# WISDEM/RAFT

Measured on AMD Instinct MI355X. Metric: design-case-frequency solves/sec (whole node), higher is better.
Workload: dtype f64

## Files before the change

raft_amd/csrc/raftx_geom.h:

```cpp
#pragma once

#define MP_N 24
#define MH_N 48
#define MI_N 48

__host__ __device__ inline void derive_design_tables(const double *strips, int64_t i0, int64_t i1, double *dsv,
                                                     int *dsf) {
    int64_t s = i0;
    while (s < i1) {
        int64_t e = s + 1;
        double proj[64];
        int np = 0;
        while (e < i1 && (e - s) < 64) {
            const double *pr = strips + (size_t)(e - 1) * NF, *cr = strips + (size_t)e * NF;
            bool same = true;
            double dv[3], pj = 0.0;
            for (int j = 0; j < 3; j++) {
                same = same && (pr[RAFTX_F_Q + j] == cr[RAFTX_F_Q + j]);
                dv[j] = cr[RAFTX_F_X + j] - pr[RAFTX_F_X + j];
                pj += dv[j] * cr[RAFTX_F_Q + j];
            }
            if (!same || !(pj > 0.0) || !(fabs(pj) <= 1.797e308)) break;
            double perp2 = 0.0, scale = 1.0;
            for (int j = 0; j < 3; j++) {
                double t = dv[j] - pj * cr[RAFTX_F_Q + j];
                perp2 += t * t;
                scale += fabs(cr[RAFTX_F_X + j]);
            }
            if (sqrt(perp2) > 1e-10 * scale) break;
            proj[np++] = pj;
            e++;
        }
        double unit = 0.0;
        for (int i = 0; i < np; i++) unit = (unit == 0.0 || proj[i] < unit) ? proj[i] : unit;
        for (int64_t i = s; i < e; i++) {
            const double *rec = strips + (size_t)i * NF;
            double *o = dsv + (size_t)i * DS_N;
            int m = 0;
            if (i > s && unit > 0.0) {
                double ratio = proj[i - s - 1] / unit;
                int mi = (int)floor(ratio + 0.5);
                if (mi >= 1 && mi <= 2 && fabs(ratio - mi) < 1e-9) {
                    const double *pr = strips + (size_t)(i - 1) * NF;
                    bool ok = true;
                    for (int j = 0; j < 3; j++) {
                        double pred = pr[RAFTX_F_X + j] + (double)mi * unit * rec[RAFTX_F_Q + j];
                        if (fabs(pred - rec[RAFTX_F_X + j]) > 1e-10 * (1.0 + fabs(rec[RAFTX_F_X + j]))) ok = false;
                    }
                    if (ok) m = mi;
                }
            }
            if (m != 0) {
                const double *pr = strips + (size_t)(i - 1) * NF;
                for (int j = 0; j < 3; j++)
                    if (pr[RAFTX_F_P1 + j] != rec[RAFTX_F_P1 + j] || pr[RAFTX_F_P2 + j] != rec[RAFTX_F_P2 + j]) m = 0;
                if ((pr[RAFTX_F_CIRC] != 0.0) != (rec[RAFTX_F_CIRC] != 0.0)) m = 0;
                if ((pr[RAFTX_F_MCF] >= 0.0) != (rec[RAFTX_F_MCF] >= 0.0)) m = 0;
                for (int j = 0; j < 3; j++) {
                    const double da = rec[RAFTX_F_AX + j] - pr[RAFTX_F_AX + j], dx = rec[RAFTX_F_X + j] - pr[RAFTX_F_X + j];
                    if (!(fabs(da - dx) <= 1e-9 * (1.0 + fabs(rec[RAFTX_F_X + j]) + fabs(rec[RAFTX_F_AX + j])))) m = 0;
                }
            }
            dsf[(size_t)i] = m | (rec[RAFTX_F_CIRC] != 0.0 ? DSI_CIRC : 0);
            for (int j = 0; j < DS_N; j++) o[j] = 0.0;
            o[DS_MCF] = rec[RAFTX_F_MCF];
            for (int j = 0; j < 3; j++) {
                o[DS_X + j] = rec[RAFTX_F_X + j];
                o[DS_U + j] = unit * rec[RAFTX_F_Q + j];
                o[DS_A + j] = rec[RAFTX_F_AX + j];
                o[DS_Q + j] = rec[RAFTX_F_Q + j];
                o[DS_P1 + j] = rec[RAFTX_F_P1 + j];
                o[DS_P2 + j] = rec[RAFTX_F_P2 + j];
            }
            if (fabs(o[DS_P1]) < 1e-15 && fabs(o[DS_P1 + 1]) < 1e-15 && fabs(o[DS_P2 + 2]) < 1e-15) dsf[(size_t)i] |= DSI_AXAL;
            if (fabs(o[DS_Q]) < 1e-15 && fabs(o[DS_Q + 1]) < 1e-15 && fabs(o[DS_P1 + 2]) < 1e-15 && fabs(o[DS_P2 + 2]) < 1e-15)
                dsf[(size_t)i] |= DSI_VAX;
            o[DS_IQ] = rec[RAFTX_F_IQ];
            o[DS_IQ + 1] = rec[RAFTX_F_IP1];
            o[DS_IQ + 2] = rec[RAFTX_F_IP2];
            o[DS_IQ + 3] = rec[RAFTX_F_AI];
            o[DS_IQ + 4] = rec[RAFTX_F_RHOV];
            o[DS_DQ] = rec[RAFTX_F_DQ];
            o[DS_DQ + 1] = rec[RAFTX_F_DP1];
            o[DS_DQ + 2] = rec[RAFTX_F_DP2];
            o[DS_DQ + 3] = rec[RAFTX_F_DEND];
        }
        s = e;
    }
}

struct GeomArgs {
    int nDesign;
    int64_t nMember;
    const int64_t *memberOff;
    const double *gm;
    const int64_t *stationOff;
    const double *gs;
    const double *pose;
    const int *mdesign;
    const int64_t *capOff;
    const double *caps;
    double *minert;
    int *err;
    double *Ms, *Cs, *Ws;
    const double *Fz;
    double *drho;
    double rho, g;
    int nw;
    const double *k;
    int *cnt, *cntm;
    double *mpose, *mhyd;
    double *abi;
    double *mcfaux;
    cplx *cm;
    int64_t *off, *cmoff;
    double *ds;
    int *dsi;
    double *A, *Ch, *Wh, *props;
    double *M0, *C0;
    int add_mask;
    int addup_in_design;
    long long *tot;
    long long *hostOut;
    int64_t mbase, sbase, cbase;
    int *mdesign_w;
    int mgrid;
    const double *fixRec;
    const int *fixInt, *fixIdx;
    int fixNM;
    __device__ int64_t mo(int d) const { return memberOff[d] - mbase; }
    __device__ int64_t so(int64_t m) const { return stationOff[m] - sbase; }
    __device__ int64_t co(int64_t m) const { return capOff[m] - cbase; }
};

#define GEOM_NOFMA _Pragma("clang fp contract(off)")

__device__ inline double geom_interp(double x, const double *gs, int n, int f) {
    GEOM_NOFMA
    if (x < gs[RAFTX_GS_S]) return gs[f];
    if (x > gs[(size_t)(n - 1) * RAFTX_GS_N + RAFTX_GS_S]) return gs[(size_t)(n - 1) * RAFTX_GS_N + f];
    int j = 0;
    for (int i = 0; i < n; i++)
        if (gs[(size_t)i * RAFTX_GS_N + RAFTX_GS_S] <= x) j = i;
    const double fj = gs[(size_t)j * RAFTX_GS_N + f];
    if (j == n - 1) return fj;
    const double xj = gs[(size_t)j * RAFTX_GS_N + RAFTX_GS_S];
    if (xj == x) return fj;
    const double slope = (gs[(size_t)(j + 1) * RAFTX_GS_N + f] - fj) / (gs[(size_t)(j + 1) * RAFTX_GS_N + RAFTX_GS_S] - xj);
    return slope * (x - xj) + fj;
}

struct GLocate {
    int idx;
    int j;
    double xj, dx;
};
__device__ inline GLocate geom_locate(double x, const double *gs, int n) {
    GEOM_NOFMA
    GLocate L{0, 0, 0.0, 0.0};
    if (x < gs[RAFTX_GS_S]) return L;
    if (x > gs[(size_t)(n - 1) * RAFTX_GS_N + RAFTX_GS_S]) { L.idx = n - 1; return L; }
    int j = 0;
    for (int i0 = 0; i0 < n; i0 += 8) {
        double sv[8];
#pragma unroll
        for (int u = 0; u < 8; u++) sv[u] = gs[(size_t)min(i0 + u, n - 1) * RAFTX_GS_N + RAFTX_GS_S];
#pragma unroll
        for (int u = 0; u < 8; u++)
            if (i0 + u < n && sv[u] <= x) j = i0 + u;
    }
    L.j = j;
    L.idx = j;
    if (j == n - 1) return L;
    L.xj = gs[(size_t)j * RAFTX_GS_N + RAFTX_GS_S];
    if (L.xj == x) return L;
    L.dx = gs[(size_t)(j + 1) * RAFTX_GS_N + RAFTX_GS_S] - L.xj;
    L.idx = -1;
    return L;
}
__device__ inline double geom_interp_at(const GLocate &L, double x, const double *gs, int f) {
    GEOM_NOFMA
    if (L.idx >= 0) return gs[(size_t)L.idx * RAFTX_GS_N + f];
    const double fj = gs[(size_t)L.j * RAFTX_GS_N + f];
    const double slope = (gs[(size_t)(L.j + 1) * RAFTX_GS_N + f] - fj) / L.dx;
    return slope * (x - L.xj) + fj;
}

__device__ inline int geom_interval_strips(double lstrip, double dlsMax) {
    GEOM_NOFMA
    if (lstrip > 0.0) return (int)ceil(lstrip / dlsMax);
    return lstrip == 0.0 ? 1 : 0;
}

struct GStrip {
    double ls, dls, ds0, ds1, drs0, drs1;
};
__device__ inline GStrip geom_strip(const double *gs, int n, int g, int j, int nsub, bool circ) {
    GEOM_NOFMA
    GStrip s;
    const int c1 = circ ? 0 : 1;
    if (g == 0) {
        s.ls = 0.0; s.dls = 0.0;
        s.ds0 = 0.5 * gs[RAFTX_GS_D]; s.ds1 = 0.5 * gs[RAFTX_GS_D + c1];
        s.drs0 = s.ds0; s.drs1 = s.ds1;
    } else if (g == n) {
        const double *b = gs + (size_t)(n - 1) * RAFTX_GS_N;
        s.ls = b[RAFTX_GS_S]; s.dls = 0.0;
        s.ds0 = 0.5 * b[RAFTX_GS_D]; s.ds1 = 0.5 * b[RAFTX_GS_D + c1];
        s.drs0 = -0.5 * b[RAFTX_GS_D]; s.drs1 = -0.5 * b[RAFTX_GS_D + c1];
    } else {
        const double *a = gs + (size_t)(g - 1) * RAFTX_GS_N, *b = gs + (size_t)g * RAFTX_GS_N;
        const double lstrip = b[RAFTX_GS_S] - a[RAFTX_GS_S];
        if (lstrip > 0.0) {
            const double dl = lstrip / nsub;
            const double m0 = 0.5 * (b[RAFTX_GS_D] - a[RAFTX_GS_D]) / lstrip;
            const double m1 = 0.5 * (b[RAFTX_GS_D + c1] - a[RAFTX_GS_D + c1]) / lstrip;
            s.ls = a[RAFTX_GS_S] + dl * (0.5 + j);
            s.dls = dl;
            s.ds0 = a[RAFTX_GS_D] + dl * 2 * m0 * (0.5 + j);
            s.ds1 = a[RAFTX_GS_D + c1] + dl * 2 * m1 * (0.5 + j);
            s.drs0 = dl * m0;
            s.drs1 = dl * m1;
        } else {
            s.ls = a[RAFTX_GS_S]; s.dls = 0.0;
            s.ds0 = 0.5 * (a[RAFTX_GS_D] + b[RAFTX_GS_D]); s.ds1 = 0.5 * (a[RAFTX_GS_D + c1] + b[RAFTX_GS_D + c1]);
            s.drs0 = 0.5 * (b[RAFTX_GS_D] - a[RAFTX_GS_D]); s.drs1 = 0.5 * (b[RAFTX_GS_D + c1] - a[RAFTX_GS_D + c1]);
        }
    }
    return s;
}
__device__ __forceinline__ void geom_strip_volumes(const GStrip &st, bool circ, double z, double &v_i, double &v_end, double &a_i) {
    GEOM_NOFMA
    const double ds0 = st.ds0, ds1 = st.ds1, dr0 = st.drs0, dr1 = st.drs1, dls = st.dls;
    if (circ) {
        v_i = 0.25 * M_PI * ds0 * ds0 * dls;
        const double a3 = ds0 + dr0, b3 = ds0 - dr0;
        v_end = M_PI / 12.0 * fabs(a3 * a3 * a3 - b3 * b3 * b3);
        a_i = M_PI * ds0 * dr0;
    } else {
        v_i = ds0 * ds1 * dls;
        const double ma = 0.5 * ((ds0 + dr0) + (ds1 + dr1)), mb = 0.5 * ((ds0 - dr0) + (ds1 - dr1));
        v_end = M_PI / 12.0 * (ma * ma * ma - mb * mb * mb);
        a_i = (ds0 + dr0) * (ds1 + dr1) - (ds0 - dr0) * (ds1 - dr1);
    }
    if (z + 0.5 * dls > 0) v_i = v_i * (0.5 * dls - z) / dls;
}
__device__ inline double geom_along(double rA, double rB, double ls, double L) {
    GEOM_NOFMA
    return rA + (ls / L) * (rB - rA);
}

__device__ inline void geom_frustum(double a0, double a1, double b0, double b1, bool circ, double H, double &V, double &hc) {
    GEOM_NOFMA
    const double sA = circ ? a0 : a0 + a1, sB = circ ? b0 : b0 + b1;
    if (sA == 0.0 && sB == 0.0) { V = 0.0; hc = 0.0; return; }
    double A1, A2, Am;
    if (circ) {
        A1 = (M_PI / 4) * a0 * a0; A2 = (M_PI / 4) * b0 * b0; Am = (M_PI / 4) * a0 * b0;
    } else {
        A1 = a0 * a1; A2 = b0 * b1; Am = sqrt(A1 * A2);
    }
    V = (A1 + A2 + Am) * H / 3;
    hc = ((A1 + 2 * Am + 3 * A2) / (A1 + Am + A2)) * H / 4;
}


__device__ inline double geom_pow5(double r) {
    GEOM_NOFMA
    const double h2 = r * r, l2 = fma(r, r, -h2);
    double h4 = h2 * h2, l4 = fma(h2, h2, -h4) + 2.0 * h2 * l2;
    const double s = h4 + l4;
    l4 = l4 - (s - h4);
    h4 = s;
    const double h5 = h4 * r, l5 = fma(h4, r, -h5) + l4 * r;
    return h5 + l5;
}
__device__ inline void geom_frustum_moi(double dA, double dB, double H, double p, double &Irad, double &Iax) {
    GEOM_NOFMA
    if (H == 0) { Irad = 0; Iax = 0; return; }
    const double r1 = dA / 2, r2 = dB / 2;
    if (dA == dB) {
        Irad = (1.0 / 12) * (p * H * M_PI * r1 * r1) * (3 * r1 * r1 + 4 * H * H);
        Iax = (1.0 / 2) * p * M_PI * H * r1 * r1 * r1 * r1;
    } else {
        const double q5 = (geom_pow5(r2) - geom_pow5(r1)) / (r2 - r1);
        Irad = (1.0 / 20) * p * M_PI * H * q5 + (1.0 / 30) * p * M_PI * H * H * H * (r1 * r1 + 3 * r1 * r2 + 6 * r2 * r2);
        Iax = (1.0 / 10) * p * M_PI * H * q5;
    }
}
__device__ inline void geom_rect_moi(double La, double Wa, double Lb, double Wb, double H, double p, double (&Iv)[3]) {
    GEOM_NOFMA
    if (H == 0) { Iv[0] = Iv[1] = Iv[2] = 0; return; }
    double x2, y2, z2;
    if (La == Lb && Wa == Wb) {
        const double M = p * La * Wa * H;
        Iv[0] = (1.0 / 12) * M * (Wa * Wa + 4 * H * H);
        Iv[1] = (1.0 / 12) * M * (La * La + 4 * H * H);
        Iv[2] = (1.0 / 12) * M * (La * La + Wa * Wa);
        return;
    } else if (La != Lb && Wa != Wb) {
        const double dL = Lb - La, dW = Wb - Wa;
        x2 = (1.0 / 12) * p * (dL * dL * dL * H * (Wb / 5 + Wa / 20) + dL * dL * La * H * (3 * Wb / 4 + Wa / 4) +
                               dL * La * La * H * (Wb + Wa / 2) + La * La * La * H * (Wb / 2 + Wa / 2));
        y2 = (1.0 / 12) * p * (dW * dW * dW * H * (Lb / 5 + La / 20) + dW * dW * Wa * H * (3 * Lb / 4 + La / 4) +
                               dW * Wa * Wa * H * (Lb + La / 2) + Wa * Wa * Wa * H * (Lb / 2 + La / 2));
        z2 = p * (Wb * Lb / 5 + Wa * Lb / 20 + La * Wb / 20 + Wa * La * (1.0 / 30)) * H * H * H;
    } else if (La == Lb) {
        x2 = (1.0 / 24) * p * (La * La * La) * H * (Wb + Wa);
        y2 = (1.0 / 48) * p * La * H * (Wb * Wb * Wb + Wa * Wb * Wb + Wa * Wa * Wb + Wa * Wa * Wa);
        z2 = (1.0 / 12) * p * La * (H * H * H) * (3 * Wb + Wa);
    } else {
        x2 = (1.0 / 48) * p * Wa * H * (Lb * Lb * Lb + La * Lb * Lb + La * La * Lb + La * La * La);
        y2 = (1.0 / 24) * p * (Wa * Wa * Wa) * H * (Lb + La);
        z2 = (1.0 / 12) * p * Wa * (H * H * H) * (3 * Lb + La);
    }
    Iv[0] = y2 + z2; Iv[1] = x2 + z2; Iv[2] = x2 + y2;
}
__device__ inline double geom_interp_inner(double x, const double *gs, int n, int c) {
    GEOM_NOFMA
#define DIN_(j) (gs[(size_t)(j) * RAFTX_GS_N + RAFTX_GS_D + c] - 2 * gs[(size_t)(j) * RAFTX_GS_N + RAFTX_GS_T])
    if (x < gs[RAFTX_GS_S]) return DIN_(0);
    if (x > gs[(size_t)(n - 1) * RAFTX_GS_N + RAFTX_GS_S]) return DIN_(n - 1);
    int j = 0;
    for (int i = 0; i < n; i++)
        if (gs[(size_t)i * RAFTX_GS_N + RAFTX_GS_S] <= x) j = i;
    const double fj = DIN_(j);
    if (j == n - 1) return fj;
    const double xj = gs[(size_t)j * RAFTX_GS_N + RAFTX_GS_S];
    if (xj == x) return fj;
    const double slope = (DIN_(j + 1) - fj) / (gs[(size_t)(j + 1) * RAFTX_GS_N + RAFTX_GS_S] - xj);
    return slope * (x - xj) + fj;
#undef DIN_
}
__device__ inline void geom_add_submember(double *M, double mass, const double (&Iv)[3], const double *p1, const double *p2,
                                          const double *q, const double (&r)[3], bool whole = false) {
    GEOM_NOFMA
    const double H[3][3] = {{0, r[2], -r[1]}, {-r[2], 0, r[0]}, {r[1], -r[0], 0}};
    for (int i = 0; i < 3; i++)
        for (int j = 0; j < 3; j++) {
            double hh = 0.0;
            for (int l = 0; l < 3; l++) hh += H[i][l] * mass * H[j][l];
            M[i * 6 + j] += (i == j) ? mass : 0.0;
            M[i * 6 + 3 + j] += mass * H[i][j];
            M[(3 + i) * 6 + j] += mass * H[j][i];
            const double ir = p1[i] * Iv[0] * p1[j] + p2[i] * Iv[1] * p2[j] + q[i] * Iv[2] * q[j];
            M[(3 + i) * 6 + 3 + j] += hh + (whole ? trunc(ir) : ir);
        }
}

struct GInertia {
    double M[36], mc[3], I3[3], vfill;
};
__device__ inline void geom_inertia_init(GInertia &J) {
    for (int i = 0; i < 36; i++) J.M[i] = 0.0;
    for (int c = 0; c < 3; c++) { J.mc[c] = 0.0; J.I3[c] = 0.0; }
    J.vfill = 0.0;
}
__device__ inline void geom_inertia_section(GInertia &J, const double *a, const double *b, bool circ, double rho_shell, bool trim,
                                            double drho, const double *rA, const double *q, const double *p1, const double *p2) {
    GEOM_NOFMA
    double (&M)[36] = J.M;
    double (&mc)[3] = J.mc;
    double (&I3)[3] = J.I3;
    double &vfill = J.vfill;
    {
        const double l = b[RAFTX_GS_S] - a[RAFTX_GS_S];
        double mass = 0.0, center[3] = {0, 0, 0};
        if (l > 0) {
            const double l_fill = (trim && a[RAFTX_GS_RHOFILL] == 0.0) ? 0.0 : a[RAFTX_GS_LFILL];
            const double rho_fill = a[RAFTX_GS_RHOFILL] + (l_fill > 0.0 ? drho : 0.0);
            const double dA0 = a[RAFTX_GS_D], dA1 = (circ ? a[RAFTX_GS_D] : a[RAFTX_GS_D + 1]), dB0 = b[RAFTX_GS_D], dB1 = (circ ? b[RAFTX_GS_D] : b[RAFTX_GS_D + 1]);
            const double iA0 = dA0 - 2 * a[RAFTX_GS_T], iA1 = dA1 - 2 * a[RAFTX_GS_T];
            const double iB0 = dB0 - 2 * b[RAFTX_GS_T], iB1 = dB1 - 2 * b[RAFTX_GS_T];
            const double f0 = (iB0 - iA0) * (l_fill / l) + iA0, f1 = (iB1 - iA1) * (l_fill / l) + iA1;
            double Vo, hco, Vi, hci, vf, hcf;
            geom_frustum(dA0, dA1, dB0, dB1, circ, l, Vo, hco);
            geom_frustum(iA0, iA1, iB0, iB1, circ, l, Vi, hci);
            const double m_shell = (Vo - Vi) * rho_shell;
            const double hc_shell = (Vo - Vi != 0) ? ((hco * Vo) - (hci * Vi)) / (Vo - Vi) : 0.0;
            geom_frustum(iA0, iA1, f0, f1, circ, l_fill, vf, hcf);
            vfill += vf;
            const double m_fill = vf * rho_fill;
            mass = m_shell + m_fill;
            const double hc = (mass != 0) ? ((hcf * m_fill) + (hc_shell * m_shell)) / mass : 0.0;
            if (circ) {
                double Iro, Iao, Iri, Iai, Irf, Iaf;
                geom_frustum_moi(dA0, dB0, l, rho_shell, Iro, Iao);
                geom_frustum_moi(iA0, iB0, l, rho_shell, Iri, Iai);
                geom_frustum_moi(iA0, f0, l_fill, rho_fill, Irf, Iaf);
                I3[0] = I3[1] = ((Iro - Iri) + Irf) - mass * hc * hc;
                I3[2] = (Iao - Iai) + Iaf;
            } else {
                double Io[3], Ii[3], If[3];
                geom_rect_moi(dA0, dA1, dB0, dB1, l, rho_shell, Io);
                geom_rect_moi(iA0, iA1, iB0, iB1, l, rho_shell, Ii);
                geom_rect_moi(iA0, iA1, f0, f1, l_fill, rho_fill, If);
                I3[0] = ((Io[0] - Ii[0]) + If[0]) - mass * hc * hc;
                I3[1] = ((Io[1] - Ii[1]) + If[1]) - mass * hc * hc;
                I3[2] = (Io[2] - Ii[2]) + If[2];
            }
            for (int c = 0; c < 3; c++) center[c] = rA[c] + q[c] * (a[RAFTX_GS_S] + hc);
        }
        double rel[3];
        for (int c = 0; c < 3; c++) { mc[c] += mass * center[c]; rel[c] = center[c] - rA[c]; }
        geom_add_submember(M, mass, I3, p1, p2, q, rel, !(l > 0));
    }
}
__device__ inline int geom_inertia_caps_finish(GInertia &J, const double *gs, int n, const double *gc, int ncap, bool circ,
                                               double rho_shell, const double *rA, const double *q, const double *p1,
                                               const double *p2, double g, double *out) {
    GEOM_NOFMA
    const int c1 = circ ? 0 : 1;
    double (&M)[36] = J.M;
    double (&mc)[3] = J.mc;
    const double vfill = J.vfill;
    const double s0 = gs[RAFTX_GS_S], s1 = gs[(size_t)(n - 1) * RAFTX_GS_N + RAFTX_GS_S];
    for (int i = 0; i < ncap; i++) {
        const double *cp = gc + (size_t)i * RAFTX_GC_N;
        const double Lc = cp[RAFTX_GC_S], h = cp[RAFTX_GC_T];
        double dA[2] = {0, 0}, dB[2] = {0, 0}, dAi[2] = {0, 0}, dBi[2] = {0, 0};
        int where;
        if (Lc == s0) {
            where = 0;
            for (int c = 0; c <= c1; c++) {
                dA[c] = gs[RAFTX_GS_D + c] - 2 * gs[RAFTX_GS_T];
                dB[c] = geom_interp_inner(Lc + h, gs, n, c);
                dAi[c] = cp[RAFTX_GC_DIN + c];
                dBi[c] = dB[c] * (dAi[c] / dA[c]);
            }
        } else if (Lc == s1) {
            where = 1;
            if (!circ) return 2;
            dA[0] = geom_interp_inner(Lc - h, gs, n, 0);
            dB[0] = gs[(size_t)(n - 1) * RAFTX_GS_N + RAFTX_GS_D] - 2 * gs[(size_t)(n - 1) * RAFTX_GS_N + RAFTX_GS_T];
            dBi[0] = cp[RAFTX_GC_DIN];
            dAi[0] = dA[0] * (dBi[0] / dB[0]);
        } else if ((Lc > s0 && Lc < s0 + h) || (Lc < s1 && Lc > s1 - h)) {
            return 3;
        } else {
            where = 2;
            if (!circ) return 2;
            if (i < ncap - 1 && Lc == gc[(size_t)(i + 1) * RAFTX_GC_N + RAFTX_GC_S]) {
                if (i >= n) return 4;
                dA[0] = geom_interp_inner(Lc - h, gs, n, 0);
                dB[0] = gs[(size_t)i * RAFTX_GS_N + RAFTX_GS_D] - 2 * gs[(size_t)i * RAFTX_GS_N + RAFTX_GS_T];
                dBi[0] = cp[RAFTX_GC_DIN];
                dAi[0] = dA[0] * (dBi[0] / dB[0]);
            } else if (i > 0 && Lc == gc[(size_t)(i - 1) * RAFTX_GC_N + RAFTX_GC_S]) {
                if (i >= n) return 4;
                dA[0] = gs[(size_t)i * RAFTX_GS_N + RAFTX_GS_D] - 2 * gs[(size_t)i * RAFTX_GS_N + RAFTX_GS_T];
                dB[0] = geom_interp_inner(Lc + h, gs, n, 0);
                dAi[0] = cp[RAFTX_GC_DIN];
                dBi[0] = dB[0] * (dAi[0] / dA[0]);
            } else {
                dA[0] = geom_interp_inner(Lc - h / 2, gs, n, 0);
                dB[0] = geom_interp_inner(Lc + h / 2, gs, n, 0);
                const double dM = geom_interp_inner(Lc, gs, n, 0);
                dAi[0] = dA[0] * (cp[RAFTX_GC_DIN] / dM);
                dBi[0] = dB[0] * (cp[RAFTX_GC_DIN] / dM);
            }
        }
        double Vo, hco, Vi, hci;
        geom_frustum(dA[0], dA[1], dB[0], dB[1], circ, h, Vo, hco);
        geom_frustum(dAi[0], dAi[1], dBi[0], dBi[1], circ, h, Vi, hci);
        const double m_cap = (Vo - Vi) * rho_shell;
        const double hc_cap = (Vo - Vi != 0) ? ((hco * Vo) - (hci * Vi)) / (Vo - Vi) : 0.0;
        double Ic[3];
        if (circ) {
            double Iro, Iao, Iri, Iai;
            geom_frustum_moi(dA[0], dB[0], h, rho_shell, Iro, Iao);
            geom_frustum_moi(dAi[0], dBi[0], h, rho_shell, Iri, Iai);
            Ic[0] = Ic[1] = (Iro - Iri) - m_cap * hc_cap * hc_cap;
            Ic[2] = Iao - Iai;
        } else {
            double Io[3], Ii[3];
            geom_rect_moi(dA[0], dA[1], dB[0], dB[1], h, rho_shell, Io);
            geom_rect_moi(dAi[0], dAi[1], dBi[0], dBi[1], h, rho_shell, Ii);
            Ic[0] = (Io[0] - Ii[0]) - m_cap * hc_cap * hc_cap;
            Ic[1] = (Io[1] - Ii[1]) - m_cap * hc_cap * hc_cap;
            Ic[2] = Io[2] - Ii[2];
        }
        double rel[3];
        for (int c = 0; c < 3; c++) {
            const double pos = rA[c] + q[c] * Lc;
            const double cc = (where == 0) ? pos + q[c] * hc_cap : (where == 1 ? pos - q[c] * (h - hc_cap) : pos - q[c] * ((h / 2) - hc_cap));
            rel[c] = cc - rA[c];
            mc[c] += m_cap * cc;
        }
        geom_add_submember(M, m_cap, Ic, p1, p2, q, rel);
    }
    const double mass = M[0];
    for (int i = 0; i < 36; i++) out[i] = M[i];
    out[36] = mass;
    double dR[3];
    for (int c = 0; c < 3; c++) {
        const double cen = (mass != 0) ? mc[c] / mass : 0.0;
        out[37 + c] = cen;
        dR[c] = cen - rA[c];
    }
    const double Fz = -g * mass;
    out[40] = 0.0; out[41] = 0.0; out[42] = Fz;
    out[43] = dR[1] * Fz; out[44] = -dR[0] * Fz; out[45] = 0.0;
    out[46] = -mass * g * dR[2];
    out[47] = vfill;
    return 0;
}
__device__ inline int geom_member_inertia(const double *gm, const double *gs, int n, const double *gc, int ncap,
                                          const double *rA, const double *q, const double *p1, const double *p2, double g,
                                          bool trim, double drho, double *out) {
    const bool circ = gm[RAFTX_GM_SHAPE] != 0.0;
    const double rho_shell = gm[RAFTX_GM_RHOSHELL];
    GInertia J;
    geom_inertia_init(J);
    for (int i = 1; i < n; i++)
        geom_inertia_section(J, gs + (size_t)(i - 1) * RAFTX_GS_N, gs + (size_t)i * RAFTX_GS_N, circ, rho_shell, trim, drho, rA, q, p1, p2);
    return geom_inertia_caps_finish(J, gs, n, gc, ncap, circ, rho_shell, rA, q, p1, p2, g, out);
}

__global__ void k_geom_zero(GeomArgs A) {
    const int d = blockIdx.x * blockDim.x + threadIdx.x;
    if (d < A.nDesign) {
        A.drho[d] = 0.0;
        A.off[d + 1] = 0;
        A.cmoff[d + 1] = 0;
    }
    if (d < 4) A.err[d] = 0;
    if (d < 5) A.tot[d] = 0;
    if (d == 0) { A.off[0] = 0; A.cmoff[0] = 0; }
    if (d < A.nDesign)
        for (int64_t m = A.mo(d); m < A.mo(d + 1); m++) A.mdesign_w[m] = d;
}
#define GEOM_MAX_STATIONS 1024
__device__ inline int64_t geom_member_of_thread(const GeomArgs &A) {
    const int64_t t = (int64_t)blockIdx.x * blockDim.x + threadIdx.x;
    if (A.mgrid <= 0) return t < A.nMember ? t : -1;
    const int64_t k = t / A.nDesign;
    if (k >= A.mgrid) return -1;
    const int d = (int)(t % A.nDesign);
    const int64_t m = A.mo(d) + k;
    return m < A.mo(d + 1) ? m : -1;
}
__device__ __forceinline__ void geom_load_row(const double *gs, int i, double (&r)[RAFTX_GS_N]) {
    const double2 *p = reinterpret_cast<const double2 *>(gs + (size_t)i * RAFTX_GS_N);
#pragma unroll
    for (int k = 0; k < RAFTX_GS_N / 2; k++) {
        const double2 v = p[k];
        r[2 * k] = v.x;
        r[2 * k + 1] = v.y;
    }
}
struct GMember {
    int wet, wetm;
    int code;
    int rej;
};
__device__ __forceinline__ void geom_pose(const double *gm, const double (&ps)[6], double (&rA0)[3], double (&q)[3], double (&p1)[3],
                                          double (&p2)[3], double (&rA)[3], double (&rB)[3], double (&R)[2][2]) {
    GEOM_NOFMA
    double q0[3], nrm = 0.0;
    for (int i = 0; i < 3; i++) {
        rA0[i] = gm[RAFTX_GM_RA + i];
        q0[i] = gm[RAFTX_GM_RB + i] - gm[RAFTX_GM_RA + i];
        nrm += q0[i] * q0[i];
    }
    nrm = sqrt(nrm);
    for (int i = 0; i < 3; i++) q0[i] /= nrm;
    const double beta = atan2(q0[1], q0[0]);
    const double phi = atan2(sqrt(q0[0] * q0[0] + q0[1] * q0[1]), q0[2]);
    const double gam = gm[RAFTX_GM_GAMMA] * (M_PI / 180.0);
    const double s1 = sin(beta), c1 = cos(beta), s2 = sin(phi), c2 = cos(phi), s3 = sin(gam), c3 = cos(gam);
    const double R0[3][3] = {{c1 * c2 * c3 - s1 * s3, -c3 * s1 - c1 * c2 * s3, c1 * s2},
                             {c1 * s3 + c2 * c3 * s1, c1 * c3 - c2 * s1 * s3, s1 * s2},
                             {-c3 * s2, s2 * s3, c2}};
    const double p10[3] = {R0[0][0], R0[1][0], R0[2][0]};
    const double p20[3] = {q0[1] * p10[2] - q0[2] * p10[1], q0[2] * p10[0] - q0[0] * p10[2], q0[0] * p10[1] - q0[1] * p10[0]};
    const double sy = sin(ps[5]), cy = cos(ps[5]), sp = sin(ps[4]), cp = cos(ps[4]), sr = sin(ps[3]), cr = cos(ps[3]);
    const double Rp[3][3] = {{cy * cp, cy * sp * sr - cr * sy, sy * sr + cy * cr * sp},
                             {cp * sy, cy * cr + sy * sp * sr, cr * sy * sp - cy * sr},
                             {-sp, cp * sr, cp * cr}};
    const double L = gm[RAFTX_GM_L];
    for (int i = 0; i < 3; i++) {
        q[i] = Rp[i][0] * q0[0] + Rp[i][1] * q0[1] + Rp[i][2] * q0[2];
        p1[i] = Rp[i][0] * p10[0] + Rp[i][1] * p10[1] + Rp[i][2] * p10[2];
        p2[i] = Rp[i][0] * p20[0] + Rp[i][1] * p20[1] + Rp[i][2] * p20[2];
        const double dsp = (Rp[i][0] - (i == 0 ? 1.0 : 0.0)) * rA0[0] + (Rp[i][1] - (i == 1 ? 1.0 : 0.0)) * rA0[1] +
                           (Rp[i][2] - (i == 2 ? 1.0 : 0.0)) * rA0[2];
        rA[i] = rA0[i] + (ps[i] + dsp);
    }
    for (int i = 0; i < 3; i++) rB[i] = rA[i] + L * q[i];
    for (int i = 0; i < 2; i++)
        for (int j = 0; j < 2; j++) R[i][j] = Rp[i][0] * R0[0][j] + Rp[i][1] * R0[1][j] + Rp[i][2] * R0[2][j];
}
#define FR_N (MP_N + MH_N + MI_N)
#define FR_I 4
__device__ __forceinline__ GMember geom_member_body(const double *gmrow, const double *gs, const int n, const double *gc, const int ncap,
                                                    const double *pose, const double rho, const double g, const bool trim,
                                                    const bool haveK, double *mp, double *mh, double *mi) {
    GEOM_NOFMA
    GMember res = {0, 0, 0, 0};
    double gm[RAFTX_GM_N];
    {
        const double2 *p = reinterpret_cast<const double2 *>(gmrow);
#pragma unroll
        for (int k = 0; k < RAFTX_GM_N / 2; k++) {
            const double2 v = p[k];
            gm[2 * k] = v.x;
            gm[2 * k + 1] = v.y;
        }
    }
    if (n < 2 || n > GEOM_MAX_STATIONS || !(gm[RAFTX_GM_DLSMAX] > 0.0) || !(gm[RAFTX_GM_L] > 0.0)) {
        res.rej = 1;
        return res;
    }
    if (((int)gm[RAFTX_GM_FLAGS] & RAFTX_GM_FLAG_MCF) && gm[RAFTX_GM_SHAPE] != 0.0 && !haveK) {
        res.rej = 2;
        return res;
    }
    double ps[6] = {0, 0, 0, 0, 0, 0};
    if (pose)
        for (int i = 0; i < 6; i++) ps[i] = pose[i];
    double a[RAFTX_GS_N], b[RAFTX_GS_N];
    geom_load_row(gs, 0, b);
    const bool circ = gm[RAFTX_GM_SHAPE] != 0.0;
    const int flags = (int)gm[RAFTX_GM_FLAGS];
    double rA0[3], q[3], p1[3], p2[3], rA[3], rB[3], R[2][2];
    const double L = gm[RAFTX_GM_L];
    geom_pose(gm, ps, rA0, q, p1, p2, rA, rB, R);
    int wet = 0;
    if (geom_along(rA[2], rB[2], 0.0, L) < 0) wet++;
    double C[36], F[6], Vt = 0.0, rcV[3] = {0, 0, 0}, AWPm = 0.0;
    for (int i = 0; i < 36; i++) C[i] = 0.0;
    for (int i = 0; i < 6; i++) F[i] = 0.0;
    const double beta2 = atan2(q[1], q[0]), phi2 = atan2(sqrt(q[0] * q[0] + q[1] * q[1]), q[2]);
    const double cosPhi = cos(phi2), sinPhi = sin(phi2), tanPhi = tan(phi2), cosBeta = cos(beta2), sinBeta = sin(beta2);
    const double rg = rho * g;
    const bool nostatic = (flags & RAFTX_GM_FLAG_NOSTATIC) != 0;
    const double rho_shell = gm[RAFTX_GM_RHOSHELL];
    for (int i = 1; i < n; i++) {
#pragma unroll
        for (int f = 0; f < RAFTX_GS_N; f++) a[f] = b[f];
        geom_load_row(gs, i, b);
        {
            const double lstrip = b[RAFTX_GS_S] - a[RAFTX_GS_S];
            const int cntg = geom_interval_strips(lstrip, gm[RAFTX_GM_DLSMAX]);
            for (int j = 0; j < cntg; j++) {
                double ls;
                if (lstrip > 0.0) {
                    const double dl = lstrip / cntg;
                    ls = a[RAFTX_GS_S] + dl * (0.5 + j);
                } else {
                    ls = a[RAFTX_GS_S];
                }
                if (geom_along(rA[2], rB[2], ls, L) < 0) wet++;
            }
        }
        if (nostatic) continue;
        {
            double ra[3], rb[3];
            for (int c = 0; c < 3; c++) {
                ra[c] = rA[c] + q[c] * a[RAFTX_GS_S];
                rb[c] = rA[c] + q[c] * b[RAFTX_GS_S];
            }
            const double aD1 = circ ? a[RAFTX_GS_D] : a[RAFTX_GS_D + 1], bD1 = circ ? b[RAFTX_GS_D] : b[RAFTX_GS_D + 1];
            if (ra[2] * rb[2] <= 0) {
                const double t = (0 - ra[2]);
                double xWP = ra[0] + t * (rb[0] - ra[0]) / (rb[2] - ra[2]);
                double yWP = ra[1] + t * (rb[1] - ra[1]) / (rb[2] - ra[2]);
                const double w0 = b[RAFTX_GS_D] + t * (a[RAFTX_GS_D] - b[RAFTX_GS_D]) / (rb[2] - ra[2]);
                const double w1 = bD1 + t * (aD1 - bD1) / (rb[2] - ra[2]);
                double AWP, IxWP, IyWP;
                if (circ) {
                    AWP = (M_PI / 4) * w0 * w0;
                    IxWP = IyWP = (M_PI / 64) * w0 * w0 * w0 * w0;
                } else {
                    AWP = w0 * w1;
                    const double Ix = (1.0 / 12) * w0 * w1 * w1 * w1, Iy = (1.0 / 12) * w0 * w0 * w0 * w1;
                    IxWP = R[0][0] * Ix * R[0][0] + R[0][1] * Iy * R[0][1];
                    IyWP = R[1][0] * Ix * R[1][0] + R[1][1] * Iy * R[1][1];
                }
                const double LWP = fabs(ra[2] / cosPhi);
                double V, hc;
                geom_frustum(a[RAFTX_GS_D], aD1, w0, w1, circ, LWP, V, hc);
                double M = 0.0;
                if (circ) M = -rg * M_PI * (w0 * w0 / 32 * (2.0 + tanPhi * tanPhi) + 0.5 * (ra[2] / cosPhi) * (ra[2] / cosPhi)) * sinPhi;
                const double Fz = rg * V;
                const double ex = ra[0] - rA[0], ey = ra[1] - rA[1];
                F[2] += Fz;
                F[3] += ey * Fz;
                F[4] += -ex * Fz;
                F[3] += M * (-sinBeta);
                F[4] += M * cosBeta;
                xWP -= rA[0];
                yWP -= rA[1];
                C[2 * 6 + 2] += rg * AWP / cosPhi;
                C[2 * 6 + 3] += rg * (-AWP * yWP);
                C[2 * 6 + 4] += rg * (AWP * xWP);
                C[3 * 6 + 2] += rg * (-AWP * yWP);
                C[3 * 6 + 3] += rg * (IxWP + AWP * yWP * yWP);
                C[3 * 6 + 4] += rg * (AWP * xWP * yWP);
                C[4 * 6 + 2] += rg * (AWP * xWP);
                C[4 * 6 + 3] += rg * (AWP * xWP * yWP);
                C[4 * 6 + 4] += rg * (IyWP + AWP * xWP * xWP);
                double rc[3];
                for (int c = 0; c < 3; c++) rc[c] = ra[c] + q[c] * hc;
                C[3 * 6 + 3] += rg * V * (rc[2] - rA[2]);
                C[4 * 6 + 4] += rg * V * (rc[2] - rA[2]);
                C[3 * 6 + 5] += -rg * V * (rc[0] - rA[0]);
                C[4 * 6 + 5] += -rg * V * (rc[1] - rA[1]);
                Vt += V;
                for (int c = 0; c < 3; c++) rcV[c] += rc[c] * V;
                AWPm = AWP;
            } else if (ra[2] <= 0 && rb[2] <= 0) {
                double V, hc;
                geom_frustum(a[RAFTX_GS_D], aD1, b[RAFTX_GS_D], bD1, circ, b[RAFTX_GS_S] - a[RAFTX_GS_S], V, hc);
                double rc[3], rr[3];
                for (int c = 0; c < 3; c++) { rc[c] = ra[c] + q[c] * hc; rr[c] = rc[c] - rA[c]; }
                const double Fz = rg * V;
                F[2] += Fz;
                F[3] += rr[1] * Fz;
                F[4] += -rr[0] * Fz;
                C[3 * 6 + 3] += rg * V * rr[2];
                C[4 * 6 + 4] += rg * V * rr[2];
                C[3 * 6 + 5] += -rg * V * rr[0];
                C[4 * 6 + 5] += -rg * V * rr[1];
                Vt += V;
                for (int c = 0; c < 3; c++) rcV[c] += rc[c] * V;
            }
        }
    }
    if (geom_along(rA[2], rB[2], b[RAFTX_GS_S], L) < 0) wet++;
    if (!nostatic) {
        for (int i = 0; i < 36; i++) mh[i] = C[i];
        for (int i = 0; i < 6; i++) mh[36 + i] = F[i];
        mh[42] = Vt; mh[43] = rcV[0]; mh[44] = rcV[1]; mh[45] = rcV[2]; mh[46] = AWPm; mh[47] = 0.0;
    }
    int code = 0;
    if (!nostatic) {
        GInertia J;
        geom_inertia_init(J);
        geom_load_row(gs, 0, b);
        for (int i = 1; i < n; i++) {
#pragma unroll
            for (int f = 0; f < RAFTX_GS_N; f++) a[f] = b[f];
            geom_load_row(gs, i, b);
            geom_inertia_section(J, a, b, circ, rho_shell, trim, 0.0, rA, q, p1, p2);
        }
        code = geom_inertia_caps_finish(J, gs, n, gc, ncap, circ, rho_shell, rA, q, p1, p2, g, mi);
    }
    for (int i = 0; i < 3; i++) {
        mp[i] = rA0[i]; mp[3 + i] = rA[i]; mp[6 + i] = q[i]; mp[9 + i] = p1[i]; mp[12 + i] = p2[i];
    }
    mp[15] = R[0][0]; mp[16] = R[0][1]; mp[17] = R[1][0]; mp[18] = R[1][1]; mp[19] = L;
    const int wetm = ((flags & RAFTX_GM_FLAG_MCF) && circ && !(flags & RAFTX_GM_FLAG_POTMOD)) ? wet : 0;
    res.wet = wet;
    res.wetm = wetm;
    if (nostatic) {
        for (int i = 0; i < MH_N; i++) mh[i] = 0.0;
        for (int i = 0; i < MI_N; i++) mi[i] = 0.0;
        return res;
    }
    if (code) {
        for (int i = 0; i < MI_N; i++) mi[i] = 0.0;
        res.code = code;
    }
    return res;
}

struct FixedArgs {
    int nFix;
    const double *gm, *gs, *gc;
    const int *desc;
    double rho, g;
    int trim, haveK;
    double *rec;
    int *irec;
};
__global__ __launch_bounds__(64) void k_geom_member_fixed(FixedArgs F) {
    const int f = blockIdx.x * blockDim.x + threadIdx.x;
    if (f >= F.nFix) return;
    const int *ds = F.desc + (size_t)f * 5;
    double *r = F.rec + (size_t)f * FR_N;
    const GMember R = geom_member_body(F.gm + (size_t)ds[0] * RAFTX_GM_N, F.gs + (size_t)ds[1] * RAFTX_GS_N, ds[2],
                                       ds[4] >= 0 ? F.gc + (size_t)ds[3] * RAFTX_GC_N : nullptr, ds[4] >= 0 ? ds[4] : 0, nullptr, F.rho,
                                       F.g, F.trim != 0, F.haveK != 0, r, r + MP_N, r + MP_N + MH_N);
    int *ir = F.irec + (size_t)f * FR_I;
    ir[0] = R.wet; ir[1] = R.wetm; ir[2] = R.code; ir[3] = R.rej;
}
__global__ __launch_bounds__(128) void k_geom_member(GeomArgs A) {
    GEOM_NOFMA
    if (A.mgrid > 0 && A.err[2]) return;
    const int64_t m = geom_member_of_thread(A);
    if (m < 0) return;
    if (A.err[2]) {
        A.cnt[m] = 0;
        A.cntm[m] = 0;
        return;
    }
    GMember R;
    int d;
    const int fix = A.fixRec ? A.fixIdx[m % A.fixNM] : -1;
    if (fix >= 0) {
        d = (int)(m / A.fixNM);
        const int4 ir = *reinterpret_cast<const int4 *>(A.fixInt + (size_t)fix * FR_I);
        R.wet = ir.x; R.wetm = ir.y; R.code = ir.z; R.rej = ir.w;
        if (!R.rej) {
            const double2 *src = reinterpret_cast<const double2 *>(A.fixRec + (size_t)fix * FR_N);
            double2 *mp = reinterpret_cast<double2 *>(A.mpose + (size_t)m * MP_N), *mh = reinterpret_cast<double2 *>(A.mhyd + (size_t)m * MH_N),
                    *mi = reinterpret_cast<double2 *>(A.minert + (size_t)m * MI_N);
#pragma unroll
            for (int i = 0; i < MP_N / 2; i++) mp[i] = src[i];
#pragma unroll 8
            for (int i = 0; i < MH_N / 2; i++) mh[i] = src[MP_N / 2 + i];
#pragma unroll 8
            for (int i = 0; i < MI_N / 2; i++) mi[i] = src[(MP_N + MH_N) / 2 + i];
        }
    } else {
        const int64_t so0 = A.so(m), so1 = A.so(m + 1);
        const int64_t co0 = A.capOff ? A.co(m) : 0, co1 = A.capOff ? A.co(m + 1) : 0;
        d = A.mdesign[m];
        R = geom_member_body(A.gm + (size_t)m * RAFTX_GM_N, A.gs + (size_t)so0 * RAFTX_GS_N, (int)(so1 - so0),
                             A.capOff ? A.caps + (size_t)co0 * RAFTX_GC_N : nullptr, A.capOff ? (int)(co1 - co0) : 0,
                             A.pose ? A.pose + (size_t)d * 6 : nullptr, A.rho, A.g, (A.add_mask & RAFTX_TRIM_BALLAST) != 0, A.k != nullptr,
                             A.mpose + (size_t)m * MP_N, A.mhyd + (size_t)m * MH_N, A.minert + (size_t)m * MI_N);
    }
    if (R.rej) {
        A.cnt[m] = 0;
        A.cntm[m] = 0;
        atomicCAS(A.err + 3, 0, R.rej == 1 ? (int)(m + 1) : -(int)(m + 1));
        return;
    }
    A.cnt[m] = R.wet;
    A.cntm[m] = R.wetm;
    if (R.wet) atomicAdd(reinterpret_cast<unsigned long long *>(A.off + d + 1), (unsigned long long)R.wet);
    if (R.wetm) atomicAdd(reinterpret_cast<unsigned long long *>(A.cmoff + d + 1), (unsigned long long)R.wetm);
    if (R.code) atomicCAS(A.err, 0, (int)(m + 1));
}

__global__ void k_geom_trim(GeomArgs A) {
    GEOM_NOFMA
    if (A.err[2] | A.err[3]) return;
    const int d = blockIdx.x * blockDim.x + threadIdx.x;
    if (d >= A.nDesign) return;
    double mass = A.M0[(size_t)d * 36], V = 0.0, vol = 0.0;
    for (int64_t m = A.mo(d); m < A.mo(d + 1); m++) {
        mass += A.minert[(size_t)m * MI_N + 36];
        vol += A.minert[(size_t)m * MI_N + 47];
        V += A.mhyd[(size_t)m * MH_N + 42];
    }
    if (!(vol > 0.0)) {
        A.drho[d] = 0.0;
        atomicCAS(A.err + 1, 0, d + 1);
        return;
    }
    const double sumFz = -mass * A.g + V * A.rho * A.g + (A.Fz ? A.Fz[d] : 0.0);
    A.drho[d] = sumFz / A.g / vol;
}
__global__ __launch_bounds__(128) void k_geom_reinertia(GeomArgs A) {
    GEOM_NOFMA
    if (A.err[2] | A.err[3]) return;
    const int64_t m = geom_member_of_thread(A);
    if (m < 0) return;
    const double *gm = A.gm + (size_t)m * RAFTX_GM_N;
    if ((int)gm[RAFTX_GM_FLAGS] & RAFTX_GM_FLAG_NOSTATIC) return;
    const double *gs = A.gs + (size_t)A.so(m) * RAFTX_GS_N;
    const int n = (int)(A.so(m + 1) - A.so(m));
    const double *mp = A.mpose + (size_t)m * MP_N;
    const int ncap = A.capOff ? (int)(A.co(m + 1) - A.co(m)) : 0;
    const double *gc = A.capOff ? A.caps + (size_t)A.co(m) * RAFTX_GC_N : nullptr;
    double *mi = A.minert + (size_t)m * MI_N;
    if (geom_member_inertia(gm, gs, n, gc, ncap, mp + 3, mp + 6, mp + 9, mp + 12, A.g, true, A.drho[A.mdesign[m]], mi))
        for (int i = 0; i < MI_N; i++) mi[i] = 0.0;
}

#define GSCAN_CH 4096
template <int T>
__global__ __launch_bounds__(T) void k_geom_scan_t(GeomArgs A) {
    __shared__ long long part[2][17];
    __shared__ unsigned buf[2][GSCAN_CH];
    const int t = threadIdx.x;
    const int n = A.nDesign;
    constexpr int PER = GSCAN_CH / T;
    long long carrya = 0, carryb = 0, mx = 0;
    for (int c0 = 0; c0 < n; c0 += GSCAN_CH) {
        const int cn = (n - c0 < GSCAN_CH) ? n - c0 : GSCAN_CH;
        for (int i = t; i < GSCAN_CH; i += T) {
            long long va = 0, vb = 0;
            if (i < cn) { va = A.off[c0 + i + 1]; vb = A.cmoff[c0 + i + 1]; }
            buf[0][i] = (unsigned)va;
            buf[1][i] = (unsigned)vb;
            mx = va > mx ? va : mx;
        }
        __syncthreads();
        long long a = 0, b = 0;
        for (int i = 0; i < PER; i++) { a += buf[0][t * PER + i]; b += buf[1][t * PER + i]; }
        const int lane = t & 63, wv = t >> 6;
        long long ia = a, ib = b;
        for (int o = 1; o < 64; o <<= 1) {
            const long long ua = __shfl_up(ia, o, 64), ub = __shfl_up(ib, o, 64);
            if (lane >= o) { ia += ua; ib += ub; }
        }
        if (lane == 63) { part[0][wv] = ia; part[1][wv] = ib; }
        __syncthreads();
        long long ra = carrya, rb = carryb, sa = 0, sb = 0;
        for (int i = 0; i < T / 64; i++) {
            if (i < wv) { ra += part[0][i]; rb += part[1][i]; }
            sa += part[0][i]; sb += part[1][i];
        }
        ra += ia - a;
        rb += ib - b;
        for (int i = 0; i < PER; i++) {
            ra += buf[0][t * PER + i];
            rb += buf[1][t * PER + i];
            buf[0][t * PER + i] = (unsigned)ra;
            buf[1][t * PER + i] = (unsigned)rb;
        }
        __syncthreads();
        for (int i = t; i < cn; i += T) {
            const long long va = buf[0][i], vb = buf[1][i];
            A.off[c0 + i + 1] = va;
            A.cmoff[c0 + i + 1] = vb;
            if (A.hostOut) A.hostOut[8 + c0 + i + 1] = va;
        }
        carrya += sa;
        carryb += sb;
        __syncthreads();
    }
    if (mx) atomicMax(reinterpret_cast<unsigned long long *>(A.tot + 2), (unsigned long long)mx);
    __syncthreads();
    if (t == 0) {
        A.off[0] = 0;
        A.cmoff[0] = 0;
        A.tot[0] = carrya;
        A.tot[1] = carryb;
        if (A.hostOut) {
            A.hostOut[0] = carrya;
            A.hostOut[1] = carryb;
            A.hostOut[2] = A.tot[2];
            int *e = reinterpret_cast<int *>(A.hostOut + 3);
            e[0] = A.err[0]; e[1] = A.err[1]; e[2] = A.err[2]; e[3] = A.err[3];
            A.hostOut[8] = 0;
        }
    }
}
__global__ __launch_bounds__(64) void k_geom_mcf(GeomArgs A, int64_t nRows) {
    GEOM_NOFMA
    const int64_t row = blockIdx.x;
    const int iw = blockIdx.y * blockDim.x + threadIdx.x;
    if (row >= nRows || iw >= A.nw) return;
    const double R = A.mcfaux[row * 3], Ca1 = A.mcfaux[row * 3 + 1], Ca2 = A.mcfaux[row * 3 + 2];
    const double k = A.k[iw];
    const double Tr = M_PI / 5 / R;
    double ramp;
    if (k <= 0.0) ramp = 0.0;
    else if (k < Tr) ramp = 0.5 * (1 - cos(M_PI * k / Tr));
    else ramp = 1.0;
    double cr = 0.0, ci = 0.0;
    if (ramp != 0.0) {
        const double x = k * R;
        const double hr = 0.5 * (j0(x) - jn(2, x)), hi = 0.5 * (y0(x) - yn(2, x));
        const double den = M_PI * (x * x);
        const double mag = den * (hr * hr + hi * hi);
        cr = 4.0 * hi / mag;
        ci = 4.0 * hr / mag;
    }
    A.cm[((size_t)row * 2 + 0) * A.nw + iw] = cplx{cr * ramp + (1.0 + Ca1) * (1 - ramp), ci * ramp};
    A.cm[((size_t)row * 2 + 1) * A.nw + iw] = cplx{cr * ramp + (1.0 + Ca2) * (1 - ramp), ci * ramp};
}


__device__ inline void geom_reduce_matrix(const double *C, const double (&a)[3], double *out) {
    GEOM_NOFMA
    const double H[3][3] = {{0, a[2], -a[1]}, {-a[2], 0, a[0]}, {a[1], -a[0], 0}};
    double t12[3][3], t21[3][3];
    for (int i = 0; i < 3; i++)
        for (int j = 0; j < 3; j++) {
            double s12 = C[i * 6 + 3 + j], s21 = C[(3 + i) * 6 + j];
            for (int l = 0; l < 3; l++) {
                s12 += C[i * 6 + l] * H[l][j];
                s21 += H[l][i] * C[l * 6 + j];
            }
            t12[i][j] = s12;
            t21[i][j] = s21;
        }
    for (int i = 0; i < 3; i++)
        for (int j = 0; j < 3; j++) {
            out[i * 6 + j] += C[i * 6 + j];
            out[i * 6 + 3 + j] += t12[i][j];
            out[(3 + i) * 6 + j] += t21[i][j];
            double s = C[(3 + i) * 6 + 3 + j];
            for (int l = 0; l < 3; l++) s += H[l][i] * t12[l][j] + C[(3 + i) * 6 + l] * H[l][j];
            out[(3 + i) * 6 + 3 + j] += s;
        }
}
__device__ inline void geom_reduce_vector(const double *W, const double (&a)[3], const double *arm0, const double (&th)[3],
                                          double *Wout, double *Cout) {
    GEOM_NOFMA
    Wout[0] += W[0]; Wout[1] += W[1]; Wout[2] += W[2];
    Wout[3] += W[3] + (a[1] * W[2] - a[2] * W[1]);
    Wout[4] += W[4] + (a[2] * W[0] - a[0] * W[2]);
    Wout[5] += W[5] + (a[0] * W[1] - a[1] * W[0]);
    for (int j = 0; j < 3; j++) {
        double tj[3] = {th[0], th[1], th[2]};
        tj[j] += 1.0;
        const double dA[3] = {arm0[0] + (tj[1] * a[2] - tj[2] * a[1]) - a[0], arm0[1] + (tj[2] * a[0] - tj[0] * a[2]) - a[1],
                              arm0[2] + (tj[0] * a[1] - tj[1] * a[0]) - a[2]};
        Cout[3 * 6 + 3 + j] -= dA[1] * W[2] - dA[2] * W[1];
        Cout[4 * 6 + 3 + j] -= dA[2] * W[0] - dA[0] * W[2];
        Cout[5 * 6 + 3 + j] -= dA[0] * W[1] - dA[1] * W[0];
    }
}

__device__ constexpr int DS_SRC[DS_N] = {
    -1, -1, RAFTX_F_MCF, -1,
    RAFTX_F_X, RAFTX_F_X + 1, RAFTX_F_X + 2,
    -2, -3, -4,
    RAFTX_F_AX, RAFTX_F_AX + 1, RAFTX_F_AX + 2,
    RAFTX_F_Q, RAFTX_F_Q + 1, RAFTX_F_Q + 2,
    RAFTX_F_P1, RAFTX_F_P1 + 1, RAFTX_F_P1 + 2,
    RAFTX_F_P2, RAFTX_F_P2 + 1, RAFTX_F_P2 + 2,
    RAFTX_F_IQ, RAFTX_F_IP1, RAFTX_F_IP2, RAFTX_F_AI, RAFTX_F_RHOV,
    RAFTX_F_DQ, RAFTX_F_DP1, RAFTX_F_DP2, RAFTX_F_DEND, -1};
static_assert(DS_MCF == 2 && DS_X == 4 && DS_U == 7 && DS_A == 10 && DS_Q == 13 && DS_P1 == 16 && DS_P2 == 19 &&
              DS_IQ == 22 && DS_DQ == 27 && DS_N == 32, "DS_SRC follows the device record layout");
#define GD_ROW (NF + 1)
#define GD_GM_N 3
#define GD_MP_N 13
#ifdef GEOM_PHASE_TIMING
__device__ unsigned long long geom_phase_cycles[10];
#define GEOM_PHASE(i)                                                                                   \
    do {                                                                                                \
        __syncthreads();                                                                                \
        const unsigned long long now_ = wall_clock64();                                                 \
        if (threadIdx.x == 0) atomicAdd(&geom_phase_cycles[i], now_ - tphase_);                         \
        tphase_ = now_;                                                                                 \
    } while (0)
#define GEOM_PHASE_BEGIN unsigned long long tphase_ = wall_clock64();
#else
#define GEOM_PHASE(i)
#define GEOM_PHASE_BEGIN
#endif
#ifndef GD_T
#define GD_T 128
#endif
static_assert(GD_T % 64 == 0 && GD_T % DS_N == 0 && GD_T <= 256, "k_geom_design: whole wavefronts, a lane keeps its record field");
template <bool ABI, bool ADDUP>
__device__ __forceinline__ void geom_design_block(const GeomArgs &A, const int d, double *gd_lds, int *wcnt) {
    GEOM_NOFMA
    const int lane = threadIdx.x;
    const int64_t i0 = A.off[d], i1 = A.off[d + 1];
    const int S = (int)(i1 - i0);
    double *rec = gd_lds;
    double *pjv = rec + (size_t)S * GD_ROW, *unv = pjv + S;
    int *okv = reinterpret_cast<int *>(unv + S), *rsv = okv + S, *mfl = rsv + S;
    GEOM_PHASE_BEGIN
    {
        const int64_t m0 = A.mo(d), m1 = A.mo(d + 1);
        const int nMem = (int)(m1 - m0);
        const int64_t s0 = A.so(m0);
        const int nSta = (int)(A.so(m1) - s0);
        int *mcum = mfl + S;
        int *mbase = mcum + nSta + 2 * nMem;
        int *ssta = mbase + nMem + 1;
        double *sgm = reinterpret_cast<double *>(okv + (((int)(ssta - okv) + nMem + 2) & ~1));
        double *sgs = sgm + (size_t)nMem * GD_GM_N;
        double *smp = sgs + (size_t)nSta * RAFTX_GS_N;
        int cnt_lane = 0;
        {
            const double *g0 = A.gm + (size_t)m0 * RAFTX_GM_N, *g1 = A.gs + (size_t)s0 * RAFTX_GS_N, *g2 = A.mpose + (size_t)m0 * MP_N;
            const int n0 = nMem * GD_GM_N, n01 = n0 + nSta * RAFTX_GS_N, total = n01 + nMem * GD_MP_N;
            constexpr int SU = 10;
            const int64_t so_lane = lane <= nMem ? A.so(m0 + lane) : s0;
            cnt_lane = lane < nMem ? A.cnt[m0 + lane] : 0;
            for (int base = 0; base < total; base += SU * GD_T) {
                double v[SU];
#pragma unroll
                for (int u = 0; u < SU; u++) {
                    const int idx = base + u * GD_T + lane;
                    const double *src;
                    if (idx < n0) {
                        const int row = idx / GD_GM_N, col = idx % GD_GM_N;
                        src = g0 + (size_t)row * RAFTX_GM_N + (col == 0 ? RAFTX_GM_DLSMAX : (col == 1 ? RAFTX_GM_SHAPE : RAFTX_GM_FLAGS));
                    } else if (idx < n01) {
                        src = g1 + (idx - n0);
                    } else {
                        const int k = idx - n01, row = k / GD_MP_N, col = k % GD_MP_N;
                        src = g2 + (size_t)row * MP_N + (col < 12 ? 3 + col : 19);
                    }
                    v[u] = idx < total ? *src : 0.0;
                }
#pragma unroll
                for (int u = 0; u < SU; u++) {
                    const int idx = base + u * GD_T + lane;
                    if (idx < total) sgm[idx] = v[u];
                }
            }
            if (lane <= nMem) mbase[lane] = ssta[lane] = (int)(so_lane - s0);
            for (int mi = lane + GD_T; mi <= nMem; mi += GD_T) mbase[mi] = ssta[mi] = (int)(A.so(m0 + mi) - s0);
        }
        __syncthreads();
        for (int u = lane; u < nSta + nMem; u += GD_T) {
            int mi = 0;
            while (mi + 1 < nMem && mbase[mi + 1] + mi + 1 <= u) mi++;
            const int sta0 = mbase[mi], n = mbase[mi + 1] - sta0, g = u - (sta0 + mi);
            int cntg = 1;
            if (g > 0 && g < n) {
                const double *gs = sgs + (size_t)sta0 * RAFTX_GS_N;
                cntg = geom_interval_strips(gs[(size_t)g * RAFTX_GS_N + RAFTX_GS_S] - gs[(size_t)(g - 1) * RAFTX_GS_N + RAFTX_GS_S],
                                            sgm[(size_t)mi * GD_GM_N]);
            }
            mcum[sta0 + 2 * mi + g + 1] = cntg;
        }
        __syncthreads();
        for (int mi = lane; mi < nMem; mi += GD_T) {
            const int n = ssta[mi + 1] - ssta[mi];
            int *cum = mcum + ssta[mi] + 2 * mi;
            const bool dry = (mi == lane ? cnt_lane : A.cnt[m0 + mi]) == 0;
            int a = 0;
            cum[0] = 0;
            for (int g = 0; g <= n; g++) { a += dry ? 0 : cum[g + 1]; cum[g + 1] = a; }
            mbase[mi + 1] = a;
        }
        __syncthreads();
        if (lane == 0) {
            int a = 0;
            mbase[0] = 0;
            for (int mi = 0; mi < nMem; mi++) { a += mbase[mi + 1]; mbase[mi + 1] = a; }
        }
        __syncthreads();
        const int total = mbase[nMem];
        GEOM_PHASE(0);
        const double rho = A.rho, cdrag = sqrt(8 / M_PI);
        double rP[3] = {0, 0, 0};
        if (A.pose)
            for (int i = 0; i < 3; i++) rP[i] = A.pose[(size_t)d * 6 + i];
        int nwet = 0;
        for (int t0 = 0; t0 < total; t0 += GD_T) {
            const int t = t0 + lane;
            const bool act = t < total;
            const int tq = act ? t : 0;
            int mi = 0;
            while (mi + 1 < nMem && mbase[mi + 1] <= tq) mi++;
            const int64_t m = m0 + mi;
            const int tt = tq - mbase[mi];
            const int n = ssta[mi + 1] - ssta[mi];
            const int *cum = mcum + ssta[mi] + 2 * mi;
            const double *gm = sgm + (size_t)mi * GD_GM_N;
            const double *gs = sgs + (size_t)ssta[mi] * RAFTX_GS_N;
            const double *mp = smp + (size_t)mi * GD_MP_N;
            const bool circ = gm[1] != 0.0;
            const int flags = (int)gm[2];
            const bool potMod = flags & RAFTX_GM_FLAG_POTMOD;
            const bool mcf = (flags & RAFTX_GM_FLAG_MCF) && circ && !potMod;
            const double L = mp[12];
            double rA[3], rB[3], q[3], p1[3], p2[3], armN[3];
            for (int i = 0; i < 3; i++) {
                rA[i] = mp[i]; q[i] = mp[3 + i]; p1[i] = mp[6 + i]; p2[i] = mp[9 + i];
                rB[i] = rA[i] + L * q[i];
                armN[i] = rA[i] - rP[i];
            }
            int g = 0;
            while (g < n && cum[g + 1] <= tt) g++;
            const int j = tt - cum[g];
            const int nsub = (g > 0 && g < n) ? cum[g + 1] - cum[g] : 1;
            GStrip st = geom_strip(gs, n, g, j, nsub, circ);
            double r[3];
            for (int c = 0; c < 3; c++) r[c] = geom_along(rA[c], rB[c], st.ls, L);
            const bool wet = act && (r[2] < 0);
            const GLocate at = geom_locate(st.ls, gs, n);
            const unsigned long long mask = __ballot(wet);
            const int wv = lane >> 6, ln = lane & 63;
            if (ln == 0) wcnt[wv] = __popcll(mask);
            __syncthreads();
            int before = 0, all = 0;
            for (int w = 0; w < GD_T / 64; w++) {
                before += w < wv ? wcnt[w] : 0;
                all += wcnt[w];
            }
            const int pos = nwet + before + __popcll(mask & ((1ull << ln) - 1ull));
            nwet += all;
            __syncthreads();
            if (!wet || pos >= S) continue;
            double *row = rec + (size_t)pos * GD_ROW;
            for (int c = 0; c < NF; c++) row[c] = 0.0;
            for (int c = 0; c < 3; c++) {
                row[RAFTX_F_X + c] = r[c];
                row[RAFTX_F_AX + c] = (r[c] - rA[c]) + armN[c];
                row[RAFTX_F_Q + c] = q[c];
                row[RAFTX_F_P1 + c] = p1[c];
                row[RAFTX_F_P2 + c] = p2[c];
            }
            row[RAFTX_F_CIRC] = circ ? 1.0 : 0.0;
            row[RAFTX_F_MCF] = -1.0;
            row[26] = (double)mi;
            row[27] = (double)tt;
            const double ds0 = st.ds0, ds1 = st.ds1, dr0 = st.drs0, dr1 = st.drs1, dls = st.dls;
            if (!potMod) {
                double v_i, v_end, a_i;
                geom_strip_volumes(st, circ, r[2], v_i, v_end, a_i);
                const double Ca1 = geom_interp_at(at, st.ls, gs, RAFTX_GS_CA + 1), Ca2 = geom_interp_at(at, st.ls, gs, RAFTX_GS_CA + 2);
                const double CaE = geom_interp_at(at, st.ls, gs, RAFTX_GS_CA + 3);
                row[RAFTX_F_IQ] = rho * v_end * CaE;
                row[RAFTX_F_AI] = a_i;
                row[RAFTX_F_RHOV] = rho * v_i;
                row[RAFTX_F_AP1] = rho * v_i * Ca1;
                row[RAFTX_F_AP2] = rho * v_i * Ca2;
                if (mcf) {
                    int64_t cmbase = A.cmoff[d], cmrow0 = cmbase;
                    int wet0 = 0;
                    for (int64_t mm = m0; mm < m; mm++) { cmrow0 += A.cntm[mm]; wet0 += A.cnt[mm]; }
                    const int posm = pos - wet0;
                    row[RAFTX_F_MCF] = (double)((cmrow0 - cmbase) + posm);
                    double *ax = A.mcfaux + (size_t)(cmrow0 + posm) * 3;
                    ax[0] = ds0 / 2; ax[1] = Ca1; ax[2] = Ca2;
                } else {
                    row[RAFTX_F_IP1] = rho * v_i * (1.0 + Ca1);
                    row[RAFTX_F_IP2] = rho * v_i * (1.0 + Ca2);
                }
            }
            double a_q, a_p1, a_p2, a_end;
            if (circ) {
                a_q = M_PI * ds0 * dls; a_p1 = ds0 * dls; a_p2 = ds0 * dls; a_end = fabs(M_PI * ds0 * dr0);
            } else {
                a_q = 2 * (ds0 + ds0) * dls; a_p1 = ds0 * dls; a_p2 = ds1 * dls;
                a_end = fabs((ds0 + dr0) * (ds1 + dr1) - (ds0 - dr0) * (ds1 - dr1));
            }
            row[RAFTX_F_DQ] = cdrag * 0.5 * rho * a_q * geom_interp_at(at, st.ls, gs, RAFTX_GS_CD + 0);
            row[RAFTX_F_DP1] = cdrag * 0.5 * rho * a_p1 * geom_interp_at(at, st.ls, gs, RAFTX_GS_CD + 1);
            row[RAFTX_F_DP2] = cdrag * 0.5 * rho * a_p2 * geom_interp_at(at, st.ls, gs, RAFTX_GS_CD + 2);
            row[RAFTX_F_DEND] = cdrag * 0.5 * rho * a_end * geom_interp_at(at, st.ls, gs, RAFTX_GS_CD + 3);
        }
        __syncthreads();
        GEOM_PHASE(1);
        if constexpr (ABI) {
            double *abi = A.abi + (size_t)i0 * NF;
            for (int t = lane; t < S * NF; t += GD_T) abi[t] = rec[(t / NF) * GD_ROW + (t % NF)];
        }
    }
    __syncthreads();
    GEOM_PHASE(2);
    for (int t = lane; t < S; t += GD_T) {
        bool pass = false;
        double pj = 0.0;
        const double *pr = rec + (size_t)(t > 0 ? t - 1 : 0) * GD_ROW, *cr = rec + (size_t)t * GD_ROW;
        double pq[3], cq[3], px[3], cx[3];
        for (int j = 0; j < 3; j++) {
            pq[j] = pr[RAFTX_F_Q + j]; cq[j] = cr[RAFTX_F_Q + j]; px[j] = pr[RAFTX_F_X + j]; cx[j] = cr[RAFTX_F_X + j];
        }
        if (t > 0) {
            bool same = true;
            double dv[3];
            for (int j = 0; j < 3; j++) {
                same = same && (pq[j] == cq[j]);
                dv[j] = cx[j] - px[j];
                pj += dv[j] * cq[j];
            }
            if (same && (pj > 0.0) && (fabs(pj) <= 1.797e308)) {
                double perp2 = 0.0, scale = 1.0;
                for (int j = 0; j < 3; j++) {
                    double tt = dv[j] - pj * cq[j];
                    perp2 += tt * tt;
                    scale += fabs(cx[j]);
                }
                pass = !(sqrt(perp2) > 1e-10 * scale);
            }
        }
        okv[t] = pass ? 1 : 0;
        pjv[t] = pj;
    }
    __syncthreads();
    bool serial = S > GD_T;
    if (!serial) {
        const int wv = lane >> 6, ln = lane & 63;
        const bool st = lane < S && (lane == 0 || !okv[lane]);
        const unsigned long long mask = __ballot(st);
        if (ln == 0) wcnt[wv] = mask ? wv * 64 + 63 - __builtin_clzll(mask) : -1;
        if (st) reinterpret_cast<unsigned long long *>(unv)[lane] = 0x7ff0000000000000ull;
        __syncthreads();
        const unsigned long long below = mask & (ln == 63 ? ~0ull : ((2ull << ln) - 1ull));
        int s = below ? wv * 64 + 63 - __builtin_clzll(below) : -1;
        for (int w = wv - 1; w >= 0 && s < 0; w--) s = wcnt[w];
        if (lane < S) {
            rsv[lane] = s;
            if (!st) atomicMin(reinterpret_cast<unsigned long long *>(unv) + s, (unsigned long long)__double_as_longlong(pjv[lane]));
        }
        serial = __syncthreads_or(lane < S && lane - s >= 64) != 0;
        if (!serial && st && reinterpret_cast<unsigned long long *>(unv)[lane] == 0x7ff0000000000000ull) unv[lane] = 0.0;
    }
    if (serial && lane == 0) {
        int s = 0;
        double unit = 0.0;
        for (int t = 0; t < S; t++) {
            if (t == 0 || !okv[t] || (t - s) >= 64) {
                if (t > 0) unv[s] = unit;
                s = t;
                unit = 0.0;
            } else {
                const double pj = pjv[t];
                unit = (unit == 0.0 || pj < unit) ? pj : unit;
            }
            rsv[t] = s;
        }
        if (S > 0) unv[s] = unit;
    }
    __syncthreads();
    for (int t = lane; t < S; t += GD_T) {
        const int s = rsv[t];
        const double unit = unv[s];
        const double *cr = rec + (size_t)t * GD_ROW, *pr = rec + (size_t)(t > 0 ? t - 1 : 0) * GD_ROW;
        double cX[3], cQ[3], cP1[3], cP2[3], cA[3], pX[3], pP1[3], pP2[3], pA[3];
        for (int j = 0; j < 3; j++) {
            cX[j] = cr[RAFTX_F_X + j]; cQ[j] = cr[RAFTX_F_Q + j]; cP1[j] = cr[RAFTX_F_P1 + j]; cP2[j] = cr[RAFTX_F_P2 + j];
            cA[j] = cr[RAFTX_F_AX + j];
            pX[j] = pr[RAFTX_F_X + j]; pP1[j] = pr[RAFTX_F_P1 + j]; pP2[j] = pr[RAFTX_F_P2 + j]; pA[j] = pr[RAFTX_F_AX + j];
        }
        const double cCirc = cr[RAFTX_F_CIRC], cMcf = cr[RAFTX_F_MCF], pCirc = pr[RAFTX_F_CIRC], pMcf = pr[RAFTX_F_MCF];
        const double pjt = pjv[t];
        int m = 0;
        if (t > s && unit > 0.0) {
            double ratio = pjt / unit;
            int mi = (int)floor(ratio + 0.5);
            if (mi >= 1 && mi <= 2 && fabs(ratio - mi) < 1e-9) {
                bool ok = true;
                for (int j = 0; j < 3; j++) {
                    double pred = pX[j] + (double)mi * unit * cQ[j];
                    if (fabs(pred - cX[j]) > 1e-10 * (1.0 + fabs(cX[j]))) ok = false;
                }
                if (ok) m = mi;
            }
        }
        if (m != 0) {
            for (int j = 0; j < 3; j++)
                if (pP1[j] != cP1[j] || pP2[j] != cP2[j]) m = 0;
            if ((pCirc != 0.0) != (cCirc != 0.0)) m = 0;
            if ((pMcf >= 0.0) != (cMcf >= 0.0)) m = 0;
            for (int j = 0; j < 3; j++) {
                const double da = cA[j] - pA[j], dx = cX[j] - pX[j];
                if (!(fabs(da - dx) <= 1e-9 * (1.0 + fabs(cX[j]) + fabs(cA[j])))) m = 0;
            }
        }
        int fl = m | (cCirc != 0.0 ? DSI_CIRC : 0);
        if (fabs(cP1[0]) < 1e-15 && fabs(cP1[1]) < 1e-15 && fabs(cP2[2]) < 1e-15) fl |= DSI_AXAL;
        if (fabs(cQ[0]) < 1e-15 && fabs(cQ[1]) < 1e-15 && fabs(cP1[2]) < 1e-15 && fabs(cP2[2]) < 1e-15)
            fl |= DSI_VAX;
        A.dsi[(size_t)i0 + t] = fl;
    }
    GEOM_PHASE(3);
    {
        double *dso = A.ds + (size_t)i0 * DS_N;
        const int j = lane % DS_N, f = DS_SRC[j], nT = S * DS_N;
        constexpr int DU = 4;
        for (int t0 = lane; t0 < nT; t0 += DU * GD_T) {
          double vv[DU];
#pragma unroll
          for (int u = 0; u < DU; u++) {
            const int t = t0 + u * GD_T;
            const int i = t < nT ? t / DS_N : 0;
            const double *cr = rec + (size_t)i * GD_ROW;
            double v = 0.0;
            if (f >= 0) v = cr[f];
            else if (f <= -2) v = unv[rsv[i]] * cr[RAFTX_F_Q + (-2 - f)];
            if (t < nT && j == DS_MCF && v >= 0.0) {
                const double *ax0 = A.mcfaux + (size_t)A.cmoff[d] * 3, *axm = ax0 + (size_t)v * 3;
                const int mrow = (int)v;
                for (int r = 0; r < mrow; r++)
                    if (ax0[r * 3] == axm[0] && ax0[r * 3 + 1] == axm[1] && ax0[r * 3 + 2] == axm[2]) {
                        v = (double)r;
                        break;
                    }
            }
            vv[u] = v;
          }
#pragma unroll
          for (int u = 0; u < DU; u++) {
            const int t = t0 + u * GD_T;
            if (t < nT) dso[t] = vv[u];
          }
        }
    }
    GEOM_PHASE(4);
    constexpr int GV = 21;
    for (int t0 = 0; t0 < S; t0 += GD_T) {
        const int t = t0 + lane;
        double gv[GV];
        if (t < S) {
            const double *cr = rec + (size_t)t * GD_ROW;
            const double ax = cr[RAFTX_F_AX], ay = cr[RAFTX_F_AX + 1], az = cr[RAFTX_F_AX + 2];
            const double cs[3] = {cr[RAFTX_F_AP1], cr[RAFTX_F_AP2], cr[RAFTX_F_IQ]};
            const int fs[3] = {RAFTX_F_P1, RAFTX_F_P2, RAFTX_F_Q};
            for (int tt = 0; tt < 3; tt++) {
                const double nx = cr[fs[tt]], ny = cr[fs[tt] + 1], nz = cr[fs[tt] + 2];
                gv[tt * 7] = cs[tt];
                gv[tt * 7 + 1] = nx; gv[tt * 7 + 2] = ny; gv[tt * 7 + 3] = nz;
                gv[tt * 7 + 4] = ay * nz - az * ny;
                gv[tt * 7 + 5] = az * nx - ax * nz;
                gv[tt * 7 + 6] = ax * ny - ay * nx;
            }
        }
        __syncthreads();
        if (t < S)
            for (int e = 0; e < GV; e++) rec[(size_t)t * GV + e] = gv[e];
    }
    __syncthreads();
    GEOM_PHASE(5);
    {
        const int k3 = lane / 36, e = lane % 36, i = e / 6, j = e % 6;
        double am = 0.0;
        if (k3 < 3) {
            const int lo = (int)(((long long)S * k3) / 3), hi = (int)(((long long)S * (k3 + 1)) / 3);
            for (int s = lo; s < hi; s++) {
                const double *g = rec + (size_t)s * GV;
                for (int tt = 0; tt < 3; tt++) am += g[tt * 7] * g[tt * 7 + 1 + i] * g[tt * 7 + 1 + j];
            }
        }
        __syncthreads();
        if (k3 < 3) rec[lane] = am;
        __syncthreads();
        if (lane < 36) {
            am = (rec[lane] + rec[36 + lane]) + rec[72 + lane];
            const size_t o = (size_t)d * 36 + lane;
            A.A[o] = am;
            if constexpr (ADDUP) {
                double m0 = A.M0[o], c0 = A.C0[o];
                if (A.add_mask & RAFTX_ADD_MORISON) m0 += am;
                if (A.add_mask & RAFTX_ADD_HYDROSTATIC) c0 += A.Ch[o];
                if (A.add_mask & RAFTX_ADD_INERTIA) { m0 += A.Ms[o]; c0 += A.Cs[o]; }
                A.M0[o] = m0;
                A.C0[o] = c0;
            }
        }
    }
    GEOM_PHASE(6);
    (void)mfl;
}
__global__ __launch_bounds__(GD_T) void k_geom_design(GeomArgs A) {
    extern __shared__ double gd_lds[];
    __shared__ int wcnt[GD_T / 64];
    if ((int)blockIdx.x >= A.nDesign) return;
    if (A.abi) geom_design_block<true, false>(A, (int)blockIdx.x, gd_lds, wcnt);
    else if (A.addup_in_design) geom_design_block<false, true>(A, (int)blockIdx.x, gd_lds, wcnt);
    else geom_design_block<false, false>(A, (int)blockIdx.x, gd_lds, wcnt);
}
__global__ void k_geom_addup(GeomArgs A) {
    const size_t o = (size_t)blockIdx.x * blockDim.x + threadIdx.x;
    if (o >= (size_t)A.nDesign * 36) return;
    if (A.add_mask & RAFTX_ADD_MORISON) A.M0[o] += A.A[o];
    if (A.add_mask & RAFTX_ADD_HYDROSTATIC) A.C0[o] += A.Ch[o];
    if (A.add_mask & RAFTX_ADD_INERTIA) { A.M0[o] += A.Ms[o]; A.C0[o] += A.Cs[o]; }
}
static size_t geom_design_lds(int maxS, int maxSta, int maxMem) {
    const size_t S = (size_t)(maxS > 0 ? maxS : 1);
    return sizeof(double) * (S * GD_ROW + 2 * S) + sizeof(int) * (3 * S + (size_t)maxSta + 3 * (size_t)maxMem + 1) + 16 +
           sizeof(int) * ((size_t)maxMem + 4) +
           sizeof(double) * ((size_t)maxMem * (GD_GM_N + GD_MP_N) + (size_t)maxSta * RAFTX_GS_N);
}

__global__ __launch_bounds__(64) void k_geom_reduce(GeomArgs A) {
    GEOM_NOFMA
    const int t = blockIdx.x * blockDim.x + threadIdx.x;
    const int d = t / 3, role = t % 3;
    if (d >= A.nDesign) return;
    double th[3] = {0, 0, 0}, rP[3] = {0, 0, 0};
    if (A.pose)
        for (int i = 0; i < 3; i++) { rP[i] = A.pose[(size_t)d * 6 + i]; th[i] = A.pose[(size_t)d * 6 + 3 + i]; }
    double out[36], Wv[6] = {0, 0, 0, 0, 0, 0}, sc0 = 0.0, sc1 = 0.0, sr[3] = {0, 0, 0};
    for (int i = 0; i < 36; i++) out[i] = 0.0;
    for (int64_t m = A.mo(d); m < A.mo(d + 1); m++) {
        const double *mp = A.mpose + (size_t)m * MP_N, *mh = A.mhyd + (size_t)m * MH_N, *mi = A.minert + (size_t)m * MI_N;
        const double a[3] = {mp[3] - rP[0], mp[4] - rP[1], mp[5] - rP[2]};
        double C[36];
        if (role == 1) {
            for (int i = 0; i < 36; i++) C[i] = 0.0;
            C[3 * 6 + 3] = C[4 * 6 + 4] = mi[46];
        } else {
            const double *src = role == 0 ? mh : mi;
            for (int i = 0; i < 36; i++) C[i] = src[i];
        }
        geom_reduce_matrix(C, a, out);
        if (role < 2) {
            const double *W = role == 0 ? mh + 36 : mi + 40;
            geom_reduce_vector(W, a, mp, th, Wv, out);
        }
        if (role == 2) {
            for (int c = 0; c < 3; c++) sr[c] += ((mi[37 + c] - mp[3 + c]) + mp[c]) * mi[36];
            sc0 += mi[47];
        } else if (role == 0) {
            const double V = mh[42];
            sc0 += V;
            sc1 += mh[46];
            if (V > 0)
                for (int c = 0; c < 3; c++) sr[c] += ((mh[43 + c] / V - mp[3 + c]) + mp[c]) * V;
        }
    }
    for (int i = 0; i < 6; i++)
        for (int j = i + 1; j < 6; j++) {
            const double s = (out[i * 6 + j] + out[j * 6 + i]) / 2;
            out[i * 6 + j] = out[j * 6 + i] = s;
        }
    double *dst = (role == 0 ? A.Ch : role == 1 ? A.Cs : A.Ms) + (size_t)d * 36;
    for (int i = 0; i < 36; i++) dst[i] = out[i];
    double *pr = A.props + (size_t)d * RAFTX_SP_N;
    if (role == 0) {
        for (int i = 0; i < 6; i++) A.Wh[(size_t)d * 6 + i] = Wv[i];
        pr[RAFTX_SP_V] = sc0;
        pr[RAFTX_SP_AWP] = sc1;
        for (int c = 0; c < 3; c++) pr[RAFTX_SP_RCB + c] = sc0 != 0.0 ? sr[c] / sc0 : 0.0;
    } else if (role == 1) {
        for (int i = 0; i < 6; i++) A.Ws[(size_t)d * 6 + i] = Wv[i];
    } else {
        pr[RAFTX_SP_VFILL] = sc0;
        pr[RAFTX_SP_DRHO] = (A.add_mask & RAFTX_TRIM_BALLAST) ? A.drho[d] : 0.0;
        pr[RAFTX_SP_MASS] = out[0];
        for (int c = 0; c < 3; c++) pr[RAFTX_SP_RCG + c] = out[0] != 0.0 ? sr[c] / out[0] : 0.0;
        pr[11] = 0.0;
    }
}

struct ExpandArgs {
    int n, nM, nSt, nCap, nP;
    const double *params;
    const double *gm, *gs, *gc;
    const int *stMember, *capMember;
    const double *stFrac, *fillFrac, *capFrac;
    const double *endCoef, *headCS, *diaCoef;
    const int *endEdit, *diaEdit;
    double *gm_out, *gs_out, *gc_out;
};
__device__ inline double affine_eval(const double *coef, const double *p, int nP) {
    GEOM_NOFMA
    double v = coef[0];
    for (int q = 0; q < nP; q++) v = v + coef[1 + q] * p[q];
    return v;
}
#define GE_T 256
__global__ void __launch_bounds__(GE_T) k_geom_expand(ExpandArgs E, unsigned nbM, unsigned nbS) {
    GEOM_NOFMA
    __shared__ double tile[GE_T * 17];
    const int kind = blockIdx.x < nbM ? 0 : (blockIdx.x < nbM + nbS ? 1 : 2);
    const int nX = kind == 0 ? E.nM : (kind == 1 ? E.nSt : E.nCap);
    const int W = kind == 2 ? RAFTX_GC_N : RAFTX_GM_N;
    const size_t total = (size_t)E.n * nX;
    const size_t row0 = (size_t)(blockIdx.x - (kind == 0 ? 0u : (kind == 1 ? nbM : nbM + nbS))) * GE_T;
    const int nrows = (int)(total - row0 < (size_t)GE_T ? total - row0 : (size_t)GE_T);
    const int t = threadIdx.x;
    if (t < nrows) {
        const size_t R = row0 + t;
        const int d = (int)(R / nX), idx = (int)(R % nX);
        const double *p = E.params + (size_t)d * E.nP;
        const int m = kind == 0 ? idx : (kind == 1 ? E.stMember[idx] : E.capMember[idx]);
        const double *bm = E.gm + (size_t)m * RAFTX_GM_N;
        const bool ed = E.endEdit[m] != 0;
        double e[6] = {0, 0, 0, 0, 0, 0}, L = bm[RAFTX_GM_L];
        if (ed) {
            for (int i = 0; i < 6; i++) e[i] = affine_eval(E.endCoef + ((size_t)m * 6 + i) * (E.nP + 1), p, E.nP);
            const double dx = e[3] - e[0], dy = e[4] - e[1], dz = e[5] - e[2];
            L = sqrt((dx * dx + dy * dy) + dz * dz);
        }
        double *o = tile + t * 17;
        if (kind == 0) {
            for (int i = 0; i < RAFTX_GM_N; i++) o[i] = bm[i];
            if (ed) {
                const double c = E.headCS[2 * m], s = E.headCS[2 * m + 1];
                o[RAFTX_GM_RA + 0] = c * e[0] + (-s) * e[1];
                o[RAFTX_GM_RA + 1] = s * e[0] + c * e[1];
                o[RAFTX_GM_RA + 2] = e[2];
                o[RAFTX_GM_RB + 0] = c * e[3] + (-s) * e[4];
                o[RAFTX_GM_RB + 1] = s * e[3] + c * e[4];
                o[RAFTX_GM_RB + 2] = e[5];
                o[RAFTX_GM_L] = L;
            }
        } else if (kind == 1) {
            const double *b = E.gs + (size_t)idx * RAFTX_GS_N;
            for (int i = 0; i < RAFTX_GS_N; i++) o[i] = b[i];
            if (ed) {
                o[RAFTX_GS_S] = E.stFrac[idx] * L;
                o[RAFTX_GS_LFILL] = E.fillFrac[idx] * L;
            }
            if (E.diaEdit[idx]) {
                o[RAFTX_GS_D] = affine_eval(E.diaCoef + ((size_t)idx * 2 + 0) * (E.nP + 1), p, E.nP);
                o[RAFTX_GS_D + 1] = affine_eval(E.diaCoef + ((size_t)idx * 2 + 1) * (E.nP + 1), p, E.nP);
            }
        } else {
            const double *b = E.gc + (size_t)idx * RAFTX_GC_N;
            for (int i = 0; i < RAFTX_GC_N; i++) o[i] = b[i];
            if (ed) o[RAFTX_GC_S] = E.capFrac[idx] * L;
        }
    }
    __syncthreads();
    double *out = (kind == 0 ? E.gm_out : (kind == 1 ? E.gs_out : E.gc_out)) + row0 * W;
    const int npiece = nrows * W / 2;
    for (int i = t; i < npiece; i += GE_T) {
        const int r = (2 * i) / W, f = (2 * i) % W;
        *reinterpret_cast<double2 *>(out + 2 * (size_t)i) = make_double2(tile[r * 17 + f], tile[r * 17 + f + 1]);
    }
}
static inline void launch_expand(const ExpandArgs &E, hipStream_t st) {
    const unsigned nbM = (unsigned)(((size_t)E.n * E.nM + GE_T - 1) / GE_T), nbS = (unsigned)(((size_t)E.n * E.nSt + GE_T - 1) / GE_T),
                   nbC = (unsigned)(((size_t)E.n * E.nCap + GE_T - 1) / GE_T);
    if (nbM + nbS + nbC) hipLaunchKernelGGL(k_geom_expand, dim3(nbM + nbS + nbC), dim3(GE_T), 0, st, E, nbM, nbS);
}
```

raft_amd/csrc/raftx_hip.hip:

```cpp

#include <hip/hip_runtime.h>
#include <rccl/rccl.h>
#include <dlfcn.h>

#include <algorithm>
#include <cmath>
#include <cstdint>
#include <cstdio>
#include <cstdlib>
#include <cstring>
#include <chrono>
#include <map>
#include <functional>
#include <mutex>
#include <type_traits>
#include <thread>
#include <unordered_map>
#include <vector>

#include "../../include/raftx.h"
#include "../../include/raftx_modal.h"
#include "../../include/raftx_current.h"
#include "../../include/raftx_channels.h"
#include "../../include/raftx_qtfgen.h"
// ... 395 lines not shown
            for (int ih = 0; ih < nHead; ih++) {
                const cplx *x = Xi + (((size_t)p * nHead + ih) * 6) * nw + i;
                const cplx x0 = x[0], x1 = x[(size_t)nw], x2 = x[(size_t)2 * nw], x3 = x[(size_t)3 * nw], x4 = x[(size_t)4 * nw],
                           x5 = x[(size_t)5 * nw];
                const double yr = ws * (l0 * x0.re + l1 * x1.re + l2 * x2.re + l3 * x3.re + l4 * x4.re + l5 * x5.re);
                const double yi = ws * (l0 * x0.im + l1 * x1.im + l2 * x2.im + l3 * x3.im + l4 * x4.im + l5 * x5.im);
                a2 += yr * yr + yi * yi;
            }
            acc += a2;
            if (psd) psd[((size_t)p * nChan + ch) * nw + i] = 0.5 * a2 * inv_dw;
        }
        for (int o = 32; o > 0; o >>= 1) acc += __shfl_xor(acc, o, 64);
        __syncthreads();
        if (lane == 0) part[wv] = acc;
        __syncthreads();
        if (threadIdx.x == 0) {
            double a = 0.0;
            for (int q = 0; q < (int)(blockDim.x >> 6); q++) a += part[q];
            sd[(size_t)p * nChan + ch] = sqrt(0.5 * a);
        }
    }
}

__global__ void __launch_bounds__(256) k_bem_excitation(DevTables T, int nHB, const double *__restrict__ heads,
                                                        const cplx *__restrict__ X, const double *__restrict__ hadj,
                                                        const double *__restrict__ xy, const cplx *__restrict__ Fadd,
                                                        cplx *__restrict__ F) {
    const int ih = blockIdx.x % T.nHead, p = blockIdx.x / T.nHead;
    const int d = p / T.nCase, ic = p % T.nCase;
    const double beta = T.beta[(size_t)ic * T.nHead + ih];
    double bdeg = fmod(beta * (180.0 / M_PI) - (hadj ? hadj[d] : 0.0), 360.0);
    if (bdeg < 0.0) bdeg += 360.0;
    int i1 = nHB - 1, i2 = 0;
    double f2;
    if (bdeg <= heads[0]) {
        const double hlast = heads[nHB - 1] - 360.0;
        f2 = (bdeg - hlast) / (heads[0] - hlast);
    } else if (bdeg >= heads[nHB - 1]) {
        const double hfirst = heads[0] + 360.0;
        f2 = (bdeg - heads[nHB - 1]) / (hfirst - heads[nHB - 1]);
    } else {
        f2 = 0.0;
        for (int i = 0; i < nHB - 1; i++)
            if (heads[i + 1] > bdeg) {
                i1 = i;
                i2 = i + 1;
                f2 = (bdeg - heads[i]) / (heads[i + 1] - heads[i]);
                break;
            }
    }
    const double f1 = 1.0 - f2, sb = sin(beta), cb = cos(beta);
    const double xr = xy ? xy[2 * d] : 0.0, yr = xy ? xy[2 * d + 1] : 0.0;
    const cplx *X1 = X + ((size_t)d * nHB + i1) * 6 * T.nw, *X2 = X + ((size_t)d * nHB + i2) * 6 * T.nw;
    const size_t base = ((size_t)p * T.nHead + ih) * 6 * T.nw;
    for (int i = threadIdx.x; i < T.nw; i += blockDim.x) {
        cplx xp[6];
#pragma unroll
        for (int j = 0; j < 6; j++) {
            const cplx a = X1[(size_t)j * T.nw + i], b = X2[(size_t)j * T.nw + i];
            xp[j] = {a.re * f1 + b.re * f2, a.im * f1 + b.im * f2};
        }
        cplx g[6];
        g[0] = {xp[0].re * cb - xp[1].re * sb, xp[0].im * cb - xp[1].im * sb};
        g[1] = {xp[0].re * sb + xp[1].re * cb, xp[0].im * sb + xp[1].im * cb};
        g[2] = xp[2];
        g[3] = {xp[3].re * cb - xp[4].re * sb, xp[3].im * cb - xp[4].im * sb};
        g[4] = {xp[3].re * sb + xp[4].re * cb, xp[3].im * sb + xp[4].im * cb};
        g[5] = xp[5];
        double ps, pc;
        sincos(-(T.k[i] * (xr * cos(beta) + yr * sin(beta))), &ps, &pc);
        const double z = T.zeta[((size_t)ic * T.nHead + ih) * T.nw + i];
#pragma unroll
        for (int j = 0; j < 6; j++) {
            const double gr = g[j].re * z, gi = g[j].im * z;
            cplx o = {gr * pc - gi * ps, gr * ps + gi * pc};
            if (Fadd) {
                const cplx a = Fadd[base + (size_t)j * T.nw + i];
                o.re += a.re;
                o.im += a.im;
            }
            F[base + (size_t)j * T.nw + i] = o;
        }
    }
}

__global__ void __launch_bounds__(256) k_channel_stats_poly(int nCase, int nHead, int nw, int nChan, double inv_dw,
                                                            const double *__restrict__ w, const cplx *__restrict__ Xi,
                                                            const double *__restrict__ L, const cplx *__restrict__ Gw,
                                                            double *__restrict__ sd, double *__restrict__ psd) {
    __shared__ double part[4];
    const int p = blockIdx.x, d = p / nCase;
    const int lane = threadIdx.x & 63, wv = threadIdx.x >> 6;
    for (int ch = 0; ch < nChan; ch++) {
        const double *row = L + ((size_t)d * nChan + ch) * 18;
        const cplx *g = Gw ? Gw + ((size_t)d * nChan + ch) * 6 * nw : nullptr;
        double acc = 0.0;
        for (int i = threadIdx.x; i < nw; i += blockDim.x) {
            const double wi = w[i], w2 = wi * wi;
            double a2 = 0.0;
            for (int ih = 0; ih < nHead; ih++) {
                const cplx *x = Xi + (((size_t)p * nHead + ih) * 6) * nw + i;
                double yr = 0.0, yi = 0.0;
#pragma unroll
                for (int j = 0; j < 6; j++) {
                    const cplx xj = x[(size_t)j * nw];
                    double cr = row[j] - w2 * row[12 + j], ci = wi * row[6 + j];
                    if (g) {
                        const cplx gj = g[(size_t)j * nw + i];
                        cr += gj.re;
                        ci += gj.im;
                    }
                    yr += cr * xj.re - ci * xj.im;
                    yi += cr * xj.im + ci * xj.re;
                }
                a2 += yr * yr + yi * yi;
            }
            acc += a2;
            if (psd) psd[((size_t)p * nChan + ch) * nw + i] = 0.5 * a2 * inv_dw;
        }
        for (int o = 32; o > 0; o >>= 1) acc += __shfl_xor(acc, o, 64);
        __syncthreads();
        if (lane == 0) part[wv] = acc;
        __syncthreads();
        if (threadIdx.x == 0) {
            double a = 0.0;
            for (int q = 0; q < (int)(blockDim.x >> 6); q++) a += part[q];
            sd[(size_t)p * nChan + ch] = sqrt(0.5 * a);
        }
    }
}

__global__ void __launch_bounds__(256) k_response_stats(int nDof, int nResp, int nw, double inv_dw, const double *__restrict__ w,
                                                        const cplx *__restrict__ Xi, const double *__restrict__ L,
                                                        const cplx *__restrict__ Gw, double *__restrict__ sd, double *__restrict__ psd) {
    __shared__ double part[4];
    const int ch = blockIdx.x;
    const int lane = threadIdx.x & 63, wv = threadIdx.x >> 6;
    const double *row = L + (size_t)ch * 3 * nDof;
    const cplx *g = Gw ? Gw + (size_t)ch * nDof * nw : nullptr;
    double acc = 0.0;
    for (int i = threadIdx.x; i < nw; i += blockDim.x) {
        const double wi = w[i], w2 = wi * wi;
        double a2 = 0.0;
        for (int ih = 0; ih < nResp; ih++) {
            const cplx *x = Xi + ((size_t)ih * nDof) * nw + i;
            double yr = 0.0, yi = 0.0;
            for (int j = 0; j < nDof; j++) {
                const cplx xj = x[(size_t)j * nw];
                double cr = row[j] - w2 * row[2 * nDof + j], ci = wi * row[nDof + j];
                if (g) {
                    const cplx gj = g[(size_t)j * nw + i];
                    cr += gj.re;
                    ci += gj.im;
                }
                yr += cr * xj.re - ci * xj.im;
                yi += cr * xj.im + ci * xj.re;
            }
            a2 += yr * yr + yi * yi;
        }
        acc += a2;
        if (psd) psd[(size_t)ch * nw + i] = 0.5 * a2 * inv_dw;
    }
    for (int o = 32; o > 0; o >>= 1) acc += __shfl_xor(acc, o, 64);
    if (lane == 0) part[wv] = acc;
    __syncthreads();
    if (threadIdx.x == 0) {
        double a = 0.0;
        for (int q = 0; q < (int)(blockDim.x >> 6); q++) a += part[q];
        sd[ch] = sqrt(0.5 * a);
    }
}

#define RAFTX_NSLOT RAFTX_SWEEP_SLOTS
struct DevPool {
    std::multimap<size_t, void *> free_;
    std::unordered_map<void *, size_t> size_;
    static size_t round_up(size_t b) {
        if (b < 256) b = 256;
        if (b <= ((size_t)1 << 20)) {
            size_t p = 256;
            while (p < b) p <<= 1;
            return p;
        }
        return (b + ((size_t)1 << 20) - 1) & ~(((size_t)1 << 20) - 1);
    }
    hipError_t get(size_t bytes, void **out) {
        const size_t cap = round_up(bytes);
        auto it = free_.lower_bound(cap);
        if (it != free_.end() && it->first <= cap + cap / 2 + ((size_t)1 << 20)) {
            *out = it->second;
            free_.erase(it);
            return hipSuccess;
        }
        static const bool dbg = getenv("RAFTX_POOL_DEBUG") != nullptr;
        const auto t0 = std::chrono::steady_clock::now();
        hipError_t e = hipMalloc(out, cap);
        if (dbg)
            fprintf(stderr, "[raftx pool] miss: hipMalloc(%zu) %.3f ms (%zu blocks free)\n", cap,
                    std::chrono::duration<double, std::milli>(std::chrono::steady_clock::now() - t0).count(), free_.size());
        if (e != hipSuccess) {
            (void)hipGetLastError();
            trim();
            e = hipMalloc(out, cap);
        }
        if (e == hipSuccess) size_[*out] = cap;
        return e;
    }
    void put(void *p) {
        if (!p) return;
        auto it = size_.find(p);
        if (it == size_.end()) {
            (void)hipFree(p);
            return;
        }
        free_.emplace(it->second, p);
    }
    void trim() {
        for (auto &kv : free_) {
            size_.erase(kv.second);
            (void)hipFree(kv.second);
        }
        free_.clear();
    }
};

template <typename Tp>
struct Pinned {
    Tp *p = nullptr;
    size_t cap = 0;
    hipError_t reserve(size_t n) {
        if (p && cap >= n) return hipSuccess;
        release();
        void *q = nullptr;
        const hipError_t e = hipHostMalloc(&q, (n ? n : 1) * sizeof(Tp), hipHostMallocDefault);
        if (e != hipSuccess) return e;
        p = reinterpret_cast<Tp *>(q);
        cap = n;
        return hipSuccess;
    }
    void release() {
        if (p) (void)hipHostFree(p);
        p = nullptr;
        cap = 0;
    }
};

struct BuildJob {
    GeomArgs A;
    std::vector<void *> tmp;
    int nDesign = 0, nw = 0;
    int64_t maxMem = 0, maxSta = 0;
    size_t nStrips = 0, nRows = 0;
    int maxS = 0;
    double *M0d = nullptr, *C0d = nullptr;
    const double *B0d = nullptr, *MBwd = nullptr;
    bool active = false;
    hipStream_t reduce_stream = nullptr;
    bool gen_deferred = false;
    size_t gen_lds = 0;
};

struct CaseSet {
    std::vector<double> key;
    DevTables T;
    std::vector<void *> allocs;
    int users = 0;
    unsigned long long stamp = 0;
};

struct FixedRecord {
    bool valid = false;
    double rho = 0, g = 0;
    int trim = 0, haveK = 0;
    double *rec = nullptr;
    int *irec = nullptr;
    int users = 0;
    unsigned long long stamp = 0;
    hipEvent_t ev = nullptr;
    hipStream_t stream = nullptr;
};
struct VariantProg {
    int nM = 0, nSt = 0, nCap = 0, nP = 0;
    int nFix = 0;
    int *fixDesc = nullptr, *fixIdx = nullptr;
    FixedRecord recs[RAFTX_NSLOT + 1];
    unsigned long long rec_clock = 0;
    bool has_caps = false;
    double *gm = nullptr, *gs = nullptr, *gc = nullptr;
    int *stMember = nullptr, *capMember = nullptr;
    double *stFrac = nullptr, *fillFrac = nullptr, *capFrac = nullptr;
    double *endCoef = nullptr, *headCS = nullptr, *diaCoef = nullptr;
    int *endEdit = nullptr, *diaEdit = nullptr;
    std::vector<int64_t> hS, hC;
    std::vector<void *> allocs;
    int cachedN = -1;
    std::vector<int64_t> memberOff, stationOff, capOff;
};
struct VariantSrc {
    const VariantProg *prog;
    const double *params;
    const FixedRecord *rec = nullptr;
};

static void expand_args(const VariantProg &P, int n, double *gm_out, double *gs_out, double *gc_out, ExpandArgs &E) {
    E.n = n; E.nM = P.nM; E.nSt = P.nSt; E.nCap = P.nCap; E.nP = P.nP;
    E.gm = P.gm; E.gs = P.gs; E.gc = P.gc;
    E.stMember = P.stMember; E.capMember = P.capMember;
    E.stFrac = P.stFrac; E.fillFrac = P.fillFrac; E.capFrac = P.capFrac;
    E.endCoef = P.endCoef; E.headCS = P.headCS; E.diaCoef = P.diaCoef;
    E.endEdit = P.endEdit; E.diaEdit = P.diaEdit;
    E.gm_out = gm_out; E.gs_out = gs_out; E.gc_out = gc_out;
}

struct DenseResident {
    int nSet = 0, n = 0, nw = 0, freq_mask = 0;
    double *w = nullptr, *M = nullptr, *B = nullptr, *C = nullptr;
    std::vector<void *> allocs;
};
struct QtfResident {
    bool valid = false;
    int nDesign = 0;
    std::vector<int64_t> off;
    int64_t *dOff = nullptr;
    double *strips = nullptr, *members = nullptr, *kay = nullptr;
    std::vector<void *> allocs;
    int64_t total(int j) const { return off[(size_t)j * (nDesign + 1) + nDesign]; }
};
struct raftx_ctx {
    int device;
    hipStream_t stream;
    bool owns_stream;
    hipEvent_t ev0, ev1;
    hipEvent_t evUp, evTot, evG0, evG1, evG2, evG3, evS0, evS1, evDone;
    hipEvent_t evZ;
    hipEvent_t evMem, evRed;
    hipStream_t sAux;
    BuildJob job;
    Pinned<long long> pin;
    Pinned<double> pinRes;
    Pinned<double> pinModal;
    Pinned<double> pinCur;
    Pinned<double> pinChan;
    Pinned<double> pinMoorT;
    hipEvent_t evMoor = nullptr;
    hipStream_t sCopy, sPrep, sD2H, sGen;
    hipStream_t sSlab[2] = {nullptr, nullptr};
    hipStream_t sD2Hhigh = nullptr;
    hipEvent_t evEpoch = nullptr;
    CaseSet csets[RAFTX_NSLOT + 1];
    unsigned long long cset_clock = 0;
    char err[512];
    DevTables T;
    DevPool pool;
    std::vector<void *> design_allocs, case_allocs, result_allocs;
    cplx *rXi, *rFw, *rZ, *rFe;
    double *rB, *rXl;
    cplx *flexXl0;
    size_t flexXl0_n, flexXl0_cap;
    unsigned long long *rXlSlots;
    size_t rXl_n;
    unsigned *kpCtr = nullptr;
    unsigned kpNext = 0;
    int nCU = 0;
    int last_flags = -1, last_minb = 0, last_rc = 0;
    cplx *rQtf;
    size_t rQtf_n;
    int rQtf_sets, rQtf_nw2;
    cplx *rXl0, *rXlOut;
    size_t rXlio_n;
    bool have_xl0, want_xlout;
    int *rNi, *rFl;
    size_t r_npair, r_nx, r_nz;
    int r_mask;
    int r_last_mask = 0;
    bool r_fe;
    int maxS;
    std::vector<int> hS;
    int *pairList;
    size_t pairList_n;
    DenseResident dense;
    int *identList = nullptr;
    size_t identList_n = 0;
    std::vector<hipEvent_t> evSlab;
    hipEvent_t evFork = nullptr, evJoin = nullptr;
    unsigned long long *dbg;
    double last_ms;
    bool have_designs, have_cases;
    int nw_designs;
    cplx *rKay;
    size_t rKay_n;
    int rKay_sets, rKay_nw2;
    bool kay_ready;
    cplx *bemF;
    size_t bemF_n;
    bool bem_ready;
    int g_n;
    size_t g_nStrips, g_nRows;
    double *g_abi, *g_A, *g_Ch, *g_Wh, *g_props, *g_Ms, *g_Cs, *g_Ws;
    bool last_gen_fused = false;
    cplx *g_cm;
    void *comm;
    int comm_rank, comm_world;
    int *commFlag = nullptr;
    std::vector<raftx_ctx *> workers[RAFTX_NSLOT];
    struct SweepSlot *slots;
    VariantProg vprog;
    struct {
        int nLine = 0, nP = 0;
        double *base = nullptr, *coef = nullptr;
        int *edit = nullptr;
    } mprog;
    QtfResident qt;
};
struct DevOffsets {
    const int64_t *memberOff, *stationOff, *capOff;
};
struct SeaStates { int nCase, nHead, nw; const double *w, *k; double depth, rho, g; const double *zeta, *beta; };
struct BuildSource {
    const int64_t *memberOff, *stationOff, *capOff;
    const double *members, *stations, *caps;
    const double *pose, *M0, *B0, *C0, *MBw, *Fz_moor, *k;
    double rho, g;
    int nw, add_mask;
    DevOffsets dOff{nullptr, nullptr, nullptr};
    const double *k_dev = nullptr;
    VariantSrc var{nullptr, nullptr};
};
struct SweepSlot {
    bool busy = false;
    int cset = -1;
    int frec = -1;
    bool prepared = false;
    int nIter = 0;
    double tol = 0, XiStart = 0, dw = 0;
    std::vector<raftx_ctx *> blk;
    std::vector<int> bnd;
    int nCase = 0, nHead = 0, nw = 0;
    double *sd = nullptr;
    int32_t *niter = nullptr, *flags = nullptr;
    raftx_c128 *Xi = nullptr;
    int64_t *stripOffsets = nullptr;
    std::vector<void *> allocs;
    hipEvent_t evXi = nullptr;
    BuildSource p1;
    size_t next_p1 = 0;
    std::chrono::steady_clock::time_point t0;
    double since() const { return std::chrono::duration<double, std::milli>(std::chrono::steady_clock::now() - t0).count(); }
    double tl[4] = {0, 0, 0, 0};
    double span[2] = {0, 0};
    size_t nSlabEv = 0;
    bool slab = false;
    std::vector<double> tlb;
    struct {
        bool on = false;
        const double *dM = nullptr, *dC = nullptr;
        double *fn = nullptr, *modes = nullptr, *props = nullptr;
        int32_t *flags = nullptr;
        hipEvent_t evUp = nullptr;
    } modal;
    struct {
        bool on = false;
        int nCur = 0;
        double shearExp = 0;
        std::vector<double> host;
        const double *par = nullptr, *Zref = nullptr;
        double *D = nullptr;
        hipEvent_t evUp = nullptr;
    } current;
    struct {
        bool on = false;
        int nChan = 0, nL = 0, nG = 0;
        const double *L = nullptr;
        const cplx *Gw = nullptr;
        double *out = nullptr;
        hipEvent_t evUp = nullptr;
    } channels;
    struct {
        bool on = false, add = false;
        int nLine = 0;
        const double *C = nullptr, *Lr = nullptr;
        Pinned<double> pin;
        double *C_out = nullptr, *F_out = nullptr, *T_out = nullptr, *Tstd_out = nullptr;
        int32_t *flags_out = nullptr;
        hipEvent_t evUp = nullptr;
    } mooring;
};

#define MAX_NW 2048
#define HIPCHK(ctx, call)                                                                              \
    do {                                                                                               \
        hipError_t e_ = (call);                                                                        \
        if (e_ != hipSuccess) {                                                                        \
            snprintf((ctx)->err, sizeof((ctx)->err), "%s failed: %s (%s:%d)", #call, hipGetErrorString(e_), \
                     __FILE__, __LINE__);                                                              \
            return -2;                                                                                 \
        }                                                                                              \
    } while (0)
#define FAIL(ctx, ...)                                        \
    do {                                                      \
        snprintf((ctx)->err, sizeof((ctx)->err), __VA_ARGS__); \
        return -1;                                            \
    } while (0)

extern "C" int raftx_version(void) { return RAFTX_VERSION; }
extern "C" int raftx_is_device(void) { return 1; }
extern "C" int raftx_device_count(void) {
    int n = 0;
    if (hipGetDeviceCount(&n) != hipSuccess) {
        (void)hipGetLastError();
        return 0;
    }
    return n;
}

extern "C" int raftx_ctx_create(int device_id, raftx_ctx **out) {
    if (!out) return -1;
    *out = nullptr;
    int ndev = 0;
    if (hipGetDeviceCount(&ndev) != hipSuccess || ndev <= 0) return -3;
    if (device_id < 0 || device_id >= ndev) return -4;
    if (hipSetDevice(device_id) != hipSuccess) return -5;
    raftx_ctx *c = new raftx_ctx();
    memset(&c->T, 0, sizeof(c->T));
    c->device = device_id;
    c->err[0] = 0;
    c->maxS = 0;
    c->pairList = nullptr;
    c->pairList_n = 0;
    c->dbg = nullptr;
    c->last_ms = 0.0;
    c->have_designs = c->have_cases = false;
    c->nw_designs = 0;
    c->g_n = 0;
    c->bemF = nullptr;
    c->bemF_n = 0;
    c->bem_ready = false;
    c->rKay = nullptr;
    c->rKay_n = 0;
    c->rKay_sets = c->rKay_nw2 = 0;
    c->kay_ready = false;
    c->rXi = c->rFw = c->rZ = c->rFe = nullptr;
    c->rB = c->rXl = nullptr;
    c->rXlSlots = nullptr;
    c->flexXl0 = nullptr;
    c->flexXl0_n = c->flexXl0_cap = 0;
    c->rXl_n = 0;
    c->rQtf = nullptr;
    c->rQtf_n = 0;
    c->rQtf_sets = c->rQtf_nw2 = 0;
    c->rXl0 = c->rXlOut = nullptr;
    c->rXlio_n = 0;
    c->have_xl0 = c->want_xlout = false;
    c->rNi = c->rFl = nullptr;
    c->r_npair = c->r_nx = c->r_nz = 0;
    c->r_mask = 0;
    c->r_fe = false;
    c->comm = nullptr;
    c->comm_rank = 0;
    c->comm_world = 1;
    c->owns_stream = true;
    c->slots = new SweepSlot[RAFTX_NSLOT];
    c->sCopy = c->sPrep = c->sD2H = c->sGen = nullptr;
    bool ok = hipStreamCreateWithFlags(&c->stream, hipStreamNonBlocking) == hipSuccess;
    c->sAux = nullptr;
    for (hipEvent_t *e : {&c->evZ, &c->ev0, &c->ev1, &c->evUp, &c->evTot, &c->evG0, &c->evG1, &c->evG2, &c->evG3, &c->evS0,
                          &c->evS1, &c->evDone, &c->evMem, &c->evRed})
        ok = ok && hipEventCreate(e) == hipSuccess;
    if (!ok) {
        delete[] c->slots;
        delete c;
        return -6;
    }
    *out = c;
    return 0;
}

static void free_list(raftx_ctx *c, std::vector<void *> &v) {
    for (void *p : v) c->pool.put(p);
    v.clear();
}

static void variant_release(raftx_ctx *c) {
    for (FixedRecord &R : c->vprog.recs)
        if (R.ev) (void)hipEventDestroy(R.ev);
    free_list(c, c->vprog.allocs);
    c->vprog = VariantProg();
}
static void mooring_program_release(raftx_ctx *c) {
    if (c->mprog.base) (void)hipFree(c->mprog.base);
    if (c->mprog.coef) (void)hipFree(c->mprog.coef);
    if (c->mprog.edit) (void)hipFree(c->mprog.edit);
    c->mprog.base = c->mprog.coef = nullptr;
    c->mprog.edit = nullptr;
    c->mprog.nLine = c->mprog.nP = 0;
}
extern "C" void raftx_ctx_destroy(raftx_ctx *c) {
    if (!c) return;
#ifdef GEOM_PHASE_TIMING
    if (c->owns_stream && c->slots) {
        unsigned long long ph[10] = {0};
        (void)hipDeviceSynchronize();
        if (hipMemcpyFromSymbol(ph, HIP_SYMBOL(geom_phase_cycles), sizeof(ph)) == hipSuccess && ph[0]) {
            unsigned long long tot = 0;
            for (int i = 0; i < 7; i++) tot += ph[i];
            fprintf(stderr, "[k_geom_design phases, %% of wave time] counts %.1f | generate %.1f | abi out %.1f | runs %.1f | ds out %.1f | g-vectors %.1f | morison+matrices %.1f\n",
                    100.0 * ph[0] / tot, 100.0 * ph[1] / tot, 100.0 * ph[2] / tot, 100.0 * ph[3] / tot, 100.0 * ph[4] / tot,
                    100.0 * ph[5] / tot, 100.0 * ph[6] / tot);
        }
    }
#endif
    (void)raftx_comm_destroy(c);
    if (c->owns_stream) {
        (void)hipSetDevice(c->device);
        (void)hipDeviceSynchronize();
    }
    for (int sl = 0; sl < RAFTX_NSLOT; sl++) {
        for (raftx_ctx *w : c->workers[sl]) raftx_ctx_destroy(w);
        c->workers[sl].clear();
    }
    (void)hipSetDevice(c->device);
    (void)hipStreamSynchronize(c->stream);
    free_list(c, c->design_allocs);
    free_list(c, c->case_allocs);
    free_list(c, c->result_allocs);
    free_list(c, c->qt.allocs);
    for (CaseSet &cs : c->csets) free_list(c, cs.allocs);
    c->pool.trim();
    if (c->rXl) (void)hipFree(c->rXl);
    if (c->rXlSlots) (void)hipFree(c->rXlSlots);
    if (c->kpCtr) (void)hipFree(c->kpCtr);
    if (c->flexXl0) (void)hipFree(c->flexXl0);
    if (c->rXl0) (void)hipFree(c->rXl0);
    if (c->rXlOut) (void)hipFree(c->rXlOut);
    if (c->rQtf) (void)hipFree(c->rQtf);
    if (c->bemF) (void)hipFree(c->bemF);
    if (c->rKay) (void)hipFree(c->rKay);
    if (c->pairList) (void)hipFree(c->pairList);
    free_list(c, c->dense.allocs);
    variant_release(c);
    mooring_program_release(c);
    if (c->identList) (void)hipFree(c->identList);
    for (hipEvent_t e : c->evSlab) (void)hipEventDestroy(e);
    if (c->evFork) (void)hipEventDestroy(c->evFork);
    if (c->evJoin) (void)hipEventDestroy(c->evJoin);
    free_list(c, c->job.tmp);
    for (int sl = 0; sl < RAFTX_NSLOT; sl++) {
        free_list(c, c->slots[sl].allocs);
        if (c->slots[sl].evXi) (void)hipEventDestroy(c->slots[sl].evXi);
        if (c->slots[sl].modal.evUp) (void)hipEventDestroy(c->slots[sl].modal.evUp);
        if (c->slots[sl].current.evUp) (void)hipEventDestroy(c->slots[sl].current.evUp);
        if (c->slots[sl].channels.evUp) (void)hipEventDestroy(c->slots[sl].channels.evUp);
        if (c->slots[sl].mooring.evUp) (void)hipEventDestroy(c->slots[sl].mooring.evUp);
        c->slots[sl].mooring.pin.release();
    }
    delete[] c->slots;
    c->pool.trim();
    c->pin.release();
    c->pinRes.release();
    c->pinModal.release();
    c->pinCur.release();
    c->pinChan.release();
    c->pinMoorT.release();
    if (c->evMoor) (void)hipEventDestroy(c->evMoor);
    for (hipEvent_t e : {c->evZ, c->ev0, c->ev1, c->evUp, c->evTot, c->evG0, c->evG1, c->evG2, c->evG3, c->evS0, c->evS1, c->evDone,
                         c->evMem, c->evRed})
        (void)hipEventDestroy(e);
    if (c->sAux) (void)hipStreamDestroy(c->sAux);
    if (c->evEpoch) (void)hipEventDestroy(c->evEpoch);
    for (hipStream_t st : {c->sCopy, c->sPrep, c->sD2H, c->sGen, c->sD2Hhigh, c->sSlab[0], c->sSlab[1]})
        if (st) (void)hipStreamDestroy(st);
    if (c->owns_stream) (void)hipStreamDestroy(c->stream);
    delete c;
}

extern "C" int raftx_host_alloc(raftx_ctx *c, size_t bytes, void **out) {
    if (!c || !out) return -1;
    *out = nullptr;
    HIPCHK(c, hipSetDevice(c->device));
    HIPCHK(c, hipHostMalloc(out, bytes ? bytes : 1, hipHostMallocDefault));
    return 0;
}
extern "C" int raftx_host_free(raftx_ctx *c, void *ptr) {
    if (!c) return -1;
    if (ptr) HIPCHK(c, hipHostFree(ptr));
    return 0;
}

extern "C" int raftx_device_locality(int device, char *pci_bus_id, int len, int *numa_node) {
    if (numa_node) *numa_node = -1;
    char id[64] = {0};
    if (hipDeviceGetPCIBusId(id, (int)sizeof(id), device) != hipSuccess) return -2;
    if (pci_bus_id && len > 0) snprintf(pci_bus_id, (size_t)len, "%s", id);
    for (char *p = id; *p; p++) *p = (char)tolower(*p);
    char path[160];
    snprintf(path, sizeof(path), "/sys/bus/pci/devices/%s/numa_node", id);
    if (FILE *f = fopen(path, "r")) {
        int node = -1;
        if (fscanf(f, "%d", &node) == 1 && numa_node) *numa_node = node;
        fclose(f);
    }
    return 0;
}

extern "C" const char *raftx_last_error(raftx_ctx *c) { return c ? c->err : "null ctx"; }
extern "C" double raftx_last_kernel_ms(raftx_ctx *c) { return c ? c->last_ms : 0.0; }

template <typename Tp>
static int pool_alloc(raftx_ctx *c, std::vector<void *> &bag, size_t n, Tp **out) {
    *out = nullptr;
    void *p = nullptr;
    HIPCHK(c, c->pool.get((n ? n : 1) * sizeof(Tp), &p));
    bag.push_back(p);
    *out = reinterpret_cast<Tp *>(p);
    return 0;
}
template <typename Tp, typename Dp>
static int upload_on(raftx_ctx *c, hipStream_t st, std::vector<void *> &bag, const Tp *host, size_t n, Dp *dev) {
    *dev = nullptr;
    if (!host || n == 0) return 0;
    Tp *p = nullptr;
    if (pool_alloc(c, bag, n, &p)) return -2;
    HIPCHK(c, hipMemcpyAsync(p, host, n * sizeof(Tp), hipMemcpyHostToDevice, st));
    *dev = p;
    return 0;
}
template <typename Tp, typename Dp>
static int upload(raftx_ctx *c, std::vector<void *> &bag, const Tp *host, size_t n, Dp *dev) { return upload_on(c, c->stream, bag, host, n, dev); }

extern "C" int raftx_upload_designs(raftx_ctx *c, int nDesign, const int64_t *stripOffsets, const double *strips,
                                    int nStripFields, const double *M0, const double *B0, const double *C0, int nw,
                                    const double *MBw, const int64_t *cmOffsets, const raftx_c128 *CmMCF) {
    RangeScope range_("raftx_upload_designs: run detection + H2D");
    if (!c) return -1;
    if (nStripFields != NF) FAIL(c, "nStripFields=%d, expected %d", nStripFields, NF);
    if (nDesign < 0 || !stripOffsets || !M0 || !B0 || !C0) FAIL(c, "upload_designs: bad arguments");
    HIPCHK(c, hipSetDevice(c->device));
    HIPCHK(c, hipStreamSynchronize(c->stream));
    free_list(c, c->design_allocs);
    c->have_designs = false;
    c->bem_ready = false;
    int maxS = 0;
    c->hS.assign((size_t)nDesign, 0);
    for (int d = 0; d < nDesign; d++) {
        int64_t S = stripOffsets[d + 1] - stripOffsets[d];
        if (S < 0) FAIL(c, "strip offsets not monotone at design %d", d);
        if (S > maxS) maxS = (int)S;
        c->hS[(size_t)d] = (int)S;
    }
    std::vector<double> dsv((size_t)stripOffsets[nDesign] * DS_N, 0.0);
    std::vector<int> dsf((size_t)stripOffsets[nDesign], 0);
    for (int d = 0; d < nDesign; d++)
        derive_design_tables(strips, stripOffsets[d], stripOffsets[d + 1], dsv.data(), dsf.data());
    DevTables &T = c->T;
    T.nDesign = nDesign;
    int rc = 0;
    rc |= upload(c, c->design_allocs, stripOffsets, (size_t)nDesign + 1, &T.off);
    rc |= upload(c, c->design_allocs, dsv.data(), dsv.size(), &T.ds);
    rc |= upload(c, c->design_allocs, dsf.data(), dsf.size(), &T.dsi);
    rc |= upload(c, c->design_allocs, M0, (size_t)nDesign * 36, &T.M0);
    rc |= upload(c, c->design_allocs, B0, (size_t)nDesign * 36, &T.B0);
    rc |= upload(c, c->design_allocs, C0, (size_t)nDesign * 36, &T.C0);
    rc |= upload(c, c->design_allocs, MBw, MBw ? (size_t)nDesign * 72 * nw : 0, &T.MBw);
    T.cmoff = nullptr;
    T.cm = nullptr;
    if (cmOffsets && CmMCF) {
        rc |= upload(c, c->design_allocs, cmOffsets, (size_t)nDesign + 1, &T.cmoff);
        rc |= upload(c, c->design_allocs, reinterpret_cast<const cplx *>(CmMCF), (size_t)cmOffsets[nDesign] * 2 * nw,
                     &T.cm);
    }
    if (rc) return -2;
    HIPCHK(c, hipStreamSynchronize(c->stream));
    c->maxS = maxS;
    c->nw_designs = nw;
    c->have_designs = true;
    c->g_n = 0;
    return 0;
}

constexpr size_t PIN_TOT = 0;
constexpr size_t PIN_ERR = 3;
constexpr size_t PIN_OFF = 8;
static int check_source(raftx_ctx *c, const BuildSource &B, int nDesign, const char *who, const char *bad) {
    const bool var = B.var.prog != nullptr;
    if (nDesign < 0 || !B.memberOff || (!B.members && !var) || !B.stationOff || (!B.stations && !var) || !B.M0 || !B.B0 || !B.C0)
        FAIL(c, "%s: %s", who, bad);
    if (!var && (B.capOff == nullptr) != (B.caps == nullptr)) FAIL(c, "%s: capOff and caps must be given together", who);
    return 0;
}
static void launch_scan(hipStream_t st, const GeomArgs &A) {
    static const int scan_t = getenv("RAFTX_SCAN_T") ? atoi(getenv("RAFTX_SCAN_T")) : 1024;
    if (scan_t == 256) hipLaunchKernelGGL(k_geom_scan_t<256>, dim3(1), dim3(256), 0, st, A);
    else hipLaunchKernelGGL(k_geom_scan_t<1024>, dim3(1), dim3(1024), 0, st, A);
}
struct Slice { int lo; int64_t m0, m1, s0, s1, c0, c1; };
static int slice_of(raftx_ctx *c, const BuildSource &B, int lo, int nDesign, Slice &L) {
    if (lo < 0 || nDesign < 0) FAIL(c, "build_designs: bad arguments");
    const int64_t m0 = B.memberOff[lo], m1 = B.memberOff[lo + nDesign];
    if (m1 < m0 || m0 < 0) FAIL(c, "build_designs: member offsets not monotone");
    const int64_t s0 = B.stationOff[m0], s1 = B.stationOff[m1];
    if (s1 < s0 || s0 < 0) FAIL(c, "build_designs: station offsets not monotone");
    const int64_t c0 = B.capOff ? B.capOff[m0] : 0, c1 = B.capOff ? B.capOff[m1] : 0;
    if (c1 < c0 || c0 < 0) FAIL(c, "build_designs: cap offsets not monotone");
    L = {lo, m0, m1, s0, s1, c0, c1};
    return 0;
}
static int upload_descriptors(raftx_ctx *c, hipStream_t sCopy, const BuildSource &B, const Slice &L, ExpandArgs &E) {
    BuildJob &J = c->job;
    GeomArgs &A = J.A;
    std::vector<void *> &tmp = J.tmp, &keep = c->design_allocs;
    const size_t lo = (size_t)L.lo, nDesign = (size_t)A.nDesign, nMember = (size_t)A.nMember, nw = (size_t)B.nw;
    const size_t nSta = (size_t)(L.s1 - L.s0), nCap = (size_t)(L.c1 - L.c0);
    int rc = 0;
    if (B.dOff.memberOff) {
        A.memberOff = B.dOff.memberOff + lo;
        A.stationOff = B.dOff.stationOff + L.m0;
        A.capOff = B.capOff ? B.dOff.capOff + L.m0 : nullptr;
    } else {
        rc |= upload_on(c, sCopy, tmp, B.memberOff + lo, nDesign + 1, &A.memberOff);
        rc |= upload_on(c, sCopy, tmp, B.stationOff + L.m0, nMember + 1, &A.stationOff);
        if (B.capOff) rc |= upload_on(c, sCopy, tmp, B.capOff + L.m0, nMember + 1, &A.capOff);
    }
    memset(&E, 0, sizeof(E));
    if (const VariantProg *P = B.var.prog) {
        if (nMember != nDesign * P->nM || nSta != nDesign * P->nSt || nCap != nDesign * P->nCap)
            FAIL(c, "build_designs: offsets do not describe %d variants of the program's base unit", A.nDesign);
        double *gm = nullptr, *gs = nullptr, *gc = nullptr;
        if (pool_alloc(c, tmp, nMember * RAFTX_GM_N, &gm) || pool_alloc(c, tmp, nSta * RAFTX_GS_N, &gs) ||
            pool_alloc(c, tmp, nCap * RAFTX_GC_N, &gc))
            return -2;
        rc |= upload_on(c, sCopy, tmp, B.var.params + lo * P->nP, nDesign * P->nP, &E.params);
        expand_args(*P, A.nDesign, gm, gs, gc, E);
        A.gm = gm; A.gs = gs; A.caps = B.capOff ? gc : nullptr;
    } else {
        rc |= upload_on(c, sCopy, tmp, B.members + (size_t)L.m0 * RAFTX_GM_N, nMember * RAFTX_GM_N, &A.gm);
        rc |= upload_on(c, sCopy, tmp, B.stations + (size_t)L.s0 * RAFTX_GS_N, nSta * RAFTX_GS_N, &A.gs);
    }
    rc |= upload_on(c, sCopy, tmp, B.pose ? B.pose + lo * 6 : nullptr, nDesign * 6, &A.pose);
    if (B.capOff && !B.var.prog) {
        if (nCap) rc |= upload_on(c, sCopy, tmp, B.caps + (size_t)L.c0 * RAFTX_GC_N, nCap * RAFTX_GC_N, &A.caps);
        else rc |= pool_alloc(c, tmp, RAFTX_GC_N, &A.caps);
    }
    if (B.k_dev) A.k = B.k_dev;
    else rc |= upload_on(c, sCopy, keep, B.k, nw, &A.k);
    rc |= upload_on(c, sCopy, keep, B.M0 + lo * 36, nDesign * 36, &J.M0d);
    rc |= upload_on(c, sCopy, keep, B.C0 + lo * 36, nDesign * 36, &J.C0d);
    rc |= upload_on(c, sCopy, keep, B.B0 + lo * 36, nDesign * 36, &J.B0d);
    rc |= upload_on(c, sCopy, keep, B.MBw ? B.MBw + lo * 72 * nw : nullptr, nDesign * 72 * nw, &J.MBwd);
    if (B.Fz_moor) rc |= upload_on(c, sCopy, tmp, B.Fz_moor + lo, nDesign, &A.Fz);
    if (rc) return -2;
    A.M0 = J.M0d; A.C0 = J.C0d;
    return 0;
}
static int alloc_member_scratch(raftx_ctx *c) {
    GeomArgs &A = c->job.A;
    std::vector<void *> &tmp = c->job.tmp, &keep = c->design_allocs;
    const size_t nDesign = (size_t)A.nDesign, nMember = (size_t)A.nMember;
    if (pool_alloc(c, tmp, nMember, &A.cnt) || pool_alloc(c, tmp, nMember, &A.cntm) || pool_alloc(c, tmp, nMember * MP_N, &A.mpose) ||
        pool_alloc(c, tmp, nMember * MH_N, &A.mhyd) || pool_alloc(c, tmp, nMember * MI_N, &A.minert) || pool_alloc(c, tmp, 4, &A.err) ||
        pool_alloc(c, tmp, nMember, &A.mdesign_w) || pool_alloc(c, tmp, nDesign, &A.drho) || pool_alloc(c, tmp, 5, &A.tot) ||
        pool_alloc(c, keep, nDesign + 1, &A.off) || pool_alloc(c, keep, nDesign + 1, &A.cmoff) || pool_alloc(c, keep, nDesign * 36, &A.Ch) ||
        pool_alloc(c, keep, nDesign * 6, &A.Wh) || pool_alloc(c, keep, nDesign * 36, &A.Ms) || pool_alloc(c, keep, nDesign * 36, &A.Cs) ||
        pool_alloc(c, keep, nDesign * 6, &A.Ws) || pool_alloc(c, keep, nDesign * RAFTX_SP_N, &A.props))
        return -2;
    A.mdesign = A.mdesign_w;
    return 0;
}
static int design_bounds(raftx_ctx *c, const BuildSource &B, const Slice &L) {
    BuildJob &J = c->job;
    J.maxMem = J.maxSta = 0;
    for (int d = 0; d < J.nDesign; d++) {
        const int64_t a = B.memberOff[L.lo + d], b = B.memberOff[L.lo + d + 1];
        if (b < a || a < L.m0 || b > L.m1) FAIL(c, "member offsets not monotone at design %d", L.lo + d);
        if (B.stationOff[b] < B.stationOff[a]) FAIL(c, "build_designs: station offsets not monotone");
        J.maxMem = std::max(J.maxMem, b - a);
        J.maxSta = std::max(J.maxSta, B.stationOff[b] - B.stationOff[a]);
    }
    return 0;
}
static int enqueue_member_pass(raftx_ctx *c, hipStream_t sPrep) {
    BuildJob &J = c->job;
    GeomArgs &A = J.A;
    const int64_t nDesign = J.nDesign, nMember = A.nMember;
    hipLaunchKernelGGL(k_geom_zero, dim3((unsigned)(nDesign / 256 + 1)), dim3(256), 0, sPrep, A);
    HIPCHK(c, hipEventRecord(c->evZ, sPrep));
    HIPCHK(c, hipEventRecord(c->evG2, sPrep));
    A.mgrid = 0;
    if (nMember > 0) {
        A.mgrid = (nDesign >= 64 && J.maxMem * nDesign <= nMember + nMember / 4) ? (int)J.maxMem : 0;
        const int64_t nThread = A.mgrid > 0 ? (int64_t)A.mgrid * nDesign : nMember;
        hipLaunchKernelGGL(k_geom_member, dim3((unsigned)((nThread + 127) / 128)), dim3(128), 0, sPrep, A);
        if (A.add_mask & RAFTX_TRIM_BALLAST) {
            hipLaunchKernelGGL(k_geom_trim, dim3((unsigned)(nDesign / 128 + 1)), dim3(128), 0, sPrep, A);
            hipLaunchKernelGGL(k_geom_reinertia, dim3((unsigned)((nThread + 127) / 128)), dim3(128), 0, sPrep, A);
        }
    }
    return 0;
}
static int enqueue_scan_reduce(raftx_ctx *c, hipStream_t sPrep) {
    BuildJob &J = c->job;
    const bool side = J.nDesign > 0 && sPrep != c->stream;
    auto scan = [&]() -> int {
        if (J.nDesign > 0) launch_scan(sPrep, J.A);
        HIPCHK(c, hipEventRecord(c->evG3, sPrep));
        HIPCHK(c, hipEventRecord(c->evTot, sPrep));
        return 0;
    };
    J.reduce_stream = nullptr;
    hipStream_t sRed = sPrep;
    if (side) {
        HIPCHK(c, hipEventRecord(c->evMem, sPrep));
        if (scan()) return -2;
        if (!c->sAux) HIPCHK(c, hipStreamCreateWithFlags(&c->sAux, hipStreamNonBlocking));
        sRed = c->sAux;
        HIPCHK(c, hipStreamWaitEvent(sRed, c->evMem, 0));
    }
    if (J.nDesign > 0) hipLaunchKernelGGL(k_geom_reduce, dim3((unsigned)(((size_t)J.nDesign * 3 + 63) / 64)), dim3(64), 0, sRed, J.A);
    if (!side) return scan();
    HIPCHK(c, hipEventRecord(c->evRed, sRed));
    J.reduce_stream = sRed;
    return 0;
}
static int build_phase1(raftx_ctx *c, hipStream_t sCopy, hipStream_t sPrep, const BuildSource &B, int lo, int nDesign) {
    RangeScope range_("build phase 1: descriptor H2D, member pass, scans (enqueue)");
    BuildJob &J = c->job;
    Slice L;
    if (int rc = slice_of(c, B, lo, nDesign, L)) return rc;
    HIPCHK(c, hipSetDevice(c->device));
    free_list(c, c->design_allocs);
    free_list(c, J.tmp);
    c->have_designs = false; c->bem_ready = false; c->g_n = 0;
    HIPCHK(c, c->pin.reserve(PIN_OFF + (size_t)nDesign + 1));
    GeomArgs &A = J.A;
    memset(&A, 0, sizeof(A));
    A.nDesign = nDesign; A.nMember = L.m1 - L.m0;
    A.rho = B.rho; A.g = B.g; A.nw = B.nw; A.add_mask = B.add_mask;
    A.mbase = L.m0; A.sbase = L.s0; A.cbase = L.c0;
    A.hostOut = c->pin.p;
    memset(c->pin.p, 0, (PIN_OFF + 1) * sizeof(long long));
    J.nDesign = nDesign; J.nw = B.nw;
    ExpandArgs E;
    if (int rc = upload_descriptors(c, sCopy, B, L, E)) return rc;
    HIPCHK(c, hipEventRecord(c->evUp, sCopy));
    HIPCHK(c, hipStreamWaitEvent(sPrep, c->evUp, 0));
    if (B.var.prog && nDesign > 0) {
        launch_expand(E, sPrep);
        if (const FixedRecord *R = B.var.rec) {
            if (R->stream != sPrep) HIPCHK(c, hipStreamWaitEvent(sPrep, R->ev, 0));
            A.fixRec = R->rec; A.fixInt = R->irec; A.fixIdx = B.var.prog->fixIdx; A.fixNM = B.var.prog->nM;
        }
    }
    if (int rc = alloc_member_scratch(c)) return rc;
    if (int rc = design_bounds(c, B, L)) return rc;
    if (int rc = enqueue_member_pass(c, sPrep)) return rc;
    if (int rc = enqueue_scan_reduce(c, sPrep)) return rc;
    J.active = true;
    return 0;
}

constexpr int GEN_CROSSING = 1;
constexpr int GEN_MAY_DEFER = 2;
constexpr int GEN_PIPELINED = 4;
static void launch_design(raftx_ctx *c, hipStream_t st) {
    hipLaunchKernelGGL(k_geom_design, dim3((unsigned)c->job.nDesign), dim3(GD_T), c->job.gen_lds, st, c->job.A);
}
static int wait_totals(raftx_ctx *c, int64_t *stripOffsets) {
    BuildJob &J = c->job;
    for (;;) {
        const hipError_t q = hipEventQuery(c->evTot);
        if (q == hipSuccess) break;
        if (q != hipErrorNotReady) HIPCHK(c, q);
    }
    HIPCHK(c, hipGetLastError());
    const int *bad = reinterpret_cast<const int *>(c->pin.p + PIN_ERR);
    if (bad[3] > 0) FAIL(c, "member %d: needs 2..%d stations, dlsMax > 0 and length > 0", bad[3] - 1, GEOM_MAX_STATIONS);
    if (bad[3] < 0) FAIL(c, "build_designs: member %d is MacCamy-Fuchs but no wave numbers were given", -bad[3] - 1);
    if (bad[0]) FAIL(c, "member %d: cap/bulkhead layout not supported (the reference raises here too)", bad[0] - 1);
    if (bad[1]) FAIL(c, "design %d: ballast trim needs some ballast volume", bad[1] - 1);
    J.nStrips = (size_t)c->pin.p[PIN_TOT]; J.nRows = (size_t)c->pin.p[PIN_TOT + 1]; J.maxS = (int)c->pin.p[PIN_TOT + 2];
    const long long *off = c->pin.p + PIN_OFF;
    if (stripOffsets) memcpy(stripOffsets, off, ((size_t)J.nDesign + 1) * sizeof(int64_t));
    c->hS.resize((size_t)J.nDesign);
    for (int d = 0; d < J.nDesign; d++) c->hS[(size_t)d] = (int)(off[d + 1] - off[d]);
    return 0;
}
static int enqueue_generation(raftx_ctx *c, hipStream_t sGen, int kind) {
    BuildJob &J = c->job;
    GeomArgs &A = J.A;
    const int nDesign = J.nDesign, nw = J.nw;
    const size_t nRows = J.nRows;
    const char *fg_ = getenv("RAFTX_FUSED_GEN");
    const bool fused_gen = fg_ && atoi(fg_);
    const bool defer = (kind & GEN_MAY_DEFER) && fused_gen && nDesign > 0 && nRows == 0;
    J.gen_deferred = false;
    const size_t gd_lds = geom_design_lds(J.maxS, (int)J.maxSta, (int)J.maxMem);
    if (gd_lds > 160 * 1024)
        FAIL(c, "build_designs: designs of up to %d submerged strips, %d stations and %d members need %zu B of LDS in k_geom_design, 160 KiB available",
             J.maxS, (int)J.maxSta, (int)J.maxMem, gd_lds);
    if (gd_lds > 64 * 1024)
        HIPCHK(c, hipFuncSetAttribute(reinterpret_cast<const void *>(k_geom_design), hipFuncAttributeMaxDynamicSharedMemorySize, (int)gd_lds));
    J.gen_lds = gd_lds;
    if (!sGen || defer) sGen = c->stream;
    HIPCHK(c, hipStreamWaitEvent(sGen, c->evTot, 0));
    HIPCHK(c, hipEventRecord(c->evG0, sGen));
    if (defer) {
        HIPCHK(c, hipStreamWaitEvent(c->stream, c->evTot, 0));
        if (J.reduce_stream) HIPCHK(c, hipStreamWaitEvent(c->stream, c->evRed, 0));
        J.gen_deferred = true;
    } else if (nDesign > 0) {
        static const bool addup_kernel = getenv("RAFTX_ADDUP_KERNEL") && atoi(getenv("RAFTX_ADDUP_KERNEL"));
        A.addup_in_design = ((kind & GEN_PIPELINED) && !addup_kernel && nRows == 0 && !A.abi) ? 1 : 0;
        if (A.addup_in_design && J.reduce_stream) HIPCHK(c, hipStreamWaitEvent(sGen, c->evRed, 0));
        launch_design(c, sGen);
        if (!A.addup_in_design) {
            if (J.reduce_stream) HIPCHK(c, hipStreamWaitEvent(sGen, c->evRed, 0));
            hipLaunchKernelGGL(k_geom_addup, dim3((unsigned)(((size_t)nDesign * 36 + 255) / 256)), dim3(256), 0, sGen, A);
        }
    }
    if (nRows > 0)
        hipLaunchKernelGGL(k_geom_mcf, dim3((unsigned)nRows, (unsigned)((nw + 63) / 64)), dim3(64), 0, sGen, A, (int64_t)nRows);
    HIPCHK(c, hipEventRecord(c->evG1, sGen));
    if (sGen != c->stream) HIPCHK(c, hipStreamWaitEvent(c->stream, c->evG1, 0));
    return 0;
}
static void publish_tables(raftx_ctx *c) {
    const BuildJob &J = c->job;
    const GeomArgs &A = J.A;
    DevTables &T = c->T;
    T.nDesign = J.nDesign; T.off = A.off; T.ds = A.ds; T.dsi = A.dsi;
    T.M0 = J.M0d; T.C0 = J.C0d; T.B0 = J.B0d; T.MBw = J.MBwd;
    T.cmoff = J.nRows ? A.cmoff : nullptr; T.cm = J.nRows ? A.cm : nullptr;
    c->maxS = J.maxS; c->nw_designs = J.nw; c->have_designs = true;
    c->g_n = J.nDesign; c->g_nStrips = J.nStrips; c->g_nRows = J.nRows;
    c->g_abi = A.abi; c->g_cm = A.cm;
    c->g_A = A.A; c->g_Ch = A.Ch; c->g_Wh = A.Wh; c->g_props = A.props;
    c->g_Ms = A.Ms; c->g_Cs = A.Cs; c->g_Ws = A.Ws;
}
static int build_phase2(raftx_ctx *c, int64_t *stripOffsets, hipStream_t sGen = nullptr, int kind = 0) {
    RangeScope range_("build phase 2: wait for totals, strip tables + statics (enqueue)");
    BuildJob &J = c->job;
    GeomArgs &A = J.A;
    if (!J.active) FAIL(c, "build_designs: phase 2 without phase 1");
    if (int rc = wait_totals(c, stripOffsets)) return rc;
    std::vector<void *> &keep = c->design_allocs;
    A.abi = nullptr;
    if ((!kind && pool_alloc(c, keep, J.nStrips * NF, &A.abi)) || pool_alloc(c, keep, J.nStrips * DS_N, &A.ds) ||
        pool_alloc(c, keep, J.nStrips, &A.dsi) || pool_alloc(c, keep, J.nRows * 3, &A.mcfaux) ||
        pool_alloc(c, keep, J.nRows * 2 * (size_t)J.nw, &A.cm) || pool_alloc(c, keep, (size_t)J.nDesign * 36, &A.A))
        return -2;
    if (int rc = enqueue_generation(c, sGen, kind)) return rc;
    publish_tables(c);
    return 0;
}
static void build_abandon(raftx_ctx *c) {
    free_list(c, c->job.tmp);
    c->job.active = false;
}
static int build_retire(raftx_ctx *c, double *ms_out) {
    float a = 0.f, b = 0.f;
    if (c->job.active) {
        HIPCHK(c, hipEventElapsedTime(&a, c->evG2, c->evG3));
        HIPCHK(c, hipEventElapsedTime(&b, c->evG0, c->evG1));
    }
    if (ms_out) *ms_out = (double)a + (double)b;
    build_abandon(c);
    return 0;
}

extern "C" int raftx_build_designs(raftx_ctx *c, int nDesign, const int64_t *memberOff, const double *members,
                                   const int64_t *stationOff, const double *stations, const int64_t *capOff,
                                   const double *caps, const double *pose, double rho, double g, int nw, const double *k,
                                   int add_mask, const double *M0, const double *B0, const double *C0, const double *MBw,
                                   const double *Fz_moor, int64_t *stripOffsets) {
    if (!c) return -1;
    if (!stripOffsets) FAIL(c, "build_designs: bad arguments");
    HIPCHK(c, hipSetDevice(c->device));
    HIPCHK(c, hipStreamSynchronize(c->stream));
    const BuildSource src{memberOff, stationOff, capOff, members, stations, caps, pose, M0, B0, C0, MBw, Fz_moor, k, rho, g, nw, add_mask};
    int rc = check_source(c, src, nDesign, "build_designs", "bad arguments");
    if (!rc && (nw < 1 || nw > MAX_NW)) {
        snprintf(c->err, sizeof(c->err), "build_designs: nw=%d outside 1..%d", nw, MAX_NW);
        rc = -1;
    }
    if (!rc) rc = build_phase1(c, c->stream, c->stream, src, 0, nDesign);
    if (!rc) rc = build_phase2(c, stripOffsets);
    const hipError_t e = hipStreamSynchronize(c->stream);
    if (rc) {
        build_abandon(c);
        c->have_designs = false;
        return rc;
    }
    HIPCHK(c, e);
    HIPCHK(c, hipGetLastError());
    double ms = 0.0;
    if (build_retire(c, &ms)) return -2;
    c->last_ms = ms;
    return 0;
}

extern "C" int raftx_fetch_strips(raftx_ctx *c, double *strips, raftx_c128 *cm) {
    if (!c) return -1;
    if (!c->g_n || !c->have_designs) FAIL(c, "fetch_strips: no raftx_build_designs call on this ctx");
    HIPCHK(c, hipSetDevice(c->device));
    if (strips && c->g_nStrips && !c->g_abi)
        FAIL(c, "fetch_strips: the tables of this batch were generated by a sweep crossing, which keeps no ABI copy of the strip records");
    if (strips && c->g_nStrips)
        HIPCHK(c, hipMemcpyAsync(strips, c->g_abi, c->g_nStrips * NF * sizeof(double), hipMemcpyDeviceToHost, c->stream));
    if (cm && c->g_nRows)
        HIPCHK(c, hipMemcpyAsync(cm, c->g_cm, c->g_nRows * 2 * (size_t)c->nw_designs * sizeof(cplx), hipMemcpyDeviceToHost, c->stream));
    HIPCHK(c, hipStreamSynchronize(c->stream));
    return 0;
}

extern "C" int raftx_fetch_statics(raftx_ctx *c, double *A_morison, double *C_hydro, double *W_hydro, double *M_struc,
                                   double *C_struc, double *W_struc, double *props) {
    if (!c) return -1;
    if (!c->g_n || !c->have_designs) FAIL(c, "fetch_statics: no raftx_build_designs call on this ctx");
    HIPCHK(c, hipSetDevice(c->device));
    const size_t n = (size_t)c->g_n;
    if (A_morison) HIPCHK(c, hipMemcpyAsync(A_morison, c->g_A, n * 36 * sizeof(double), hipMemcpyDeviceToHost, c->stream));
    if (C_hydro) HIPCHK(c, hipMemcpyAsync(C_hydro, c->g_Ch, n * 36 * sizeof(double), hipMemcpyDeviceToHost, c->stream));
    if (W_hydro) HIPCHK(c, hipMemcpyAsync(W_hydro, c->g_Wh, n * 6 * sizeof(double), hipMemcpyDeviceToHost, c->stream));
    if (props) HIPCHK(c, hipMemcpyAsync(props, c->g_props, n * RAFTX_SP_N * sizeof(double), hipMemcpyDeviceToHost, c->stream));
    if (M_struc) HIPCHK(c, hipMemcpyAsync(M_struc, c->g_Ms, n * 36 * sizeof(double), hipMemcpyDeviceToHost, c->stream));
    if (C_struc) HIPCHK(c, hipMemcpyAsync(C_struc, c->g_Cs, n * 36 * sizeof(double), hipMemcpyDeviceToHost, c->stream));
    if (W_struc) HIPCHK(c, hipMemcpyAsync(W_struc, c->g_Ws, n * 6 * sizeof(double), hipMemcpyDeviceToHost, c->stream));
    HIPCHK(c, hipStreamSynchronize(c->stream));
    return 0;
}

static int upload_case_tables(raftx_ctx *c, hipStream_t st, std::vector<void *> &bag, DevTables &T, const SeaStates &sea) {
    const int nCase = sea.nCase, nHead = sea.nHead, nw = sea.nw;
    const double *k = sea.k, depth = sea.depth;
    std::vector<double> csh(nw), cch(nw);
    for (int i = 0; i < nw; i++) {
        double kh = k[i] * depth;
        if (k[i] == 0.0 || kh > 89.4) {
            csh[i] = cch[i] = 1.0;
        } else {
            double e2kh = exp(-2.0 * kh);
            csh[i] = 1.0 / (-expm1(-2.0 * kh));
            cch[i] = 1.0 / (1.0 + e2kh);
        }
    }
    T.nCase = nCase; T.nHead = nHead; T.nw = nw;
    T.depth = depth; T.rho = sea.rho; T.g = sea.g;
    int rc = 0;
    rc |= upload_on(c, st, bag, sea.w, (size_t)nw, &T.w);
    rc |= upload_on(c, st, bag, k, (size_t)nw, &T.k);
    rc |= upload_on(c, st, bag, csh.data(), (size_t)nw, &T.csh);
    rc |= upload_on(c, st, bag, cch.data(), (size_t)nw, &T.cch);
    rc |= upload_on(c, st, bag, sea.zeta, (size_t)nCase * nHead * nw, &T.zeta);
    rc |= upload_on(c, st, bag, sea.beta, (size_t)nCase * nHead, &T.beta);
    const hipError_t e = hipStreamSynchronize(st);
    if (rc) return -2;
    HIPCHK(c, e);
    return 0;
}

extern "C" int raftx_upload_cases(raftx_ctx *c, int nCase, int nHead, int nw, const double *w, const double *k,
                                  double depth, double rho, double g, const double *zeta, const double *beta) {
    RangeScope range_("raftx_upload_cases: H2D");
    if (!c) return -1;
    if (nCase < 0 || nHead < 1 || nw < 1 || !w || !k || !zeta || !beta) FAIL(c, "upload_cases: bad arguments");
    if (nw > MAX_NW) FAIL(c, "nw=%d exceeds the %d bins per workgroup supported by this build", nw, MAX_NW);
    HIPCHK(c, hipSetDevice(c->device));
    HIPCHK(c, hipStreamSynchronize(c->stream));
    free_list(c, c->case_allocs);
    c->have_cases = false;
    c->bem_ready = false;
    if (int rc = upload_case_tables(c, c->stream, c->case_allocs, c->T, SeaStates{nCase, nHead, nw, w, k, depth, rho, g, zeta, beta})) return rc;
    c->have_cases = true;
    return 0;
}

#define LDS_LIMIT (160 * 1024)

struct Shape {
    int nb, threads;
};
#ifndef RAFTX_MINB128
#define RAFTX_MINB128 2
#endif
#define SHAPES(X) X(1, 64, 1) X(2, 64, 1) X(4, 64, 1) X(2, 128, RAFTX_MINB128) X(1, 256, 2) X(2, 256, 2) X(2, 512, 1) X(3, 512, 1) X(4, 512, 1)
static bool shape_ok(Shape sh, int nw) {
#define X(NB_, MT_, MB_) if (sh.nb == NB_ && sh.threads == MT_) return (long)NB_ * MT_ >= nw;
    SHAPES(X)
#undef X
    return false;
}
static Shape pick_shape(int nw) {
    static const char *env = getenv("RAFTX_SHAPE");
    if (env) {
        Shape sh = {0, 0};
        if (sscanf(env, "%d,%d", &sh.nb, &sh.threads) == 2 && shape_ok(sh, nw)) return sh;
    }
    if (nw <= 64) return {1, 64};
    if (nw <= 128) return {2, 64};
    if (nw <= 256) return {2, 128};
    if (nw <= 512) return {2, 256};
    int nb = (nw + 511) / 512;
    return {nb < 2 ? 2 : nb, 512};
}

static int prep_lds(raftx_ctx *c, const void *kernel, size_t bytes) {
    if (bytes > LDS_LIMIT)
        FAIL(c, "a design has %d submerged strips / nw=%d: %zu B of LDS needed, 160 KiB available", c->maxS, c->T.nw, bytes);
    if (bytes > 64 * 1024)
        HIPCHK(c, hipFuncSetAttribute(kernel, hipFuncAttributeMaxDynamicSharedMemorySize, (int)bytes));
    return 0;
}
#define NO_KERNEL(c, sh) FAIL(c, "no kernel for shape %d x %d", (sh).nb, (sh).threads)

enum Drain { DRAIN_STREAM, DRAIN_DEVICE };
template <typename Tp>
static int grow_device(raftx_ctx *c, Tp **ptr, size_t *have_n, size_t want_n, Drain drain = DRAIN_STREAM) {
    HIPCHK(c, drain == DRAIN_DEVICE ? hipDeviceSynchronize() : hipStreamSynchronize(c->stream));
    if (*ptr) (void)hipFree(*ptr);
    *ptr = nullptr;
    *have_n = 0;
    void *p_ = nullptr;
    HIPCHK(c, hipMalloc(&p_, (want_n ? want_n : 1) * sizeof(Tp)));
    *ptr = reinterpret_cast<Tp *>(p_);
    *have_n = want_n;
    return 0;
}
template <typename Tp>
static int zeroed_once(raftx_ctx *c, Tp **ptr, size_t n) {
    if (*ptr) return 0;
    void *p_ = nullptr;
    HIPCHK(c, hipMalloc(&p_, n * sizeof(Tp)));
    *ptr = reinterpret_cast<Tp *>(p_);
    HIPCHK(c, hipMemsetAsync(*ptr, 0, n * sizeof(Tp), c->stream));
    return 0;
}

static int check_ready(raftx_ctx *c) {
    if (!c) return -1;
    if (!c->have_designs) FAIL(c, "no designs uploaded");
    if (!c->have_cases) FAIL(c, "no cases uploaded");
    if ((c->T.MBw || c->T.cm) && c->nw_designs != c->T.nw)
        FAIL(c, "nw mismatch between designs (%d) and cases (%d)", c->nw_designs, c->T.nw);
    return 0;
}

struct Scratch {
    raftx_ctx *c;
    std::vector<void *> bag;
    explicit Scratch(raftx_ctx *c_) : c(c_) {}
    ~Scratch() {
        (void)hipStreamSynchronize(c->stream);
        free_list(c, bag);
    }
    template <typename Tp>
    Tp *alloc(size_t n) {
        void *p = nullptr;
        if (n == 0) return nullptr;
        if (c->pool.get(n * sizeof(Tp), &p) != hipSuccess) return nullptr;
        bag.push_back(p);
        return reinterpret_cast<Tp *>(p);
    }
};

#define D2H(c, dst, src, bytes) HIPCHK(c, hipMemcpyAsync(dst, src, bytes, hipMemcpyDeviceToHost, (c)->stream))
#define H2D(c, dst, src, bytes) HIPCHK(c, hipMemcpyAsync(dst, src, bytes, hipMemcpyHostToDevice, (c)->stream))

static int finish_timed(raftx_ctx *c) {
    HIPCHK(c, hipEventRecord(c->ev1, c->stream));
    HIPCHK(c, hipGetLastError());
    HIPCHK(c, hipStreamSynchronize(c->stream));
    float ms = 0.f;
    HIPCHK(c, hipEventElapsedTime(&ms, c->ev0, c->ev1));
    c->last_ms = ms;
    return 0;
}

typedef void (*excitation_fn)(DevTables, cplx *);
static excitation_fn excitation_kernel(Shape sh) {
#define X(NB_, MT_, MB_) if (sh.nb == NB_ && sh.threads == MT_) return k_excitation<NB_, MT_, MB_>;
    SHAPES(X)
#undef X
    return nullptr;
}
extern "C" int raftx_excitation(raftx_ctx *c, raftx_c128 *F_iner) {
    if (check_ready(c)) return -1;
    if (!F_iner) FAIL(c, "excitation: F_iner is NULL");
    HIPCHK(c, hipSetDevice(c->device));
    const DevTables &T = c->T;
    size_t npair = (size_t)T.nDesign * T.nCase;
    size_t n = npair * T.nHead * 6 * T.nw;
    Scratch sc(c);
    cplx *dF = sc.alloc<cplx>(n);
    if (n && !dF) FAIL(c, "excitation: device allocation failed");
    const Shape sh = pick_shape(T.nw);
    HIPCHK(c, hipEventRecord(c->ev0, c->stream));
    if (npair) {
// ... 3107 lines not shown
```

Measured before the change: 688.0 million.

## Fuse variant expansion into geometry kernels instead of materializing expanded tables

Variant designs are no longer expanded by a separate k_geom_expand kernel into full member/station/cap tables by default. The base tables plus per-design parameters go to the geometry kernels, which rebuild the edited fields on the fly through a row-accessor template (GeomRowsProg). This removes an expand launch, the scratch allocations and the global-memory round trip of the expanded rows. In exchange, affine evaluations are repeated inside the member and design kernels and the templates add register pressure. The old path is kept when RAFTX_FUSED_GEN is set.

```diff
diff --git a/raft_amd/csrc/raftx_geom.h b/raft_amd/csrc/raftx_geom.h
--- a/raft_amd/csrc/raftx_geom.h
+++ b/raft_amd/csrc/raftx_geom.h
@@ -89,6 +89,15 @@
     }
 }
 
+struct VariantView {
+    int nM, nSt, nCap, nP;
+    const double *params;
+    const double *gm, *gs, *gc;
+    const int *stMember, *capMember;
+    const double *stFrac, *fillFrac, *capFrac;
+    const double *endCoef, *headCS, *diaCoef;
+    const int *endEdit, *diaEdit;
+};
 struct GeomArgs {
     int nDesign;
     int64_t nMember;
@@ -128,12 +137,114 @@
     const double *fixRec;
     const int *fixInt, *fixIdx;
     int fixNM;
+    VariantView prog;
     __device__ int64_t mo(int d) const { return memberOff[d] - mbase; }
     __device__ int64_t so(int64_t m) const { return stationOff[m] - sbase; }
     __device__ int64_t co(int64_t m) const { return capOff[m] - cbase; }
 };
 
 #define GEOM_NOFMA _Pragma("clang fp contract(off)")
+
+__device__ __forceinline__ double affine_eval(const double *coef, const double *p, int nP) {
+    GEOM_NOFMA
+    double v = coef[0];
+    for (int q = 0; q < nP; q++) v = v + coef[1 + q] * p[q];
+    return v;
+}
+__device__ __forceinline__ void variant_ends(const VariantView &V, int m, const double *p, double (&e)[6], double &L) {
+    GEOM_NOFMA
+    for (int i = 0; i < 6; i++) e[i] = affine_eval(V.endCoef + ((size_t)m * 6 + i) * (V.nP + 1), p, V.nP);
+    const double dx = e[3] - e[0], dy = e[4] - e[1], dz = e[5] - e[2];
+    L = sqrt((dx * dx + dy * dy) + dz * dz);
+}
+template <class Row>
+__device__ __forceinline__ void variant_member_edit(const VariantView &V, int m, const double (&e)[6], double L, Row &o) {
+    GEOM_NOFMA
+    const double c = V.headCS[2 * m], s = V.headCS[2 * m + 1];
+    o[RAFTX_GM_RA + 0] = c * e[0] + (-s) * e[1];
+    o[RAFTX_GM_RA + 1] = s * e[0] + c * e[1];
+    o[RAFTX_GM_RA + 2] = e[2];
+    o[RAFTX_GM_RB + 0] = c * e[3] + (-s) * e[4];
+    o[RAFTX_GM_RB + 1] = s * e[3] + c * e[4];
+    o[RAFTX_GM_RB + 2] = e[5];
+    o[RAFTX_GM_L] = L;
+}
+__device__ __forceinline__ double variant_station_S(const VariantView &V, int idx, double L) {
+    GEOM_NOFMA
+    return V.stFrac[idx] * L;
+}
+__device__ __forceinline__ double variant_station_LFILL(const VariantView &V, int idx, double L) {
+    GEOM_NOFMA
+    return V.fillFrac[idx] * L;
+}
+__device__ __forceinline__ double variant_station_D(const VariantView &V, int idx, int c, const double *p) {
+    return affine_eval(V.diaCoef + ((size_t)idx * 2 + c) * (V.nP + 1), p, V.nP);
+}
+template <class Row>
+__device__ __forceinline__ void variant_station_edit(const VariantView &V, int idx, bool ed, double L, const double *p, Row &o) {
+    if (ed) {
+        o[RAFTX_GS_S] = variant_station_S(V, idx, L);
+        o[RAFTX_GS_LFILL] = variant_station_LFILL(V, idx, L);
+    }
+    if (V.diaEdit[idx]) {
+        o[RAFTX_GS_D] = variant_station_D(V, idx, 0, p);
+        o[RAFTX_GS_D + 1] = variant_station_D(V, idx, 1, p);
+    }
+}
+__device__ __forceinline__ double variant_cap_S(const VariantView &V, int idx, double L) {
+    GEOM_NOFMA
+    return V.capFrac[idx] * L;
+}
+
+__device__ __forceinline__ void geom_load_row(const double *gs, int i, double (&r)[RAFTX_GS_N]) {
+    const double2 *p = reinterpret_cast<const double2 *>(gs + (size_t)i * RAFTX_GS_N);
+#pragma unroll
+    for (int k = 0; k < RAFTX_GS_N / 2; k++) {
+        const double2 v = p[k];
+        r[2 * k] = v.x;
+        r[2 * k + 1] = v.y;
+    }
+}
+static_assert(RAFTX_GM_N == RAFTX_GS_N, "member and station rows are loaded alike");
+struct GeomRowsPlain {
+    const double *gmrow, *gs, *gc;
+    __device__ __forceinline__ void member(double (&gm)[RAFTX_GM_N]) const { geom_load_row(gmrow, 0, gm); }
+    __device__ __forceinline__ double mcol(int f) const { return gmrow[f]; }
+    __device__ __forceinline__ void station(int i, double (&r)[RAFTX_GS_N]) const { geom_load_row(gs, i, r); }
+    __device__ __forceinline__ double st(int j, int f) const { return gs[(size_t)j * RAFTX_GS_N + f]; }
+    __device__ __forceinline__ double cap(int i, int f) const { return gc[(size_t)i * RAFTX_GC_N + f]; }
+};
+struct GeomRowsProg {
+    const VariantView V;
+    const double *p;
+    int bm, s0, c0;
+    bool ed;
+    double e[6], L;
+    __device__ __forceinline__ GeomRowsProg(const VariantView &V_, int bm_, int s0_, int c0_, int d)
+        : V(V_), p(V_.params + (size_t)d * V_.nP), bm(bm_), s0(s0_), c0(c0_), ed(V_.endEdit[bm_] != 0), e{0, 0, 0, 0, 0, 0}, L(0.0) {
+        if (ed) variant_ends(V, bm, p, e, L);
+    }
+    __device__ __forceinline__ void member(double (&gm)[RAFTX_GM_N]) const {
+        geom_load_row(V.gm, bm, gm);
+        if (ed) variant_member_edit(V, bm, e, L, gm);
+    }
+    __device__ __forceinline__ double mcol(int f) const { return V.gm[(size_t)bm * RAFTX_GM_N + f]; }
+    __device__ __forceinline__ void station(int i, double (&r)[RAFTX_GS_N]) const {
+        geom_load_row(V.gs, s0 + i, r);
+        variant_station_edit(V, s0 + i, ed, L, p, r);
+    }
+    __device__ __forceinline__ double st(int j, int f) const {
+        const int idx = s0 + j;
+        if (f == RAFTX_GS_S && ed) return variant_station_S(V, idx, L);
+        if (f == RAFTX_GS_LFILL && ed) return variant_station_LFILL(V, idx, L);
+        if ((f == RAFTX_GS_D || f == RAFTX_GS_D + 1) && V.diaEdit[idx]) return variant_station_D(V, idx, f - RAFTX_GS_D, p);
+        return V.gs[(size_t)idx * RAFTX_GS_N + f];
+    }
+    __device__ __forceinline__ double cap(int i, int f) const {
+        if (f == RAFTX_GC_S && ed) return variant_cap_S(V, c0 + i, L);
+        return V.gc[(size_t)(c0 + i) * RAFTX_GC_N + f];
+    }
+};
 
 __device__ inline double geom_interp(double x, const double *gs, int n, int f) {
     GEOM_NOFMA
@@ -316,22 +427,26 @@
     }
     Iv[0] = y2 + z2; Iv[1] = x2 + z2; Iv[2] = x2 + y2;
 }
-__device__ inline double geom_interp_inner(double x, const double *gs, int n, int c) {
-    GEOM_NOFMA
-#define DIN_(j) (gs[(size_t)(j) * RAFTX_GS_N + RAFTX_GS_D + c] - 2 * gs[(size_t)(j) * RAFTX_GS_N + RAFTX_GS_T])
-    if (x < gs[RAFTX_GS_S]) return DIN_(0);
-    if (x > gs[(size_t)(n - 1) * RAFTX_GS_N + RAFTX_GS_S]) return DIN_(n - 1);
+template <class Rows>
+__device__ __forceinline__ double geom_interp_inner_body(double x, const Rows &R, int n, int c) {
+    GEOM_NOFMA
+#define DIN_(j) (R.st(j, RAFTX_GS_D + c) - 2 * R.st(j, RAFTX_GS_T))
+    if (x < R.st(0, RAFTX_GS_S)) return DIN_(0);
+    if (x > R.st(n - 1, RAFTX_GS_S)) return DIN_(n - 1);
     int j = 0;
     for (int i = 0; i < n; i++)
-        if (gs[(size_t)i * RAFTX_GS_N + RAFTX_GS_S] <= x) j = i;
+        if (R.st(i, RAFTX_GS_S) <= x) j = i;
     const double fj = DIN_(j);
     if (j == n - 1) return fj;
-    const double xj = gs[(size_t)j * RAFTX_GS_N + RAFTX_GS_S];
+    const double xj = R.st(j, RAFTX_GS_S);
     if (xj == x) return fj;
-    const double slope = (DIN_(j + 1) - fj) / (gs[(size_t)(j + 1) * RAFTX_GS_N + RAFTX_GS_S] - xj);
+    const double slope = (DIN_(j + 1) - fj) / (R.st(j + 1, RAFTX_GS_S) - xj);
     return slope * (x - xj) + fj;
 #undef DIN_
 }
+template <class Rows>
+__device__ inline double geom_interp_inner(double x, const Rows &R, int n, int c) { return geom_interp_inner_body(x, R, n, c); }
+__device__ __forceinline__ double geom_interp_inner(double x, const GeomRowsProg &R, int n, int c) { return geom_interp_inner_body(x, R, n, c); }
 __device__ inline void geom_add_submember(double *M, double mass, const double (&Iv)[3], const double *p1, const double *p2,
                                           const double *q, const double (&r)[3], bool whole = false) {
     GEOM_NOFMA
@@ -406,58 +521,58 @@
         geom_add_submember(M, mass, I3, p1, p2, q, rel, !(l > 0));
     }
 }
-__device__ inline int geom_inertia_caps_finish(GInertia &J, const double *gs, int n, const double *gc, int ncap, bool circ,
-                                               double rho_shell, const double *rA, const double *q, const double *p1,
-                                               const double *p2, double g, double *out) {
+template <class Rows>
+__device__ __forceinline__ int geom_inertia_caps_body(GInertia &J, const Rows &R, int n, int ncap, bool circ,
+                                                      double rho_shell, const double *rA, const double *q, const double *p1,
+                                                      const double *p2, double g, double *out) {
     GEOM_NOFMA
     const int c1 = circ ? 0 : 1;
     double (&M)[36] = J.M;
     double (&mc)[3] = J.mc;
     const double vfill = J.vfill;
-    const double s0 = gs[RAFTX_GS_S], s1 = gs[(size_t)(n - 1) * RAFTX_GS_N + RAFTX_GS_S];
+    const double s0 = R.st(0, RAFTX_GS_S), s1 = R.st(n - 1, RAFTX_GS_S);
     for (int i = 0; i < ncap; i++) {
-        const double *cp = gc + (size_t)i * RAFTX_GC_N;
-        const double Lc = cp[RAFTX_GC_S], h = cp[RAFTX_GC_T];
+        const double Lc = R.cap(i, RAFTX_GC_S), h = R.cap(i, RAFTX_GC_T);
         double dA[2] = {0, 0}, dB[2] = {0, 0}, dAi[2] = {0, 0}, dBi[2] = {0, 0};
         int where;
         if (Lc == s0) {
             where = 0;
             for (int c = 0; c <= c1; c++) {
-                dA[c] = gs[RAFTX_GS_D + c] - 2 * gs[RAFTX_GS_T];
-                dB[c] = geom_interp_inner(Lc + h, gs, n, c);
-                dAi[c] = cp[RAFTX_GC_DIN + c];
+                dA[c] = R.st(0, RAFTX_GS_D + c) - 2 * R.st(0, RAFTX_GS_T);
+                dB[c] = geom_interp_inner(Lc + h, R, n, c);
+                dAi[c] = R.cap(i, RAFTX_GC_DIN + c);
                 dBi[c] = dB[c] * (dAi[c] / dA[c]);
             }
         } else if (Lc == s1) {
             where = 1;
             if (!circ) return 2;
-            dA[0] = geom_interp_inner(Lc - h, gs, n, 0);
-            dB[0] = gs[(size_t)(n - 1) * RAFTX_GS_N + RAFTX_GS_D] - 2 * gs[(size_t)(n - 1) * RAFTX_GS_N + RAFTX_GS_T];
-            dBi[0] = cp[RAFTX_GC_DIN];
+            dA[0] = geom_interp_inner(Lc - h, R, n, 0);
+            dB[0] = R.st(n - 1, RAFTX_GS_D) - 2 * R.st(n - 1, RAFTX_GS_T);
+            dBi[0] = R.cap(i, RAFTX_GC_DIN);
             dAi[0] = dA[0] * (dBi[0] / dB[0]);
         } else if ((Lc > s0 && Lc < s0 + h) || (Lc < s1 && Lc > s1 - h)) {
             return 3;
         } else {
             where = 2;
             if (!circ) return 2;
-            if (i < ncap - 1 && Lc == gc[(size_t)(i + 1) * RAFTX_GC_N + RAFTX_GC_S]) {
+            if (i < ncap - 1 && Lc == R.cap(i + 1, RAFTX_GC_S)) {
                 if (i >= n) return 4;
-                dA[0] = geom_interp_inner(Lc - h, gs, n, 0);
-                dB[0] = gs[(size_t)i * RAFTX_GS_N + RAFTX_GS_D] - 2 * gs[(size_t)i * RAFTX_GS_N + RAFTX_GS_T];
-                dBi[0] = cp[RAFTX_GC_DIN];
+                dA[0] = geom_interp_inner(Lc - h, R, n, 0);
+                dB[0] = R.st(i, RAFTX_GS_D) - 2 * R.st(i, RAFTX_GS_T);
+                dBi[0] = R.cap(i, RAFTX_GC_DIN);
                 dAi[0] = dA[0] * (dBi[0] / dB[0]);
-            } else if (i > 0 && Lc == gc[(size_t)(i - 1) * RAFTX_GC_N + RAFTX_GC_S]) {
+            } else if (i > 0 && Lc == R.cap(i - 1, RAFTX_GC_S)) {
                 if (i >= n) return 4;
-                dA[0] = gs[(size_t)i * RAFTX_GS_N + RAFTX_GS_D] - 2 * gs[(size_t)i * RAFTX_GS_N + RAFTX_GS_T];
-                dB[0] = geom_interp_inner(Lc + h, gs, n, 0);
-                dAi[0] = cp[RAFTX_GC_DIN];
+                dA[0] = R.st(i, RAFTX_GS_D) - 2 * R.st(i, RAFTX_GS_T);
+                dB[0] = geom_interp_inner(Lc + h, R, n, 0);
+                dAi[0] = R.cap(i, RAFTX_GC_DIN);
                 dBi[0] = dB[0] * (dAi[0] / dA[0]);
             } else {
-                dA[0] = geom_interp_inner(Lc - h / 2, gs, n, 0);
-                dB[0] = geom_interp_inner(Lc + h / 2, gs, n, 0);
-                const double dM = geom_interp_inner(Lc, gs, n, 0);
-                dAi[0] = dA[0] * (cp[RAFTX_GC_DIN] / dM);
-                dBi[0] = dB[0] * (cp[RAFTX_GC_DIN] / dM);
+                dA[0] = geom_interp_inner(Lc - h / 2, R, n, 0);
+                dB[0] = geom_interp_inner(Lc + h / 2, R, n, 0);
+                const double dM = geom_interp_inner(Lc, R, n, 0);
+                dAi[0] = dA[0] * (R.cap(i, RAFTX_GC_DIN) / dM);
+                dBi[0] = dB[0] * (R.cap(i, RAFTX_GC_DIN) / dM);
             }
         }
         double Vo, hco, Vi, hci;
@@ -505,16 +620,32 @@
     out[47] = vfill;
     return 0;
 }
-__device__ inline int geom_member_inertia(const double *gm, const double *gs, int n, const double *gc, int ncap,
-                                          const double *rA, const double *q, const double *p1, const double *p2, double g,
-                                          bool trim, double drho, double *out) {
-    const bool circ = gm[RAFTX_GM_SHAPE] != 0.0;
-    const double rho_shell = gm[RAFTX_GM_RHOSHELL];
+template <class Rows>
+__device__ inline int geom_inertia_caps_finish(GInertia &J, const Rows &R, int n, int ncap, bool circ, double rho_shell, const double *rA,
+                                               const double *q, const double *p1, const double *p2, double g, double *out) {
+    return geom_inertia_caps_body(J, R, n, ncap, circ, rho_shell, rA, q, p1, p2, g, out);
+}
+__device__ __forceinline__ int geom_inertia_caps_finish(GInertia &J, const GeomRowsProg &R, int n, int ncap, bool circ, double rho_shell,
+                                                        const double *rA, const double *q, const double *p1, const double *p2, double g,
+                                                        double *out) {
+    return geom_inertia_caps_body(J, R, n, ncap, circ, rho_shell, rA, q, p1, p2, g, out);
+}
+template <class Rows>
+__device__ __forceinline__ int geom_member_inertia(const Rows &R, int n, int ncap, const double *rA, const double *q, const double *p1,
+                                                   const double *p2, double g, bool trim, double drho, double *out) {
+    const bool circ = R.mcol(RAFTX_GM_SHAPE) != 0.0;
+    const double rho_shell = R.mcol(RAFTX_GM_RHOSHELL);
     GInertia J;
     geom_inertia_init(J);
-    for (int i = 1; i < n; i++)
-        geom_inertia_section(J, gs + (size_t)(i - 1) * RAFTX_GS_N, gs + (size_t)i * RAFTX_GS_N, circ, rho_shell, trim, drho, rA, q, p1, p2);
-    return geom_inertia_caps_finish(J, gs, n, gc, ncap, circ, rho_shell, rA, q, p1, p2, g, out);
+    double a[RAFTX_GS_N], b[RAFTX_GS_N];
+    R.station(0, b);
+    for (int i = 1; i < n; i++) {
+#pragma unroll
+        for (int f = 0; f < RAFTX_GS_N; f++) a[f] = b[f];
+        R.station(i, b);
+        geom_inertia_section(J, a, b, circ, rho_shell, trim, drho, rA, q, p1, p2);
+    }
+    return geom_inertia_caps_finish(J, R, n, ncap, circ, rho_shell, rA, q, p1, p2, g, out);
 }
 
 __global__ void k_geom_zero(GeomArgs A) {
@@ -527,7 +658,7 @@
     if (d < 4) A.err[d] = 0;
     if (d < 5) A.tot[d] = 0;
     if (d == 0) { A.off[0] = 0; A.cmoff[0] = 0; }
-    if (d < A.nDesign)
+    if (d < A.nDesign && !A.prog.params)
         for (int64_t m = A.mo(d); m < A.mo(d + 1); m++) A.mdesign_w[m] = d;
 }
 #define GEOM_MAX_STATIONS 1024
@@ -539,15 +670,6 @@
     const int d = (int)(t % A.nDesign);
     const int64_t m = A.mo(d) + k;
     return m < A.mo(d + 1) ? m : -1;
-}
-__device__ __forceinline__ void geom_load_row(const double *gs, int i, double (&r)[RAFTX_GS_N]) {
-    const double2 *p = reinterpret_cast<const double2 *>(gs + (size_t)i * RAFTX_GS_N);
-#pragma unroll
-    for (int k = 0; k < RAFTX_GS_N / 2; k++) {
-        const double2 v = p[k];
-        r[2 * k] = v.x;
-        r[2 * k + 1] = v.y;
-    }
 }
 struct GMember {
     int wet, wetm;
@@ -593,21 +715,14 @@
 }
 #define FR_N (MP_N + MH_N + MI_N)
 #define FR_I 4
-__device__ __forceinline__ GMember geom_member_body(const double *gmrow, const double *gs, const int n, const double *gc, const int ncap,
-                                                    const double *pose, const double rho, const double g, const bool trim,
-                                                    const bool haveK, double *mp, double *mh, double *mi) {
+template <class Rows>
+__device__ __forceinline__ GMember geom_member_body(const Rows &rows, const int n, const int ncap, const double *pose, const double rho,
+                                                    const double g, const bool trim, const bool haveK, double *mp, double *mh,
+                                                    double *mi) {
     GEOM_NOFMA
     GMember res = {0, 0, 0, 0};
     double gm[RAFTX_GM_N];
-    {
-        const double2 *p = reinterpret_cast<const double2 *>(gmrow);
-#pragma unroll
-        for (int k = 0; k < RAFTX_GM_N / 2; k++) {
-            const double2 v = p[k];
-            gm[2 * k] = v.x;
-            gm[2 * k + 1] = v.y;
-        }
-    }
+    rows.member(gm);
     if (n < 2 || n > GEOM_MAX_STATIONS || !(gm[RAFTX_GM_DLSMAX] > 0.0) || !(gm[RAFTX_GM_L] > 0.0)) {
         res.rej = 1;
         return res;
@@ -620,7 +735,7 @@
     if (pose)
         for (int i = 0; i < 6; i++) ps[i] = pose[i];
     double a[RAFTX_GS_N], b[RAFTX_GS_N];
-    geom_load_row(gs, 0, b);
+    rows.station(0, b);
     const bool circ = gm[RAFTX_GM_SHAPE] != 0.0;
     const int flags = (int)gm[RAFTX_GM_FLAGS];
     double rA0[3], q[3], p1[3], p2[3], rA[3], rB[3], R[2][2];
@@ -639,7 +754,7 @@
     for (int i = 1; i < n; i++) {
 #pragma unroll
         for (int f = 0; f < RAFTX_GS_N; f++) a[f] = b[f];
-        geom_load_row(gs, i, b);
+        rows.station(i, b);
         {
             const double lstrip = b[RAFTX_GS_S] - a[RAFTX_GS_S];
             const int cntg = geom_interval_strips(lstrip, gm[RAFTX_GM_DLSMAX]);
@@ -738,14 +853,14 @@
     if (!nostatic) {
         GInertia J;
         geom_inertia_init(J);
-        geom_load_row(gs, 0, b);
+        rows.station(0, b);
         for (int i = 1; i < n; i++) {
 #pragma unroll
             for (int f = 0; f < RAFTX_GS_N; f++) a[f] = b[f];
-            geom_load_row(gs, i, b);
+            rows.station(i, b);
             geom_inertia_section(J, a, b, circ, rho_shell, trim, 0.0, rA, q, p1, p2);
         }
-        code = geom_inertia_caps_finish(J, gs, n, gc, ncap, circ, rho_shell, rA, q, p1, p2, g, mi);
+        code = geom_inertia_caps_finish(J, rows, n, ncap, circ, rho_shell, rA, q, p1, p2, g, mi);
     }
     for (int i = 0; i < 3; i++) {
         mp[i] = rA0[i]; mp[3 + i] = rA[i]; mp[6 + i] = q[i]; mp[9 + i] = p1[i]; mp[12 + i] = p2[i];
@@ -780,9 +895,10 @@
     if (f >= F.nFix) return;
     const int *ds = F.desc + (size_t)f * 5;
     double *r = F.rec + (size_t)f * FR_N;
-    const GMember R = geom_member_body(F.gm + (size_t)ds[0] * RAFTX_GM_N, F.gs + (size_t)ds[1] * RAFTX_GS_N, ds[2],
-                                       ds[4] >= 0 ? F.gc + (size_t)ds[3] * RAFTX_GC_N : nullptr, ds[4] >= 0 ? ds[4] : 0, nullptr, F.rho,
-                                       F.g, F.trim != 0, F.haveK != 0, r, r + MP_N, r + MP_N + MH_N);
+    const GeomRowsPlain rows{F.gm + (size_t)ds[0] * RAFTX_GM_N, F.gs + (size_t)ds[1] * RAFTX_GS_N,
+                             ds[4] >= 0 ? F.gc + (size_t)ds[3] * RAFTX_GC_N : nullptr};
+    const GMember R = geom_member_body(rows, ds[2], ds[4] >= 0 ? ds[4] : 0, nullptr, F.rho, F.g, F.trim != 0, F.haveK != 0, r, r + MP_N,
+                                       r + MP_N + MH_N);
     int *ir = F.irec + (size_t)f * FR_I;
     ir[0] = R.wet; ir[1] = R.wetm; ir[2] = R.code; ir[3] = R.rej;
 }
@@ -817,11 +933,19 @@
     } else {
         const int64_t so0 = A.so(m), so1 = A.so(m + 1);
         const int64_t co0 = A.capOff ? A.co(m) : 0, co1 = A.capOff ? A.co(m + 1) : 0;
-        d = A.mdesign[m];
-        R = geom_member_body(A.gm + (size_t)m * RAFTX_GM_N, A.gs + (size_t)so0 * RAFTX_GS_N, (int)(so1 - so0),
-                             A.capOff ? A.caps + (size_t)co0 * RAFTX_GC_N : nullptr, A.capOff ? (int)(co1 - co0) : 0,
-                             A.pose ? A.pose + (size_t)d * 6 : nullptr, A.rho, A.g, (A.add_mask & RAFTX_TRIM_BALLAST) != 0, A.k != nullptr,
-                             A.mpose + (size_t)m * MP_N, A.mhyd + (size_t)m * MH_N, A.minert + (size_t)m * MI_N);
+        const int n = (int)(so1 - so0), ncap = A.capOff ? (int)(co1 - co0) : 0;
+        const bool trim = (A.add_mask & RAFTX_TRIM_BALLAST) != 0;
+        double *mp = A.mpose + (size_t)m * MP_N, *mh = A.mhyd + (size_t)m * MH_N, *mi = A.minert + (size_t)m * MI_N;
+        if (A.prog.params) {
+            d = (int)(m / A.prog.nM);
+            const GeomRowsProg rows(A.prog, (int)(m % A.prog.nM), (int)(so0 - (int64_t)d * A.prog.nSt), (int)(co0 - (int64_t)d * A.prog.nCap), d);
+            R = geom_member_body(rows, n, ncap, A.pose ? A.pose + (size_t)d * 6 : nullptr, A.rho, A.g, trim, A.k != nullptr, mp, mh, mi);
+        } else {
+            d = A.mdesign[m];
+            const GeomRowsPlain rows{A.gm + (size_t)m * RAFTX_GM_N, A.gs + (size_t)so0 * RAFTX_GS_N,
+                                     A.capOff ? A.caps + (size_t)co0 * RAFTX_GC_N : nullptr};
+            R = geom_member_body(rows, n, ncap, A.pose ? A.pose + (size_t)d * 6 : nullptr, A.rho, A.g, trim, A.k != nullptr, mp, mh, mi);
+        }
     }
     if (R.rej) {
         A.cnt[m] = 0;
@@ -860,15 +984,24 @@
     if (A.err[2] | A.err[3]) return;
     const int64_t m = geom_member_of_thread(A);
     if (m < 0) return;
-    const double *gm = A.gm + (size_t)m * RAFTX_GM_N;
-    if ((int)gm[RAFTX_GM_FLAGS] & RAFTX_GM_FLAG_NOSTATIC) return;
-    const double *gs = A.gs + (size_t)A.so(m) * RAFTX_GS_N;
-    const int n = (int)(A.so(m + 1) - A.so(m));
+    const int64_t so0 = A.so(m), co0 = A.capOff ? A.co(m) : 0;
+    const int n = (int)(A.so(m + 1) - so0);
     const double *mp = A.mpose + (size_t)m * MP_N;
-    const int ncap = A.capOff ? (int)(A.co(m + 1) - A.co(m)) : 0;
-    const double *gc = A.capOff ? A.caps + (size_t)A.co(m) * RAFTX_GC_N : nullptr;
+    const int ncap = A.capOff ? (int)(A.co(m + 1) - co0) : 0;
     double *mi = A.minert + (size_t)m * MI_N;
-    if (geom_member_inertia(gm, gs, n, gc, ncap, mp + 3, mp + 6, mp + 9, mp + 12, A.g, true, A.drho[A.mdesign[m]], mi))
+    int code;
+    if (A.prog.params) {
+        const int d = (int)(m / A.prog.nM);
+        const GeomRowsProg rows(A.prog, (int)(m % A.prog.nM), (int)(so0 - (int64_t)d * A.prog.nSt), (int)(co0 - (int64_t)d * A.prog.nCap), d);
+        if ((int)rows.mcol(RAFTX_GM_FLAGS) & RAFTX_GM_FLAG_NOSTATIC) return;
+        code = geom_member_inertia(rows, n, ncap, mp + 3, mp + 6, mp + 9, mp + 12, A.g, true, A.drho[d], mi);
+    } else {
+        const GeomRowsPlain rows{A.gm + (size_t)m * RAFTX_GM_N, A.gs + (size_t)so0 * RAFTX_GS_N,
+                                 A.capOff ? A.caps + (size_t)co0 * RAFTX_GC_N : nullptr};
+        if ((int)rows.mcol(RAFTX_GM_FLAGS) & RAFTX_GM_FLAG_NOSTATIC) return;
+        code = geom_member_inertia(rows, n, ncap, mp + 3, mp + 6, mp + 9, mp + 12, A.g, true, A.drho[A.mdesign[m]], mi);
+    }
+    if (code)
         for (int i = 0; i < MI_N; i++) mi[i] = 0.0;
 }
 
@@ -1043,7 +1176,7 @@
 #define GD_T 128
 #endif
 static_assert(GD_T % 64 == 0 && GD_T % DS_N == 0 && GD_T <= 256, "k_geom_design: whole wavefronts, a lane keeps its record field");
-template <bool ABI, bool ADDUP>
+template <bool ABI, bool ADDUP, bool PROG = false>
 __device__ __forceinline__ void geom_design_block(const GeomArgs &A, const int d, double *gd_lds, int *wcnt) {
     GEOM_NOFMA
     const int lane = threadIdx.x;
@@ -1066,7 +1199,8 @@
         double *smp = sgs + (size_t)nSta * RAFTX_GS_N;
         int cnt_lane = 0;
         {
-            const double *g0 = A.gm + (size_t)m0 * RAFTX_GM_N, *g1 = A.gs + (size_t)s0 * RAFTX_GS_N, *g2 = A.mpose + (size_t)m0 * MP_N;
+            const double *g0 = PROG ? A.prog.gm : A.gm + (size_t)m0 * RAFTX_GM_N, *g1 = PROG ? A.prog.gs : A.gs + (size_t)s0 * RAFTX_GS_N,
+                         *g2 = A.mpose + (size_t)m0 * MP_N;
             const int n0 = nMem * GD_GM_N, n01 = n0 + nSta * RAFTX_GS_N, total = n01 + nMem * GD_MP_N;
             constexpr int SU = 10;
             const int64_t so_lane = lane <= nMem ? A.so(m0 + lane) : s0;
@@ -1096,6 +1230,28 @@
             }
             if (lane <= nMem) mbase[lane] = ssta[lane] = (int)(so_lane - s0);
             for (int mi = lane + GD_T; mi <= nMem; mi += GD_T) mbase[mi] = ssta[mi] = (int)(A.so(m0 + mi) - s0);
+        }
+        if constexpr (PROG) {
+            __syncthreads();
+            const VariantView &V = A.prog;
+            for (int u = lane; u < 2 * nSta; u += GD_T) {
+                const int idx = u >> 1;
+                double *o = sgs + (size_t)idx * RAFTX_GS_N;
+                if (u & 1) {
+                    if (V.diaEdit[idx]) {
+                        const double *p = V.params + (size_t)d * V.nP;
+                        o[RAFTX_GS_D] = variant_station_D(V, idx, 0, p);
+                        o[RAFTX_GS_D + 1] = variant_station_D(V, idx, 1, p);
+                    }
+                } else {
+                    const int bm = V.stMember[idx];
+                    if (V.endEdit[bm]) {
+                        const double L = smp[(size_t)bm * GD_MP_N + 12];
+                        o[RAFTX_GS_S] = variant_station_S(V, idx, L);
+                        o[RAFTX_GS_LFILL] = variant_station_LFILL(V, idx, L);
+                    }
+                }
+            }
         }
         __syncthreads();
         for (int u = lane; u < nSta + nMem; u += GD_T) {
@@ -1436,7 +1592,10 @@
     extern __shared__ double gd_lds[];
     __shared__ int wcnt[GD_T / 64];
     if ((int)blockIdx.x >= A.nDesign) return;
-    if (A.abi) geom_design_block<true, false>(A, (int)blockIdx.x, gd_lds, wcnt);
+    if (A.prog.params) {
+        if (A.addup_in_design) geom_design_block<false, true, true>(A, (int)blockIdx.x, gd_lds, wcnt);
+        else geom_design_block<false, false, true>(A, (int)blockIdx.x, gd_lds, wcnt);
+    } else if (A.abi) geom_design_block<true, false>(A, (int)blockIdx.x, gd_lds, wcnt);
     else if (A.addup_in_design) geom_design_block<false, true>(A, (int)blockIdx.x, gd_lds, wcnt);
     else geom_design_block<false, false>(A, (int)blockIdx.x, gd_lds, wcnt);
 }
@@ -1515,22 +1674,10 @@
     }
 }
 
-struct ExpandArgs {
-    int n, nM, nSt, nCap, nP;
-    const double *params;
-    const double *gm, *gs, *gc;
-    const int *stMember, *capMember;
-    const double *stFrac, *fillFrac, *capFrac;
-    const double *endCoef, *headCS, *diaCoef;
-    const int *endEdit, *diaEdit;
+struct ExpandArgs : VariantView {
+    int n;
     double *gm_out, *gs_out, *gc_out;
 };
-__device__ inline double affine_eval(const double *coef, const double *p, int nP) {
-    GEOM_NOFMA
-    double v = coef[0];
-    for (int q = 0; q < nP; q++) v = v + coef[1 + q] * p[q];
-    return v;
-}
 #define GE_T 256
 __global__ void __launch_bounds__(GE_T) k_geom_expand(ExpandArgs E, unsigned nbM, unsigned nbS) {
     GEOM_NOFMA
@@ -1550,39 +1697,19 @@
         const double *bm = E.gm + (size_t)m * RAFTX_GM_N;
         const bool ed = E.endEdit[m] != 0;
         double e[6] = {0, 0, 0, 0, 0, 0}, L = bm[RAFTX_GM_L];
-        if (ed) {
-            for (int i = 0; i < 6; i++) e[i] = affine_eval(E.endCoef + ((size_t)m * 6 + i) * (E.nP + 1), p, E.nP);
-            const double dx = e[3] - e[0], dy = e[4] - e[1], dz = e[5] - e[2];
-            L = sqrt((dx * dx + dy * dy) + dz * dz);
-        }
+        if (ed) variant_ends(E, m, p, e, L);
         double *o = tile + t * 17;
         if (kind == 0) {
             for (int i = 0; i < RAFTX_GM_N; i++) o[i] = bm[i];
-            if (ed) {
-                const double c = E.headCS[2 * m], s = E.headCS[2 * m + 1];
-                o[RAFTX_GM_RA + 0] = c * e[0] + (-s) * e[1];
-                o[RAFTX_GM_RA + 1] = s * e[0] + c * e[1];
-                o[RAFTX_GM_RA + 2] = e[2];
-                o[RAFTX_GM_RB + 0] = c * e[3] + (-s) * e[4];
-                o[RAFTX_GM_RB + 1] = s * e[3] + c * e[4];
-                o[RAFTX_GM_RB + 2] = e[5];
-                o[RAFTX_GM_L] = L;
-            }
+            if (ed) variant_member_edit(E, m, e, L, o);
         } else if (kind == 1) {
             const double *b = E.gs + (size_t)idx * RAFTX_GS_N;
             for (int i = 0; i < RAFTX_GS_N; i++) o[i] = b[i];
-            if (ed) {
-                o[RAFTX_GS_S] = E.stFrac[idx] * L;
-                o[RAFTX_GS_LFILL] = E.fillFrac[idx] * L;
-            }
-            if (E.diaEdit[idx]) {
-                o[RAFTX_GS_D] = affine_eval(E.diaCoef + ((size_t)idx * 2 + 0) * (E.nP + 1), p, E.nP);
-                o[RAFTX_GS_D + 1] = affine_eval(E.diaCoef + ((size_t)idx * 2 + 1) * (E.nP + 1), p, E.nP);
-            }
+            variant_station_edit(E, idx, ed, L, p, o);
         } else {
             const double *b = E.gc + (size_t)idx * RAFTX_GC_N;
             for (int i = 0; i < RAFTX_GC_N; i++) o[i] = b[i];
-            if (ed) o[RAFTX_GC_S] = E.capFrac[idx] * L;
+            if (ed) o[RAFTX_GC_S] = variant_cap_S(E, idx, L);
         }
     }
     __syncthreads();
diff --git a/raft_amd/csrc/raftx_hip.hip b/raft_amd/csrc/raftx_hip.hip
--- a/raft_amd/csrc/raftx_hip.hip
+++ b/raft_amd/csrc/raftx_hip.hip
@@ -721,14 +721,22 @@
     const FixedRecord *rec = nullptr;
 };
 
+static void variant_view(const VariantProg &P, VariantView &V) {
+    V.nM = P.nM; V.nSt = P.nSt; V.nCap = P.nCap; V.nP = P.nP;
+    V.gm = P.gm; V.gs = P.gs; V.gc = P.gc;
+    V.stMember = P.stMember; V.capMember = P.capMember;
+    V.stFrac = P.stFrac; V.fillFrac = P.fillFrac; V.capFrac = P.capFrac;
+    V.endCoef = P.endCoef; V.headCS = P.headCS; V.diaCoef = P.diaCoef;
+    V.endEdit = P.endEdit; V.diaEdit = P.diaEdit;
+}
 static void expand_args(const VariantProg &P, int n, double *gm_out, double *gs_out, double *gc_out, ExpandArgs &E) {
-    E.n = n; E.nM = P.nM; E.nSt = P.nSt; E.nCap = P.nCap; E.nP = P.nP;
-    E.gm = P.gm; E.gs = P.gs; E.gc = P.gc;
-    E.stMember = P.stMember; E.capMember = P.capMember;
-    E.stFrac = P.stFrac; E.fillFrac = P.fillFrac; E.capFrac = P.capFrac;
-    E.endCoef = P.endCoef; E.headCS = P.headCS; E.diaCoef = P.diaCoef;
-    E.endEdit = P.endEdit; E.diaEdit = P.diaEdit;
+    variant_view(P, E);
+    E.n = n;
     E.gm_out = gm_out; E.gs_out = gs_out; E.gc_out = gc_out;
+}
+static bool fused_gen_asked() {
+    const char *fg = getenv("RAFTX_FUSED_GEN");
+    return fg && atoi(fg);
 }
 
 struct DenseResident {
@@ -1243,13 +1251,21 @@
     if (const VariantProg *P = B.var.prog) {
         if (nMember != nDesign * P->nM || nSta != nDesign * P->nSt || nCap != nDesign * P->nCap)
             FAIL(c, "build_designs: offsets do not describe %d variants of the program's base unit", A.nDesign);
-        double *gm = nullptr, *gs = nullptr, *gc = nullptr;
-        if (pool_alloc(c, tmp, nMember * RAFTX_GM_N, &gm) || pool_alloc(c, tmp, nSta * RAFTX_GS_N, &gs) ||
-            pool_alloc(c, tmp, nCap * RAFTX_GC_N, &gc))
-            return -2;
-        rc |= upload_on(c, sCopy, tmp, B.var.params + lo * P->nP, nDesign * P->nP, &E.params);
-        expand_args(*P, A.nDesign, gm, gs, gc, E);
-        A.gm = gm; A.gs = gs; A.caps = B.capOff ? gc : nullptr;
+        const double *params = nullptr;
+        if (nDesign * P->nP) rc |= upload_on(c, sCopy, tmp, B.var.params + lo * P->nP, nDesign * P->nP, &params);
+        else rc |= pool_alloc(c, tmp, 1, &params);
+        if (fused_gen_asked()) {
+            double *gm = nullptr, *gs = nullptr, *gc = nullptr;
+            if (pool_alloc(c, tmp, nMember * RAFTX_GM_N, &gm) || pool_alloc(c, tmp, nSta * RAFTX_GS_N, &gs) ||
+                pool_alloc(c, tmp, nCap * RAFTX_GC_N, &gc))
+                return -2;
+            E.params = params;
+            expand_args(*P, A.nDesign, gm, gs, gc, E);
+            A.gm = gm; A.gs = gs; A.caps = B.capOff ? gc : nullptr;
+        } else {
+            variant_view(*P, A.prog);
+            A.prog.params = params;
+        }
     } else {
         rc |= upload_on(c, sCopy, tmp, B.members + (size_t)L.m0 * RAFTX_GM_N, nMember * RAFTX_GM_N, &A.gm);
         rc |= upload_on(c, sCopy, tmp, B.stations + (size_t)L.s0 * RAFTX_GS_N, nSta * RAFTX_GS_N, &A.gs);
@@ -1362,7 +1378,7 @@
     HIPCHK(c, hipEventRecord(c->evUp, sCopy));
     HIPCHK(c, hipStreamWaitEvent(sPrep, c->evUp, 0));
     if (B.var.prog && nDesign > 0) {
-        launch_expand(E, sPrep);
+        if (E.gm_out) launch_expand(E, sPrep);
         if (const FixedRecord *R = B.var.rec) {
             if (R->stream != sPrep) HIPCHK(c, hipStreamWaitEvent(sPrep, R->ev, 0));
             A.fixRec = R->rec; A.fixInt = R->irec; A.fixIdx = B.var.prog->fixIdx; A.fixNM = B.var.prog->nM;
@@ -1407,9 +1423,7 @@
     GeomArgs &A = J.A;
     const int nDesign = J.nDesign, nw = J.nw;
     const size_t nRows = J.nRows;
-    const char *fg_ = getenv("RAFTX_FUSED_GEN");
-    const bool fused_gen = fg_ && atoi(fg_);
-    const bool defer = (kind & GEN_MAY_DEFER) && fused_gen && nDesign > 0 && nRows == 0;
+    const bool defer = (kind & GEN_MAY_DEFER) && fused_gen_asked() && !A.prog.params && nDesign > 0 && nRows == 0;
     J.gen_deferred = false;
     const size_t gd_lds = geom_design_lds(J.maxS, (int)J.maxSta, (int)J.maxMem);
     if (gd_lds > 160 * 1024)
```

Result: faster. 706.7 million, median of 6 (+2.7%).
